# jakovdev/SequenceAligner

Hardware: AMD Instinct MI355X
Metric: pair-alignments/sec (higher is better)
Workload: dtype u16x2; 1 GPU; cfg2: 10000 protein seqs x U[80,120], nw blosum62 {'gap_pen': 4}, all-vs-all packed triangular; pairs=49995000, cells=501594494441, parallelism=pair-range x1

## Files before the change

### include/seqalign_hip.h

```cpp
#ifndef SEQALIGN_HIP_H
#define SEQALIGN_HIP_H

#include <stdbool.h>
#include <stddef.h>
#include <stdint.h>

#ifdef __cplusplus
extern "C" {
#endif

#define SA_ABI_VERSION 4


struct sa_meta {
	int32_t off;
	int32_t len;
};

struct sa_input {
	uint8_t *seqs;
	struct sa_meta *meta;
	int32_t max;
	int32_t num;
};

struct sa_output {
	int32_t *matrix;
	const char **seqs;
	size_t dim;
	bool triangular;
};

enum sa_method { SA_METHOD_NW = 0, SA_METHOD_GA = 1, SA_METHOD_SW = 2, SA_METHOD_COUNT = 3 };
enum sa_gap_kind { SA_GAP_LINEAR = 0, SA_GAP_AFFINE = 1 };

#define SA_LUT_SIZE 128
#define SA_SUB_DIM 24
#define SA_SCORE_MIN (INT32_MIN / 2)

struct sa_scoring {
	int32_t method;
	int32_t gap_pen;
	int32_t gap_opn;
	int32_t gap_ext;
	int32_t lut[SA_LUT_SIZE];
	int32_t sub[SA_SUB_DIM * SA_SUB_DIM];
};


bool sa_hip_memory(size_t bytes);

bool sa_hip_align(struct sa_input in, struct sa_output out, const struct sa_scoring *sc);

int32_t sa_hip_filter(struct sa_input in, float threshold, uint8_t *keep);


typedef struct sa_ctx sa_ctx;

sa_ctx *sa_ctx_create(int device, struct sa_input in, const struct sa_scoring *sc);
void sa_ctx_destroy(sa_ctx *ctx);

int64_t sa_ctx_pairs(const sa_ctx *ctx);

int sa_ctx_align_range(sa_ctx *ctx, int64_t start, int64_t count, int32_t *d_scores, void *stream);

int sa_ctx_token_tiles(const sa_ctx *ctx, int64_t *lean, int64_t *legacy);

int sa_ctx_align_host(sa_ctx *ctx, int64_t start, int64_t count, struct sa_output out, double *phase_seconds);

int sa_hip_host_register(void *p, size_t bytes);
int sa_hip_host_unregister(void *p);

int sa_ctx_scores_fit16(const sa_ctx *ctx);
int sa_ctx_align_range16(sa_ctx *ctx, int64_t start, int64_t count, int16_t *d_scores, void *stream);
int sa_hip_widen16(const int16_t *d_src, int32_t *d_dst, int64_t count, void *stream);

int64_t sa_ctx_share_elems(sa_ctx *ctx, int64_t start, int64_t count, int world, int to_host);
int sa_ctx_align_share(sa_ctx *ctx, int64_t start, int64_t count, int world, int rank, void *d_share, int elem16,
		       int32_t *host_packed, void *stream);
int sa_ctx_place_shares(sa_ctx *ctx, int64_t start, int64_t count, int world, int to_host, const void *d_shares, int elem16,
			int32_t *d_packed, void *stream);

void sa_ctx_leave_room(sa_ctx *ctx, int on);

int sa_ctx_expand_full(sa_ctx *ctx, const int32_t *d_packed, int32_t *d_full, void *stream);

#define SA_HIP_Z_PAIR_LEVEL 7
typedef struct sa_zjob sa_zjob;
sa_zjob *sa_zjob_create(int device, const int32_t *d_packed, const int32_t *d_full, int32_t num, size_t chunk_dim, int level);
size_t sa_zjob_tiles_per_row(const sa_zjob *job);
int sa_zjob_tile_row(sa_zjob *job, size_t tile_row, const uint8_t **streams, size_t *sizes);
int sa_zjob_next(sa_zjob *job, uint32_t *rows, uint32_t *cols, const uint8_t **streams, size_t *sizes);
void sa_zjob_stats(const sa_zjob *job, double *encode_ms, double *copy_ms, uint64_t *raw_bytes, uint64_t *out_bytes);
double sa_zjob_align_seconds(const sa_zjob *job);
void sa_zjob_destroy(sa_zjob *job);
sa_zjob *sa_hip_tiles_begin(struct sa_input in, const struct sa_scoring *sc, size_t chunk_dim, int level);

#define SA_HIP_NEIGHBORS_MAX 64
int sa_ctx_neighbors(sa_ctx *ctx, const int32_t *d_packed, int32_t k, int32_t *d_index, int32_t *d_score, void *stream);
bool sa_hip_neighbors(struct sa_input in, const struct sa_scoring *sc, int32_t k, int32_t *index, int32_t *score);
int sa_zjob_neighbors(sa_zjob *job, int32_t k, int32_t *index, int32_t *score);
double sa_hip_last_neighbors_seconds(void);

enum { SA_ALN_M = 0, SA_ALN_I = 1, SA_ALN_D = 2 };
struct sa_aln {
	int32_t score;
	int32_t a_begin, a_end;
	int32_t b_begin, b_end;
	int32_t columns;
	int32_t identities;
	int32_t cigar_len;
	int64_t cigar_off;
};
typedef struct sa_alns sa_alns;
sa_alns *sa_ctx_alignments(sa_ctx *ctx, const int32_t *a, const int32_t *b, int64_t npairs);
sa_alns *sa_hip_alignments(struct sa_input in, const struct sa_scoring *sc, const int32_t *a, const int32_t *b, int64_t npairs);
const struct sa_aln *sa_alns_records(const sa_alns *alns);
const uint32_t *sa_alns_cigar(const sa_alns *alns, int64_t *runs);
int64_t sa_alns_count(const sa_alns *alns);
void sa_alns_destroy(sa_alns *alns);
double sa_hip_last_alignments_seconds(void);
void sa_hip_last_alignments_breakdown(double *fill_seconds, double *walk_seconds, int64_t *cells, int32_t *batches);

int sa_ctx_edge_offsets(sa_ctx *ctx, const int32_t *d_packed, int32_t min_score, int64_t *d_offsets, void *stream);
int sa_ctx_edge_fill(sa_ctx *ctx, const int32_t *d_packed, int32_t min_score, const int64_t *d_offsets,
		     int32_t *d_index, int32_t *d_score, void *stream);
typedef struct sa_edges sa_edges;
sa_edges *sa_hip_edges(struct sa_input in, const struct sa_scoring *sc, int32_t min_score);
sa_edges *sa_zjob_edges(sa_zjob *job, int32_t min_score);
const int64_t *sa_edges_offsets(const sa_edges *e, int32_t *num);
const int32_t *sa_edges_index(const sa_edges *e, int64_t *count);
const int32_t *sa_edges_score(const sa_edges *e);
void sa_edges_destroy(sa_edges *e);
double sa_hip_last_edges_seconds(void);

size_t sa_linkage_scratch_bytes(int32_t num);
int sa_ctx_linkage(sa_ctx *ctx, const int32_t *d_packed, int32_t *d_pairs, int32_t *d_score, void *d_scratch, void *stream);
typedef struct sa_linkage sa_linkage;
sa_linkage *sa_hip_linkage(struct sa_input in, const struct sa_scoring *sc);
sa_linkage *sa_zjob_linkage(sa_zjob *job);
const int32_t *sa_linkage_pairs(const sa_linkage *l, int32_t *merges);
const int32_t *sa_linkage_score(const sa_linkage *l);
void sa_linkage_destroy(sa_linkage *l);
double sa_hip_last_linkage_seconds(void);
int sa_hip_last_linkage_rounds(void);
int32_t sa_linkage_labels(const int32_t *pairs, const int32_t *score, int32_t num, int32_t min_score, int32_t *labels);
int sa_linkage_merges(const int32_t *pairs, int32_t num, int32_t *left, int32_t *right, int32_t *size);

#define SA_HIP_SELECT_MAX 16
size_t  sa_select_scratch_bytes(int32_t m);
int64_t sa_score_rank(int64_t pairs, double q);
int  sa_ctx_select(sa_ctx *ctx, const int32_t *d_packed, const int64_t *ranks, int32_t m,
		   int32_t *d_value, int64_t *d_below, void *d_scratch, void *stream);
bool sa_hip_select(struct sa_input in, const struct sa_scoring *sc, const int64_t *ranks, int32_t m, int32_t *value, int64_t *below);
int  sa_zjob_select(sa_zjob *job, const int64_t *ranks, int32_t m, int32_t *value, int64_t *below);
sa_edges   *sa_hip_edges_at_rank(struct sa_input in, const struct sa_scoring *sc, int64_t rank, int32_t *min_score, int64_t *below);
sa_linkage *sa_hip_linkage_with_ranks(struct sa_input in, const struct sa_scoring *sc, const int64_t *ranks, int32_t m,
				      int32_t *value, int64_t *below);
double sa_hip_last_select_seconds(void);

enum { SA_NORM_SELF = 0, SA_NORM_LENGTH = 1 };
enum { SA_NORM_MIN = 0, SA_NORM_MAX = 1, SA_NORM_MEAN = 2 };
#define SA_NORM_SCALE 1000000
struct sa_norm {
	int32_t source;
	int32_t rule;
	int32_t *denominators;
};
int32_t sa_norm_value(int32_t s, int32_t di, int32_t dj, int32_t rule);
int sa_ctx_denominators(sa_ctx *ctx, int32_t source, int32_t *d_den, void *stream);
int sa_ctx_normalize(sa_ctx *ctx, const int32_t *d_packed, const int32_t *d_den, int32_t rule, int32_t *d_out, void *stream);
int sa_zjob_normalize(sa_zjob *job, const struct sa_norm *norm);
bool sa_hip_neighbors_norm(struct sa_input in, const struct sa_scoring *sc, int32_t k, int32_t *index, int32_t *score, const struct sa_norm *norm);
sa_edges *sa_hip_edges_norm(struct sa_input in, const struct sa_scoring *sc, int32_t min_score, const struct sa_norm *norm);
sa_linkage *sa_hip_linkage_norm(struct sa_input in, const struct sa_scoring *sc, const struct sa_norm *norm);
bool sa_hip_select_norm(struct sa_input in, const struct sa_scoring *sc, const int64_t *ranks, int32_t m, int32_t *value, int64_t *below,
			const struct sa_norm *norm);
sa_edges *sa_hip_edges_at_rank_norm(struct sa_input in, const struct sa_scoring *sc, int64_t rank, int32_t *min_score, int64_t *below,
				    const struct sa_norm *norm);
sa_linkage *sa_hip_linkage_with_ranks_norm(struct sa_input in, const struct sa_scoring *sc, const int64_t *ranks, int32_t m,
					   int32_t *value, int64_t *below, const struct sa_norm *norm);
double sa_hip_last_normalize_seconds(void);

enum { SA_PID_COLUMNS = 0, SA_PID_SHORTER = 1, SA_PID_LONGER = 2, SA_PID_MEAN = 3 };
struct sa_identity_out {
	int32_t *score, *identities, *columns, *pid;
	int32_t denom;
};
int32_t sa_pid_value(int32_t identities, int32_t columns, int32_t len_i, int32_t len_j, int32_t denom);
int sa_ctx_identity_range(sa_ctx *ctx, int64_t start, int64_t count, const struct sa_identity_out *d_out, void *stream);
bool sa_hip_identity(struct sa_input in, const struct sa_scoring *sc, int32_t denom, int32_t *identities, int32_t *columns, int32_t *pid);
int sa_zjob_identity(sa_zjob *job, int32_t denom);
bool sa_hip_neighbors_pid(struct sa_input in, const struct sa_scoring *sc, int32_t k, int32_t *index, int32_t *score, int32_t denom);
sa_edges *sa_hip_edges_pid(struct sa_input in, const struct sa_scoring *sc, int32_t min_score, int32_t denom);
sa_linkage *sa_hip_linkage_pid(struct sa_input in, const struct sa_scoring *sc, int32_t denom);
bool sa_hip_select_pid(struct sa_input in, const struct sa_scoring *sc, const int64_t *ranks, int32_t m, int32_t *value, int64_t *below,
		       int32_t denom);
sa_edges *sa_hip_edges_at_rank_pid(struct sa_input in, const struct sa_scoring *sc, int64_t rank, int32_t *min_score, int64_t *below,
				   int32_t denom);
sa_linkage *sa_hip_linkage_with_ranks_pid(struct sa_input in, const struct sa_scoring *sc, const int64_t *ranks, int32_t m,
					  int32_t *value, int64_t *below, int32_t denom);
double sa_hip_last_identity_seconds(void);

int64_t sa_pairs_cells(const struct sa_meta *meta, int32_t num, int64_t start, int64_t count);
int sa_pairs_partition(const struct sa_meta *meta, int32_t num, int parts, int64_t *bounds);

void sa_ctx_timing(sa_ctx *ctx, int enable);
int sa_ctx_timing_read(sa_ctx *ctx, char *kernel_name, int cap, int64_t *launches, double *total_ms,
		       int64_t *pairs, int64_t *cells, double *all_kernels_ms);


int sa_matrix_load(const char *name, int32_t lut[SA_LUT_SIZE], int32_t sub[SA_SUB_DIM * SA_SUB_DIM]);
int sa_matrix_count(void);
const char *sa_matrix_name(int index);
int sa_matrix_is_nucleotide(int index);

int sa_method_parse(const char *alias);
const char *sa_method_name(int method);
int sa_method_gap_kind(int method);
// ... 31 lines not shown
```

### sequencealigner_amd/binding.py

```python
from __future__ import annotations

import ctypes as C
import importlib.util
import os
import pathlib
import sys
from dataclasses import dataclass, field
from typing import Iterable, Optional, Sequence

import numpy as np

_LIB_PATH = pathlib.Path(__file__).resolve().parent / "lib" / "libseqalign_hip.so"
_lib: Optional[C.CDLL] = None

LUT_SIZE = 128
NEIGHBORS_MAX = 64
SUB_DIM = 24
SCORE_MIN = -(1 << 30)

METHOD_NW, METHOD_GA, METHOD_SW = 0, 1, 2
GAP_LINEAR, GAP_AFFINE = 0, 1


class AlignError(RuntimeError):
    """A call through the C ABI returned failure (message = sa_last_error())."""


class _Meta(C.Structure):
    _fields_ = [("off", C.c_int32), ("len", C.c_int32)]


class _Input(C.Structure):
    _fields_ = [("seqs", C.c_void_p), ("meta", C.c_void_p), ("max", C.c_int32), ("num", C.c_int32)]


class _Output(C.Structure):
    _fields_ = [("matrix", C.c_void_p), ("seqs", C.c_void_p), ("dim", C.c_size_t), ("triangular", C.c_bool)]


class _Scoring(C.Structure):
    _fields_ = [("method", C.c_int32), ("gap_pen", C.c_int32), ("gap_opn", C.c_int32), ("gap_ext", C.c_int32),
                ("lut", C.c_int32 * LUT_SIZE), ("sub", C.c_int32 * (SUB_DIM * SUB_DIM))]


ABI_SYMBOLS = (
    "sa_hip_memory", "sa_hip_align", "sa_hip_filter", "sa_ctx_create", "sa_ctx_destroy", "sa_ctx_pairs", "sa_pairs_cells",
    "sa_ctx_align_range", "sa_ctx_align_range16", "sa_ctx_token_tiles", "sa_ctx_scores_fit16", "sa_hip_widen16", "sa_ctx_expand_full", "sa_pairs_partition", "sa_ctx_timing", "sa_ctx_timing_read",
    "sa_matrix_load", "sa_matrix_count", "sa_matrix_name", "sa_matrix_is_nucleotide", "sa_method_parse",
    "sa_method_name", "sa_method_gap_kind", "sa_hip_device_count", "sa_hip_device_name", "sa_last_error",
    "sa_abi_version",
    "sa_hip_last_align_seconds", "sa_ctx_align_host", "sa_hip_host_register", "sa_hip_host_unregister",
    "sa_ctx_share_elems", "sa_ctx_align_share", "sa_ctx_place_shares", "sa_hip_last_align_breakdown", "sa_ctx_leave_room", "sa_hip_set_progress",
    "sa_hip_last_align_path",
    "sa_zjob_create", "sa_zjob_destroy", "sa_zjob_tiles_per_row", "sa_zjob_tile_row", "sa_zjob_stats", "sa_zjob_next", "sa_zjob_align_seconds", "sa_hip_tiles_begin",
    "sa_ctx_neighbors", "sa_hip_neighbors", "sa_zjob_neighbors", "sa_hip_last_neighbors_seconds",
    "sa_ctx_alignments", "sa_hip_alignments", "sa_alns_records", "sa_alns_cigar", "sa_alns_count", "sa_alns_destroy",
    "sa_hip_last_alignments_seconds", "sa_hip_last_alignments_breakdown",
    "sa_norm_value", "sa_ctx_denominators", "sa_ctx_normalize", "sa_zjob_normalize", "sa_hip_neighbors_norm", "sa_hip_edges_norm",
    "sa_hip_linkage_norm", "sa_hip_select_norm", "sa_hip_edges_at_rank_norm", "sa_hip_linkage_with_ranks_norm", "sa_hip_last_normalize_seconds",
    "sa_ctx_edge_offsets", "sa_ctx_edge_fill", "sa_hip_edges", "sa_zjob_edges", "sa_edges_offsets", "sa_edges_index", "sa_edges_score",
    "sa_edges_destroy", "sa_hip_last_edges_seconds",
    "sa_linkage_scratch_bytes", "sa_ctx_linkage", "sa_hip_linkage", "sa_zjob_linkage", "sa_linkage_pairs", "sa_linkage_score",
    "sa_linkage_destroy", "sa_hip_last_linkage_seconds", "sa_hip_last_linkage_rounds", "sa_linkage_labels", "sa_linkage_merges",
    "sa_select_scratch_bytes", "sa_score_rank", "sa_ctx_select", "sa_hip_select", "sa_zjob_select", "sa_hip_edges_at_rank",
    "sa_hip_linkage_with_ranks", "sa_hip_last_select_seconds",
    "sa_pid_value", "sa_ctx_identity_range", "sa_hip_identity", "sa_zjob_identity", "sa_hip_neighbors_pid", "sa_hip_edges_pid",
    "sa_hip_linkage_pid", "sa_hip_select_pid", "sa_hip_edges_at_rank_pid", "sa_hip_linkage_with_ranks_pid", "sa_hip_last_identity_seconds",
)


class _Norm(C.Structure):
    _fields_ = [("source", C.c_int32), ("rule", C.c_int32), ("denominators", C.c_void_p)]


class _IdentityOut(C.Structure):
    _fields_ = [("score", C.c_void_p), ("identities", C.c_void_p), ("columns", C.c_void_p), ("pid", C.c_void_p), ("denom", C.c_int32)]


def library_path() -> pathlib.Path:
    return _LIB_PATH


def _share_hip_runtime_with_torch() -> None:
    if "torch" in sys.modules or os.environ.get("SA_HIP_NO_TORCH_RUNTIME"):
        return
    try:
        spec = importlib.util.find_spec("torch")
    except (ImportError, ValueError):
        return
    if spec is None or not spec.submodule_search_locations:
        return
    cand = pathlib.Path(list(spec.submodule_search_locations)[0]) / "lib" / "libamdhip64.so"
    if cand.exists():
        C.CDLL(str(cand), mode=C.RTLD_GLOBAL)


def load_library() -> C.CDLL:
    global _lib
    if _lib is not None:
        return _lib
    if not _LIB_PATH.exists():
        raise AlignError(f"{_LIB_PATH} is missing: run `python __graft_entry__.py` (hipcc, gfx950) first; "
                         "there is no CPU fallback")
    _share_hip_runtime_with_torch()
    lib = C.CDLL(str(_LIB_PATH))
    lib.sa_hip_memory.argtypes = [C.c_size_t]
    lib.sa_hip_memory.restype = C.c_bool
    lib.sa_hip_align.argtypes = [_Input, _Output, C.POINTER(_Scoring)]
    lib.sa_hip_align.restype = C.c_bool
    lib.sa_hip_filter.argtypes = [_Input, C.c_float, C.c_void_p]
    lib.sa_hip_filter.restype = C.c_int32
    lib.sa_ctx_create.argtypes = [C.c_int, _Input, C.POINTER(_Scoring)]
    lib.sa_ctx_create.restype = C.c_void_p
    lib.sa_ctx_destroy.argtypes = [C.c_void_p]
    lib.sa_ctx_destroy.restype = None
    lib.sa_ctx_pairs.argtypes = [C.c_void_p]
    lib.sa_ctx_pairs.restype = C.c_int64
    lib.sa_pairs_cells.argtypes = [C.c_void_p, C.c_int32, C.c_int64, C.c_int64]
    lib.sa_pairs_cells.restype = C.c_int64
    lib.sa_ctx_align_range.argtypes = [C.c_void_p, C.c_int64, C.c_int64, C.c_void_p, C.c_void_p]
    lib.sa_ctx_align_range.restype = C.c_int
    lib.sa_ctx_token_tiles.argtypes = [C.c_void_p, C.POINTER(C.c_int64), C.POINTER(C.c_int64)]
    lib.sa_ctx_token_tiles.restype = C.c_int
    lib.sa_ctx_align_range16.argtypes = [C.c_void_p, C.c_int64, C.c_int64, C.c_void_p, C.c_void_p]
    lib.sa_ctx_align_range16.restype = C.c_int
    lib.sa_ctx_scores_fit16.argtypes = [C.c_void_p]
    lib.sa_ctx_scores_fit16.restype = C.c_int
    lib.sa_hip_widen16.argtypes = [C.c_void_p, C.c_void_p, C.c_int64, C.c_void_p]
    lib.sa_hip_widen16.restype = C.c_int
    lib.sa_ctx_expand_full.argtypes = [C.c_void_p, C.c_void_p, C.c_void_p, C.c_void_p]
    lib.sa_ctx_expand_full.restype = C.c_int
    lib.sa_pairs_partition.argtypes = [C.c_void_p, C.c_int32, C.c_int, C.POINTER(C.c_int64)]
    lib.sa_pairs_partition.restype = C.c_int
    lib.sa_ctx_timing.argtypes = [C.c_void_p, C.c_int]
    lib.sa_ctx_timing.restype = None
    lib.sa_ctx_timing_read.argtypes = [C.c_void_p, C.c_char_p, C.c_int, C.POINTER(C.c_int64), C.POINTER(C.c_double),
                                       C.POINTER(C.c_int64), C.POINTER(C.c_int64), C.POINTER(C.c_double)]
    lib.sa_ctx_timing_read.restype = C.c_int
    lib.sa_matrix_load.argtypes = [C.c_char_p, C.POINTER(C.c_int32), C.POINTER(C.c_int32)]
    lib.sa_matrix_load.restype = C.c_int
    lib.sa_matrix_count.restype = C.c_int
    lib.sa_matrix_name.argtypes = [C.c_int]
    lib.sa_matrix_name.restype = C.c_char_p
    lib.sa_matrix_is_nucleotide.argtypes = [C.c_int]
    lib.sa_matrix_is_nucleotide.restype = C.c_int
    lib.sa_method_parse.argtypes = [C.c_char_p]
    lib.sa_method_parse.restype = C.c_int
    lib.sa_method_name.argtypes = [C.c_int]
    lib.sa_method_name.restype = C.c_char_p
    lib.sa_method_gap_kind.argtypes = [C.c_int]
    lib.sa_method_gap_kind.restype = C.c_int
    lib.sa_hip_device_count.restype = C.c_int
    lib.sa_hip_device_name.argtypes = [C.c_int]
    lib.sa_hip_device_name.restype = C.c_char_p
    lib.sa_last_error.restype = C.c_char_p
    lib.sa_abi_version.restype = C.c_int
    lib.sa_hip_last_align_seconds.restype = C.c_double
    lib.sa_hip_last_align_path.restype = C.c_int
    lib.sa_ctx_align_host.argtypes = [C.c_void_p, C.c_int64, C.c_int64, _Output, C.POINTER(C.c_double)]
    lib.sa_ctx_align_host.restype = C.c_int
    lib.sa_hip_host_register.argtypes = [C.c_void_p, C.c_size_t]
    lib.sa_hip_host_register.restype = C.c_int
    lib.sa_hip_host_unregister.argtypes = [C.c_void_p]
    lib.sa_hip_host_unregister.restype = C.c_int
    lib.sa_hip_last_align_breakdown.argtypes = [C.POINTER(C.c_double), C.c_int]
    lib.sa_hip_last_align_breakdown.restype = C.c_int
    lib.sa_hip_set_progress.argtypes = [C.c_void_p, C.c_void_p]
    lib.sa_hip_set_progress.restype = None
    lib.sa_ctx_leave_room.argtypes = [C.c_void_p, C.c_int]
    lib.sa_ctx_leave_room.restype = None
    lib.sa_ctx_share_elems.argtypes = [C.c_void_p, C.c_int64, C.c_int64, C.c_int, C.c_int]
    lib.sa_ctx_share_elems.restype = C.c_int64
    lib.sa_ctx_align_share.argtypes = [C.c_void_p, C.c_int64, C.c_int64, C.c_int, C.c_int, C.c_void_p, C.c_int, C.c_void_p, C.c_void_p]
    lib.sa_ctx_align_share.restype = C.c_int
    lib.sa_ctx_place_shares.argtypes = [C.c_void_p, C.c_int64, C.c_int64, C.c_int, C.c_int, C.c_void_p, C.c_int, C.c_void_p, C.c_void_p]
    lib.sa_ctx_place_shares.restype = C.c_int
    lib.sa_zjob_create.argtypes = [C.c_int, C.c_void_p, C.c_void_p, C.c_int32, C.c_size_t, C.c_int]
    lib.sa_zjob_create.restype = C.c_void_p
    lib.sa_zjob_destroy.argtypes = [C.c_void_p]
    lib.sa_zjob_destroy.restype = None
    lib.sa_zjob_tiles_per_row.argtypes = [C.c_void_p]
    lib.sa_zjob_tiles_per_row.restype = C.c_size_t
    lib.sa_zjob_tile_row.argtypes = [C.c_void_p, C.c_size_t, C.POINTER(C.c_void_p), C.POINTER(C.c_size_t)]
    lib.sa_zjob_tile_row.restype = C.c_int
    lib.sa_zjob_stats.argtypes = [C.c_void_p, C.POINTER(C.c_double), C.POINTER(C.c_double), C.POINTER(C.c_uint64), C.POINTER(C.c_uint64)]
    lib.sa_zjob_stats.restype = None
    lib.sa_zjob_next.argtypes = [C.c_void_p, C.POINTER(C.c_uint32), C.POINTER(C.c_uint32), C.POINTER(C.c_void_p), C.POINTER(C.c_size_t)]
    lib.sa_zjob_next.restype = C.c_int
    lib.sa_zjob_align_seconds.argtypes = [C.c_void_p]
    lib.sa_zjob_align_seconds.restype = C.c_double
    lib.sa_hip_tiles_begin.argtypes = [_Input, C.POINTER(_Scoring), C.c_size_t, C.c_int]
    lib.sa_hip_tiles_begin.restype = C.c_void_p
    lib.sa_ctx_neighbors.argtypes = [C.c_void_p, C.c_void_p, C.c_int32, C.c_void_p, C.c_void_p, C.c_void_p]
    lib.sa_ctx_neighbors.restype = C.c_int
    lib.sa_hip_neighbors.argtypes = [_Input, C.POINTER(_Scoring), C.c_int32, C.c_void_p, C.c_void_p]
    lib.sa_hip_neighbors.restype = C.c_bool
    lib.sa_zjob_neighbors.argtypes = [C.c_void_p, C.c_int32, C.c_void_p, C.c_void_p]
    lib.sa_zjob_neighbors.restype = C.c_int
    lib.sa_hip_last_neighbors_seconds.restype = C.c_double
    lib.sa_ctx_alignments.argtypes = [C.c_void_p, C.c_void_p, C.c_void_p, C.c_int64]
    lib.sa_ctx_alignments.restype = C.c_void_p
    lib.sa_hip_alignments.argtypes = [_Input, C.POINTER(_Scoring), C.c_void_p, C.c_void_p, C.c_int64]
    lib.sa_hip_alignments.restype = C.c_void_p
    lib.sa_alns_records.argtypes = [C.c_void_p]
    lib.sa_alns_records.restype = C.c_void_p
    lib.sa_alns_cigar.argtypes = [C.c_void_p, C.POINTER(C.c_int64)]
    lib.sa_alns_cigar.restype = C.c_void_p
    lib.sa_alns_count.argtypes = [C.c_void_p]
    lib.sa_alns_count.restype = C.c_int64
    lib.sa_alns_destroy.argtypes = [C.c_void_p]
    lib.sa_alns_destroy.restype = None
    lib.sa_hip_last_alignments_seconds.restype = C.c_double
    lib.sa_hip_last_alignments_breakdown.argtypes = [C.POINTER(C.c_double), C.POINTER(C.c_double), C.POINTER(C.c_int64), C.POINTER(C.c_int32)]
    lib.sa_hip_last_alignments_breakdown.restype = None
    lib.sa_ctx_edge_offsets.argtypes = [C.c_void_p, C.c_void_p, C.c_int32, C.c_void_p, C.c_void_p]
    lib.sa_ctx_edge_offsets.restype = C.c_int
    lib.sa_ctx_edge_fill.argtypes = [C.c_void_p, C.c_void_p, C.c_int32, C.c_void_p, C.c_void_p, C.c_void_p, C.c_void_p]
    lib.sa_ctx_edge_fill.restype = C.c_int
    lib.sa_hip_edges.argtypes = [_Input, C.POINTER(_Scoring), C.c_int32]
    lib.sa_hip_edges.restype = C.c_void_p
    lib.sa_zjob_edges.argtypes = [C.c_void_p, C.c_int32]
    lib.sa_zjob_edges.restype = C.c_void_p
    lib.sa_edges_offsets.argtypes = [C.c_void_p, C.POINTER(C.c_int32)]
    lib.sa_edges_offsets.restype = C.c_void_p
    lib.sa_edges_index.argtypes = [C.c_void_p, C.POINTER(C.c_int64)]
    lib.sa_edges_index.restype = C.c_void_p
    lib.sa_edges_score.argtypes = [C.c_void_p]
    lib.sa_edges_score.restype = C.c_void_p
    lib.sa_edges_destroy.argtypes = [C.c_void_p]
    lib.sa_edges_destroy.restype = None
    lib.sa_hip_last_edges_seconds.restype = C.c_double
    lib.sa_linkage_scratch_bytes.argtypes = [C.c_int32]
    lib.sa_linkage_scratch_bytes.restype = C.c_size_t
    lib.sa_ctx_linkage.argtypes = [C.c_void_p, C.c_void_p, C.c_void_p, C.c_void_p, C.c_void_p, C.c_void_p]
    lib.sa_ctx_linkage.restype = C.c_int
    lib.sa_hip_linkage.argtypes = [_Input, C.POINTER(_Scoring)]
    lib.sa_hip_linkage.restype = C.c_void_p
    lib.sa_zjob_linkage.argtypes = [C.c_void_p]
    lib.sa_zjob_linkage.restype = C.c_void_p
    lib.sa_linkage_pairs.argtypes = [C.c_void_p, C.POINTER(C.c_int32)]
    lib.sa_linkage_pairs.restype = C.c_void_p
    lib.sa_linkage_score.argtypes = [C.c_void_p]
    lib.sa_linkage_score.restype = C.c_void_p
    lib.sa_linkage_destroy.argtypes = [C.c_void_p]
    lib.sa_linkage_destroy.restype = None
    lib.sa_hip_last_linkage_seconds.restype = C.c_double
    lib.sa_hip_last_linkage_rounds.restype = C.c_int
    lib.sa_linkage_labels.argtypes = [C.c_void_p, C.c_void_p, C.c_int32, C.c_int32, C.c_void_p]
    lib.sa_linkage_labels.restype = C.c_int32
    lib.sa_linkage_merges.argtypes = [C.c_void_p, C.c_int32, C.c_void_p, C.c_void_p, C.c_void_p]
    lib.sa_linkage_merges.restype = C.c_int
    lib.sa_select_scratch_bytes.argtypes = [C.c_int32]
    lib.sa_select_scratch_bytes.restype = C.c_size_t
    lib.sa_score_rank.argtypes = [C.c_int64, C.c_double]
    lib.sa_score_rank.restype = C.c_int64
    lib.sa_ctx_select.argtypes = [C.c_void_p, C.c_void_p, C.c_void_p, C.c_int32, C.c_void_p, C.c_void_p, C.c_void_p, C.c_void_p]
    lib.sa_ctx_select.restype = C.c_int
    lib.sa_hip_select.argtypes = [_Input, C.POINTER(_Scoring), C.c_void_p, C.c_int32, C.c_void_p, C.c_void_p]
    lib.sa_hip_select.restype = C.c_bool
    lib.sa_zjob_select.argtypes = [C.c_void_p, C.c_void_p, C.c_int32, C.c_void_p, C.c_void_p]
    lib.sa_zjob_select.restype = C.c_int
    lib.sa_hip_edges_at_rank.argtypes = [_Input, C.POINTER(_Scoring), C.c_int64, C.POINTER(C.c_int32), C.POINTER(C.c_int64)]
    lib.sa_hip_edges_at_rank.restype = C.c_void_p
    lib.sa_hip_linkage_with_ranks.argtypes = [_Input, C.POINTER(_Scoring), C.c_void_p, C.c_int32, C.c_void_p, C.c_void_p]
    lib.sa_hip_linkage_with_ranks.restype = C.c_void_p
    lib.sa_hip_last_select_seconds.restype = C.c_double
    lib.sa_norm_value.argtypes = [C.c_int32, C.c_int32, C.c_int32, C.c_int32]
    lib.sa_norm_value.restype = C.c_int32
    lib.sa_ctx_denominators.argtypes = [C.c_void_p, C.c_int32, C.c_void_p, C.c_void_p]
    lib.sa_ctx_denominators.restype = C.c_int
    lib.sa_ctx_normalize.argtypes = [C.c_void_p, C.c_void_p, C.c_void_p, C.c_int32, C.c_void_p, C.c_void_p]
    lib.sa_ctx_normalize.restype = C.c_int
    lib.sa_zjob_normalize.argtypes = [C.c_void_p, C.POINTER(_Norm)]
    lib.sa_zjob_normalize.restype = C.c_int
    lib.sa_hip_neighbors_norm.argtypes = lib.sa_hip_neighbors.argtypes + [C.POINTER(_Norm)]
    lib.sa_hip_neighbors_norm.restype = C.c_bool
# ... 515 lines not shown

@dataclass
class Alignments:
    pairs: np.ndarray
    records: np.ndarray
    cigar: np.ndarray

    def runs(self, t: int) -> list[tuple[int, str]]:
        r = self.records[t]
        return [(int(w) >> 4, CIGAR_OPS[int(w) & 15]) for w in self.cigar[int(r["cigar_off"]):int(r["cigar_off"]) + int(r["cigar_len"])]]

    def cigar_string(self, t: int) -> str:
        return "".join(f"{n}{op}" for n, op in self.runs(t))

    def aligned(self, t: int, store: "SequenceStore") -> tuple[str, str]:
        r = self.records[t]
        sa, sb = store.sequence(int(self.pairs[t, 0])).decode(), store.sequence(int(self.pairs[t, 1])).decode()
        i, j, ga, gb = int(r["a_begin"]), int(r["b_begin"]), [], []
        for n, op in self.runs(t):
            ga.append(sa[i:i + n] if op != "D" else "-" * n)
            gb.append(sb[j:j + n] if op != "I" else "-" * n)
            i += n if op != "D" else 0
            j += n if op != "I" else 0
        return "".join(ga), "".join(gb)


def _pairs_array(pairs) -> np.ndarray:
    arr = np.asarray(pairs, dtype=np.int64).reshape(-1, 2) if len(pairs) else np.zeros((0, 2), np.int64)
    if arr.size and (arr.min() < -2**31 or arr.max() >= 2**31):
        raise AlignError("pair indices must be int32")
    return np.ascontiguousarray(arr.astype(np.int32))


def _take_alignments(lib, handle, pairs: np.ndarray) -> Alignments:
    if not handle:
        raise AlignError(_err())
    try:
        n = int(lib.sa_alns_count(handle))
        runs = C.c_int64(0)
        cig = lib.sa_alns_cigar(handle, C.byref(runs))
        rec = lib.sa_alns_records(handle)
        records = np.frombuffer(C.string_at(rec, n * ALN_DTYPE.itemsize), dtype=ALN_DTYPE).copy() if n else np.zeros(0, ALN_DTYPE)
        cigar = np.frombuffer(C.string_at(cig, 4 * runs.value), dtype=np.uint32).copy() if runs.value else np.zeros(0, np.uint32)
    finally:
        lib.sa_alns_destroy(handle)
    return Alignments(pairs=pairs, records=records, cigar=cigar)


def hip_alignments(store: SequenceStore, scoring: Scoring, pairs) -> Alignments:
    lib = load_library()
    arr = _pairs_array(pairs)
    a, b = np.ascontiguousarray(arr[:, 0]), np.ascontiguousarray(arr[:, 1])
    sc = scoring._as_c()
    return _take_alignments(lib, lib.sa_hip_alignments(store._as_c(), C.byref(sc), a.ctypes.data, b.ctypes.data, len(arr)), arr)


def last_alignments_seconds() -> float:
    return float(load_library().sa_hip_last_alignments_seconds())


def last_alignments_breakdown() -> dict:
    f, w, c, b = C.c_double(0), C.c_double(0), C.c_int64(0), C.c_int32(0)
    load_library().sa_hip_last_alignments_breakdown(C.byref(f), C.byref(w), C.byref(c), C.byref(b))
    return {"fill_seconds": f.value, "walk_seconds": w.value, "cells": c.value, "batches": b.value}


class PinnedMatrix:

    def __init__(self, elements: int, shared: Optional[str] = None, create: bool = True):
        self._lib = load_library()
        if shared is not None:
            if create:
                with open(shared, "wb") as f:
                    f.truncate(4 * max(int(elements), 1))
            self.array = np.memmap(shared, dtype=np.int32, mode="r+", shape=(max(int(elements), 1),))[:int(elements)]
        else:
            import mmap
            self._map = mmap.mmap(-1, 4 * max(int(elements), 1))
            self.array = np.frombuffer(self._map, dtype=np.int32)[:int(elements)]
        self.path = shared
        self._registered = False
        if elements and self._lib.sa_hip_host_register(C.c_void_p(self.array.ctypes.data), self.array.nbytes):
            raise AlignError(_err())
        self._registered = bool(elements)

    @property
    def ptr(self) -> int:
        return int(self.array.ctypes.data)

    def close(self) -> None:
        if self._registered:
            self._registered = False
            try:
                self._lib.sa_hip_host_unregister(C.c_void_p(self.array.ctypes.data))
            except ImportError:
                pass

    __del__ = close


def hip_filter(store: SequenceStore, threshold: float) -> np.ndarray:
    keep = np.ones(store.num, dtype=np.uint8)
    rc = load_library().sa_hip_filter(store._as_c(), C.c_float(threshold), keep.ctypes.data)
    if rc < 0:
        raise AlignError(_err())
    return keep.astype(bool)


class Context:

    def __init__(self, store: SequenceStore, scoring: Scoring, device: int = 0):
        self._lib = load_library()
        self._store = store
        sc = scoring._as_c()
        self._h = self._lib.sa_ctx_create(int(device), store._as_c(), C.byref(sc))
        if not self._h:
            raise AlignError(_err())
        self.num = store.num
        self.device = int(device)

    def close(self) -> None:
        if getattr(self, "_h", None):
            self._lib.sa_ctx_destroy(self._h)
            self._h = None

    __del__ = close

    def __enter__(self):
        return self

    def __exit__(self, *exc):
        self.close()

    @property
    def pairs(self) -> int:
        return int(self._lib.sa_ctx_pairs(self._h))

    def cells(self, start: int = 0, count: Optional[int] = None) -> int:
        return self._store.cells(start, count)

    def partition(self, parts: int) -> list[int]:
        return self._store.partition(parts)

    def align_range(self, start: int, count: int, d_scores_ptr: int, stream: int = 0) -> None:
        if self._lib.sa_ctx_align_range(self._h, start, count, C.c_void_p(d_scores_ptr), C.c_void_p(stream)):
            raise AlignError(_err())

    def token_tiles(self) -> tuple[int, int]:
        lean, legacy = C.c_int64(0), C.c_int64(0)
        if self._lib.sa_ctx_token_tiles(self._h, C.byref(lean), C.byref(legacy)):
            raise AlignError(_err())
        return int(lean.value), int(legacy.value)

    @property
    def scores_fit16(self) -> bool:
        return bool(self._lib.sa_ctx_scores_fit16(self._h))

    def align_range16(self, start: int, count: int, d_scores16_ptr: int, stream: int = 0) -> None:
        if self._lib.sa_ctx_align_range16(self._h, start, count, C.c_void_p(d_scores16_ptr), C.c_void_p(stream)):
            raise AlignError(_err())

    def widen16(self, d_src16_ptr: int, d_dst32_ptr: int, count: int, stream: int = 0) -> None:
        if self._lib.sa_hip_widen16(C.c_void_p(d_src16_ptr), C.c_void_p(d_dst32_ptr), count, C.c_void_p(stream)):
            raise AlignError(_err())

    def leave_room(self, on: bool) -> None:
        self._lib.sa_ctx_leave_room(self._h, int(on))

    def share_elems(self, start: int, count: int, world: int, to_host: bool = False) -> int:
        v = int(self._lib.sa_ctx_share_elems(self._h, start, count, world, int(to_host)))
        if v < 0:
            raise AlignError(_err())
        return v

    def align_share(self, start: int, count: int, world: int, rank: int, d_share_ptr: int, elem16: bool, stream: int = 0,
                    host_packed_ptr: int = 0) -> None:
        if self._lib.sa_ctx_align_share(self._h, start, count, world, rank, C.c_void_p(d_share_ptr), int(elem16),
                                        C.c_void_p(host_packed_ptr or None), C.c_void_p(stream)):
            raise AlignError(_err())

    def place_shares(self, start: int, count: int, world: int, d_shares_ptr: int, elem16: bool, d_packed_ptr: int, stream: int = 0,
                     to_host: bool = False) -> None:
        if self._lib.sa_ctx_place_shares(self._h, start, count, world, int(to_host), C.c_void_p(d_shares_ptr), int(elem16),
                                         C.c_void_p(d_packed_ptr), C.c_void_p(stream)):
            raise AlignError(_err())

    def align_host(self, matrix: Optional[np.ndarray], triangular: bool, start: int = 0, count: Optional[int] = None) -> float:
        count = self.pairs - start if count is None else count
        out = _Output(matrix.ctypes.data if matrix is not None else None, None, self.num, bool(triangular))
        phase = C.c_double()
        if self._lib.sa_ctx_align_host(self._h, start, count, out, C.byref(phase)):
            raise AlignError(_err())
        return float(phase.value)

    def expand_full(self, d_packed_ptr: int, d_full_ptr: int, stream: int = 0) -> None:
        if self._lib.sa_ctx_expand_full(self._h, C.c_void_p(d_packed_ptr), C.c_void_p(d_full_ptr), C.c_void_p(stream)):
            raise AlignError(_err())

    def neighbors(self, d_packed_ptr: int, k: int, d_index_ptr: int, d_score_ptr: int, stream: int = 0) -> None:
        if self._lib.sa_ctx_neighbors(self._h, C.c_void_p(d_packed_ptr), int(k), C.c_void_p(d_index_ptr), C.c_void_p(d_score_ptr),
                                      C.c_void_p(stream)):
            raise AlignError(_err())

    def edge_offsets(self, d_packed_ptr: int, min_score: int, d_offsets_ptr: int, stream: int = 0) -> None:
        if self._lib.sa_ctx_edge_offsets(self._h, C.c_void_p(d_packed_ptr), _min_score(min_score), C.c_void_p(d_offsets_ptr),
                                         C.c_void_p(stream)):
            raise AlignError(_err())

    def edge_fill(self, d_packed_ptr: int, min_score: int, d_offsets_ptr: int, d_index_ptr: int, d_score_ptr: int, stream: int = 0) -> None:
        if self._lib.sa_ctx_edge_fill(self._h, C.c_void_p(d_packed_ptr), _min_score(min_score), C.c_void_p(d_offsets_ptr),
                                      C.c_void_p(d_index_ptr), C.c_void_p(d_score_ptr), C.c_void_p(stream)):
            raise AlignError(_err())

    def linkage(self, d_packed_ptr: int, d_pairs_ptr: int, d_score_ptr: int, d_scratch_ptr: int, stream: int = 0) -> None:
        if self._lib.sa_ctx_linkage(self._h, C.c_void_p(d_packed_ptr), C.c_void_p(d_pairs_ptr), C.c_void_p(d_score_ptr),
                                    C.c_void_p(d_scratch_ptr), C.c_void_p(stream)):
            raise AlignError(_err())

    def select(self, d_packed_ptr: int, ranks, d_value_ptr: int, d_below_ptr: int, d_scratch_ptr: int, stream: int = 0) -> None:
        r = _ranks(ranks)
        if self._lib.sa_ctx_select(self._h, C.c_void_p(d_packed_ptr), r.ctypes.data, len(r), C.c_void_p(d_value_ptr),
                                   C.c_void_p(d_below_ptr), C.c_void_p(d_scratch_ptr), C.c_void_p(stream)):
            raise AlignError(_err())

    def denominators(self, source: int, d_den_ptr: int, stream: int = 0) -> None:
        source = int(source)
        if not -2**31 <= source < 2**31:
            raise AlignError(f"source = {source} is not an int32")
        if self._lib.sa_ctx_denominators(self._h, source, C.c_void_p(d_den_ptr or None), C.c_void_p(stream)):
            raise AlignError(_err())

    def normalize(self, d_packed_ptr: int, d_den_ptr: int, rule: int, d_out_ptr: int, stream: int = 0) -> None:
        rule = int(rule)
        if not -2**31 <= rule < 2**31:
            raise AlignError(f"rule = {rule} is not an int32")
        if self._lib.sa_ctx_normalize(self._h, C.c_void_p(d_packed_ptr or None), C.c_void_p(d_den_ptr or None), rule,
                                      C.c_void_p(d_out_ptr or None), C.c_void_p(stream)):
            raise AlignError(_err())

    def identity_range(self, start: int, count: int, score: int = 0, identities: int = 0, columns: int = 0, pid: int = 0,
                       denom: int = 0, stream: int = 0) -> None:
        out = _IdentityOut(score or None, identities or None, columns or None, pid or None, _denom(denom))
        if self._lib.sa_ctx_identity_range(self._h, int(start), int(count), C.byref(out), C.c_void_p(stream)):
            raise AlignError(_err())

    def alignments(self, pairs) -> Alignments:
        arr = _pairs_array(pairs)
        a, b = np.ascontiguousarray(arr[:, 0]), np.ascontiguousarray(arr[:, 1])
        return _take_alignments(self._lib, self._lib.sa_ctx_alignments(self._h, a.ctypes.data, b.ctypes.data, len(arr)), arr)

    def timing(self, enable: bool) -> None:
        self._lib.sa_ctx_timing(self._h, int(enable))

    def timing_read(self) -> dict:
        name = C.create_string_buffer(256)
        launches, pairs, cells = C.c_int64(), C.c_int64(), C.c_int64()
        ms, all_ms = C.c_double(), C.c_double()
        if self._lib.sa_ctx_timing_read(self._h, name, 256, C.byref(launches), C.byref(ms), C.byref(pairs),
                                        C.byref(cells), C.byref(all_ms)):
            raise AlignError(_err())
        return dict(kernel=name.value.decode(), launches=int(launches.value), ms=float(ms.value),
                    pairs=int(pairs.value), cells=int(cells.value), all_kernels_ms=float(all_ms.value))


class DeflateJob:

    def __init__(self, num: int, chunk_dim: int, d_packed_ptr: int = 0, d_full_ptr: int = 0, device: int = 0, level: int = 6, _handle=None):
        self._lib = load_library()
        self._h = _handle or self._lib.sa_zjob_create(int(device), C.c_void_p(d_packed_ptr or None), C.c_void_p(d_full_ptr or None),
                                                      int(num), int(chunk_dim), int(level))
        if not self._h:
            raise AlignError(_err())
        self.tiles_per_row = int(self._lib.sa_zjob_tiles_per_row(self._h))
        self.num = int(num)

    @classmethod
    def begin(cls, store: "SequenceStore", scoring: "Scoring", chunk_dim: int, level: int = 6) -> "DeflateJob":
        lib = load_library()
        sc = scoring._as_c()
        h = lib.sa_hip_tiles_begin(store._as_c(), C.byref(sc), int(chunk_dim), int(level))
        if not h:
            raise AlignError(_err())
        job = cls(store.num, chunk_dim, _handle=h)
        job._store = store
        return job

    def next(self) -> list[tuple[int, int, bytes]]:
        n = self.tiles_per_row
        rows, cols = (C.c_uint32 * n)(), (C.c_uint32 * n)()
        ptrs, sizes = (C.c_void_p * n)(), (C.c_size_t * n)()
        got = self._lib.sa_zjob_next(self._h, rows, cols, ptrs, sizes)
        if got < 0:
            raise AlignError(_err())
        return [(int(rows[t]), int(cols[t]), C.string_at(ptrs[t], sizes[t])) for t in range(got)]

    @property
    def align_seconds(self) -> float:
        return float(self._lib.sa_zjob_align_seconds(self._h))

    def tile_row(self, row: int) -> list[bytes]:
        ptrs = (C.c_void_p * self.tiles_per_row)()
        sizes = (C.c_size_t * self.tiles_per_row)()
        if self._lib.sa_zjob_tile_row(self._h, int(row), ptrs, sizes):
            raise AlignError(_err())
        return [C.string_at(ptrs[t], sizes[t]) for t in range(self.tiles_per_row)]

# ... 49 lines not shown
```

### sequencealigner_amd/csrc/sa_context.hip

```cpp
#include <algorithm>
#include <cmath>
#include <cstdio>
#include <cstdlib>
#include <cstring>

#include "sa_ctx.h"

bool sa_device_ready(int device)
{
	int count = 0;
	hipError_t err = hipGetDeviceCount(&count);
	if (err != hipSuccess || count <= 0) {
		sa_set_error("No HIP devices available (%s); libseqalign_hip has no CPU fallback",
			     err == hipSuccess ? "device count is 0" : hipGetErrorString(err));
		return false;
	}
	if (device < 0 || device >= count) {
		sa_set_error("HIP device %d out of range (%d visible)", device, count);
		return false;
	}
	SA_HIP_CHECK(hipSetDevice(device), return false);
	return true;
}

extern "C" int sa_hip_device_count(void)
{
	int count = 0;
	if (hipGetDeviceCount(&count) != hipSuccess)
		return 0;
	return count;
}

extern "C" const char *sa_hip_device_name(int device)
{
	static thread_local char name[256];
	hipDeviceProp_t prop;
	if (hipGetDeviceProperties(&prop, device) != hipSuccess)
		return nullptr;
	snprintf(name, sizeof(name), "%s (%s, %d CUs)", prop.name, prop.gcnArchName, prop.multiProcessorCount);
	return name;
}

static bool validate_and_encode(const sa_input &in, const sa_scoring &sc, std::vector<uint8_t> &codes,
				std::vector<int32_t> &off, int32_t &max_len)
{
	if (!in.seqs || !in.meta) {
		sa_set_error("sa_input: null sequence store");
		return false;
	}
	if (in.num < 2) {
		sa_set_error("Not enough sequences: %d (min: 2)", in.num);
		return false;
	}
	if (sc.method < 0 || sc.method >= SA_METHOD_COUNT) {
		sa_set_error("Invalid alignment method id %d", sc.method);
		return false;
	}
	int64_t end = 0;
	max_len = 0;
	off.assign((size_t)in.num + 1, 0);
	for (int32_t k = 0; k < in.num; k++) {
		const sa_meta m = in.meta[k];
		if (m.len < 1 || m.off < 0) {
			sa_set_error("Sequence #%d has invalid offset/length (%d/%d)", k + 1, m.off, m.len);
			return false;
		}
		off[(size_t)k] = (int32_t)end;
		end += (int64_t)m.len + 1;
		max_len = std::max(max_len, m.len);
		if (end > INT32_MAX) {
			sa_set_error("Sequence store exceeds 2 GiB");
			return false;
		}
	}
	off[(size_t)in.num] = (int32_t)end;
	codes.assign((size_t)end, (uint8_t)SA_CODE_SEP);
	for (int32_t k = 0; k < in.num; k++) {
		const sa_meta m = in.meta[k];
		const uint8_t *s = in.seqs + m.off;
		for (int32_t p = 0; p < m.len; p++) {
			const uint8_t ch = s[p];
			const int32_t idx = ch < SA_LUT_SIZE ? sc.lut[ch] : -1;
			if (idx < 0 || idx >= SA_SUB_DIM) {
				sa_set_error("Invalid character 0x%02x in sequence #%d at position %d", ch, k + 1, p + 1);
				return false;
			}
			codes[(size_t)off[(size_t)k] + p] = (uint8_t)idx;
		}
		if (s[m.len] != 0) {
			sa_set_error("Sequence #%d is not NUL-terminated at its recorded length", k + 1);
			return false;
		}
	}
	int64_t amax = 0, smax = 0;
	if (sc.method == SA_METHOD_NW)
		amax = std::llabs((int64_t)sc.gap_pen);
	else
		amax = std::max(std::llabs((int64_t)sc.gap_opn), std::llabs((int64_t)sc.gap_ext));
	for (int k = 0; k < SA_SUB_DIM * SA_SUB_DIM; k++)
		smax = std::max<int64_t>(smax, std::llabs((int64_t)sc.sub[k]));
	const __int128 bound = (__int128)(2 * (int64_t)max_len + 3) * amax + (__int128)max_len * smax;
	if (bound >= ((__int128)1 << 30)) {
		sa_set_error("Gap penalty %lld with sequence length %d overflows 32-bit scores "
			     "(undefined in the reference as well)", (long long)amax, max_len);
		return false;
	}
	return true;
}

SaPlanInputs sa_plan_inputs(const sa_ctx *ctx)
{
	SaPlanInputs in;
	in.num = ctx->num;
	in.meta = ctx->meta.data();
	in.min_len = ctx->min_len;
	in.method = ctx->sc.method;
	in.gap_ext = ctx->sc.gap_ext;
	in.sys_ok = ctx->sys_ok;
	in.pk_kmax = ctx->pk_kmax;
	in.pk16_kmax = ctx->pk16_kmax;
	in.pk16_f16_kmax = ctx->pk16_f16_kmax;
	in.pk_chunk_cap = ctx->pk_chunk_cap;
	in.pk_q = ctx->pk_q;
	in.pk_floor = ctx->pk_floor;
	in.pk_gain = ctx->pk_gain;
	in.pk_slack = ctx->pk_slack;
	in.persistent_wgs = ctx->persistent_wgs;
	in.env_chunk = ctx->env.chunk;
	in.no_sort = ctx->env.no_sort;
	in.no_tokens = ctx->env.no_tokens;
	return in;
}

namespace {
struct CtxDeleter {
	void operator()(sa_ctx *c) const { sa_ctx_destroy(c); }
};
}

static sa_ctx *ctx_create_impl(int device, struct sa_input in, const struct sa_scoring *sc)
{
	if (!sc) {
		sa_set_error("sa_ctx_create: null scoring");
		return nullptr;
	}
	std::vector<uint8_t> codes;
	std::vector<int32_t> off;
	int32_t max_len = 0;
	const auto t_encode = std::chrono::steady_clock::now();
	if (!validate_and_encode(in, *sc, codes, off, max_len))
		return nullptr;
	const double encode_ms = sa_ms_since(t_encode);
	const SaEnv env = sa_env_read();
	const bool verbose = env.verbose;
	const auto t_create = std::chrono::steady_clock::now();
	auto since = [&]() { return std::chrono::duration<double, std::milli>(std::chrono::steady_clock::now() - t_create).count(); };
	if (!sa_device_ready(device))
		return nullptr;
	const double device_ms = since();
	if (verbose)
		fprintf(stderr, "[seqalign_hip] sa_ctx_create: device ready at %.1f ms\n", since());

	std::unique_ptr<sa_ctx, CtxDeleter> holder(new sa_ctx());
	sa_ctx *ctx = holder.get();
	ctx->env = env;
	ctx->setup.encode = encode_ms;
	ctx->setup.device = device_ms;
	ctx->device = device;
	ctx->num = in.num;
	ctx->max_len = max_len;
	ctx->min_len = max_len;
	for (int32_t k = 0; k < in.num; k++)
		ctx->min_len = std::min<int32_t>(ctx->min_len, (int32_t)in.meta[k].len);
	ctx->pairs = (int64_t)in.num * (in.num - 1) / 2;
	ctx->sc = *sc;
	ctx->meta.resize((size_t)in.num);
	for (int32_t k = 0; k < in.num; k++)
		ctx->meta[(size_t)k] = sa_meta{ off[(size_t)k], in.meta[k].len };
	ctx->off = off;
	ctx->codes = codes;
	{
		const SaKernelLimits L = sa_kernel_limits(*sc, max_len, ctx->min_len, env.force_generic, env.no_pk, env.no_pk16);
		ctx->sys_ok = L.sys_ok;
		ctx->sys_pconst = L.sys_pconst;
		ctx->sys_q = L.sys_q;
		ctx->sys_gain = L.sys_gain;
		ctx->sys_slack = L.sys_slack;
		ctx->pk_kmax = L.pk_kmax;
		ctx->pk16_kmax = L.pk16_kmax;
		ctx->pk16_f16_kmax = L.pk16_f16_kmax;
		ctx->pk_chunk_cap = L.pk_chunk_cap;
		ctx->pk_pconst = L.pk_pconst;
		ctx->pk_q = L.pk_q;
		ctx->pk_floor = L.pk_floor;
		ctx->pk_gain = L.pk_gain;
		ctx->pk_slack = L.pk_slack;
		ctx->pk_extra = L.pk_extra;
	}
	const bool col_major = sc->method != SA_METHOD_NW;
	int8_t sub8[SA_SUB_DIM * SA_SUB_DIM];
	for (int a = 0; a < SA_SUB_DIM; a++)
		for (int b = 0; b < SA_SUB_DIM; b++)
			sub8[a * SA_SUB_DIM + b] = (int8_t)std::max(-128, std::min(127, sc->sub[col_major ? b * SA_SUB_DIM + a : a * SA_SUB_DIM + b]));

	bool ok = false;
	do {
		SA_HIP_CHECK(hipMalloc(&ctx->d_codes, codes.size()), break);
		SA_HIP_CHECK(hipMalloc(&ctx->d_meta, sizeof(sa_meta) * (size_t)in.num), break);
		SA_HIP_CHECK(hipMalloc(&ctx->d_sub, sizeof(sc->sub)), break);
		if (verbose)
			fprintf(stderr, "[seqalign_hip] sa_ctx_create: first allocations at %.1f ms\n", since());
		SA_HIP_CHECK(hipMemcpy(ctx->d_codes, codes.data(), codes.size(), hipMemcpyHostToDevice), break);
		if (verbose)
			fprintf(stderr, "[seqalign_hip] sa_ctx_create: first upload at %.1f ms\n", since());
		SA_HIP_CHECK(hipMemcpy(ctx->d_meta, ctx->meta.data(), sizeof(sa_meta) * (size_t)in.num, hipMemcpyHostToDevice), break);
		SA_HIP_CHECK(hipMemcpy(ctx->d_sub, sc->sub, sizeof(sc->sub), hipMemcpyHostToDevice), break);
		SA_HIP_CHECK(hipMalloc(&ctx->d_off, sizeof(int32_t) * off.size()), break);
		SA_HIP_CHECK(hipMemcpy(ctx->d_off, off.data(), sizeof(int32_t) * off.size(), hipMemcpyHostToDevice), break);
		SA_HIP_CHECK(hipMalloc(&ctx->d_sub8, sizeof(sub8)), break);
		SA_HIP_CHECK(hipMemcpy(ctx->d_sub8, sub8, sizeof(sub8), hipMemcpyHostToDevice), break);
		if (verbose)
			fprintf(stderr, "[seqalign_hip] sa_ctx_create: uploads at %.1f ms\n", since());

		hipDeviceProp_t prop;
		SA_HIP_CHECK(hipGetDeviceProperties(&prop, device), break);
		ctx->scratch_stride = 2 * ((int64_t)max_len + 2);
		int64_t blocks = (int64_t)prop.multiProcessorCount * 8;
		const int64_t budget = (int64_t)1 << 30;
		const int64_t per_block = ctx->scratch_stride * 4 * (int64_t)sizeof(int32_t);
		blocks = std::max<int64_t>(prop.multiProcessorCount, std::min(blocks, budget / per_block));
		ctx->generic_blocks = (int)blocks;
		SA_HIP_CHECK(hipMalloc(&ctx->d_scratch, (size_t)(blocks * per_block)), break);
		SA_HIP_CHECK(hipMalloc(&ctx->d_counters, sizeof(unsigned) * sa_ctx::COUNTER_SLOTS * sa_ctx::COUNTERS_PER_SLOT), break);
		SA_HIP_CHECK(hipMemset(ctx->d_counters, 0, sizeof(unsigned) * sa_ctx::COUNTER_SLOTS * sa_ctx::COUNTERS_PER_SLOT), break);
		if (verbose)
			fprintf(stderr, "[seqalign_hip] sa_ctx_create: scratch at %.1f ms\n", since());
		ctx->persistent_wgs = prop.multiProcessorCount * 32;
		int families = 0;
		for (int32_t k = 0; k < in.num; k++) {
			const int n = in.meta[k].len, k8 = (n + 7) / 8, k16 = (n + 15) / 16;
			families |= k8 <= ctx->pk_kmax ? SA_WARM_PK8
				    : (k16 >= SA_PK_K16_MIN && k16 <= ctx->pk16_kmax) ? (sa_pk_bundle_klo(16, k16) >= 45 ? SA_WARM_PK16HI : SA_WARM_PK16)
										       : SA_WARM_S32;
		}
		if (verbose)
			fprintf(stderr, "[seqalign_hip] sa_ctx_create: buffers, streams and events at %.1f ms\n", since());
		ctx->setup.upload = since() - device_ms;
		const double t_warm = since();
		SA_HIP_CHECK(sa_warm_kernels(sc->method, families), break);
		ctx->setup.code_objects = since() - t_warm;
		if (verbose)
			fprintf(stderr, "[seqalign_hip] sa_ctx_create: code objects of families %d loaded at %.1f ms\n", families, since());
		ok = true;
	} while (0);
	if (!ok)
		return nullptr;
	return holder.release();
}

extern "C" sa_ctx *sa_ctx_create(int device, struct sa_input in, const struct sa_scoring *sc)
{
	return sa_guard("sa_ctx_create", (sa_ctx *)nullptr, [&] { return ctx_create_impl(device, in, sc); });
}

extern "C" void sa_ctx_destroy(sa_ctx *ctx)
{
	if (!ctx)
		return;
	(void)hipSetDevice(ctx->device);
	for (auto &ev : ctx->events) {
		(void)hipEventDestroy(ev.e0);
		(void)hipEventDestroy(ev.e1);
	}
	sa_plan_release(ctx);
	sa_deliver_release(ctx);
	for (auto &ar : ctx->arranged) {
		(void)hipFree(ar.d_codes);
		(void)hipFree(ar.d_off);
		(void)hipFree(ar.d_rowmap);
		(void)hipFree(ar.d_posmap);
		(void)hipFree(ar.d_tok);
		(void)hipFree(ar.d_tok_off);
		(void)hipFree(ar.d_mine);
// ... 157 lines not shown
```

### sequencealigner_amd/csrc/sa_ctx.h

```cpp
#ifndef SA_CTX_H
#define SA_CTX_H

#include <atomic>
#include <chrono>
#include <deque>
#include <exception>
#include <memory>
#include <new>
#include <string>
#include <vector>

#include "sa_env.h"
#include "sa_guard.h"
#include "sa_internal.h"
#include "sa_plan.h"

struct sa_ctx {
	int device = 0;
	int32_t num = 0, max_len = 0, min_len = 0;
	int64_t pairs = 0;
	sa_scoring sc{};
	SaEnv env;
	std::vector<sa_meta> meta;
	std::vector<int32_t> off;
	std::vector<uint8_t> codes;
	uint8_t *d_codes = nullptr;
	sa_meta *d_meta = nullptr;
	int32_t *d_off = nullptr;
	int32_t *d_sub = nullptr;
	int8_t *d_sub8 = nullptr;
	int32_t *d_scratch = nullptr;
	int64_t scratch_stride = 0;
	int generic_blocks = 0;
	void *d_id_scratch = nullptr;
	enum { COUNTER_SLOTS = 256, COUNTERS_PER_SLOT = 2 * SA_PLAN_NCLASSES };
	unsigned *d_counters = nullptr;
	uint64_t call_no = 0;
	hipEvent_t slot_done[COUNTER_SLOTS] = {};
	bool slot_dirty[COUNTER_SLOTS] = {};
	int32_t *d_long_scratch = nullptr;
	int64_t long_stride = 0;
	int long_wgs = 0;
	int persistent_wgs = 0;
	bool sys_ok = false;
	int32_t sys_pconst = 0, sys_q = 0;
	int64_t sys_gain = 0, sys_slack = 0;
	int pk_kmax = 0, pk16_kmax = 0;
	int pk16_f16_kmax = 0;
	int pk_chunk_cap = SA_SYS_CHUNK;
	int32_t pk_pconst = 0, pk_q = 0, pk_floor = 0;
	int64_t pk_gain = 0, pk_slack = 0, pk_extra = 0;
	struct Arranged {
		SaArrKey key;
		uint8_t *d_codes = nullptr;
		int32_t *d_off = nullptr, *d_rowmap = nullptr, *d_posmap = nullptr;
		uint16_t *d_tok = nullptr, *d_mine = nullptr, *d_any = nullptr;
		int32_t *d_tok_off = nullptr;
	};
	std::deque<Arranged> arranged;
	int64_t tok_lean = 0, tok_legacy = 0;
	bool out_is_host = false;
	struct Plan {
		SaHostPlan h;
		struct DevClass {
			int32_t *d_jlist = nullptr, *d_tprefix = nullptr, *d_tlist = nullptr;
			int64_t *d_doff = nullptr;
		};
		struct DevBundle {
			SaPkClassArgs *d_args = nullptr;
			uint32_t *d_ulist = nullptr;
		};
		std::vector<DevClass> dc;
		std::vector<DevBundle> db;
		SaPlaceSeg *d_segs = nullptr;
		int32_t nsegs = 0;
		uint64_t stamp = 0;
	};
	std::vector<std::unique_ptr<Plan>> plans;
	Plan *plan = nullptr;
	uint64_t plan_clock = 0;
	bool timing = false;
	struct Timed {
		std::string name;
		hipEvent_t e0, e1;
		int64_t pairs, cells;
	};
	std::vector<Timed> events;
	bool leave_room = false;
	struct ProgItem {
		const unsigned *counter;
		int64_t tiles;
	};
	std::vector<ProgItem> prog_items;
	struct SetupMs {
		double encode = 0, device = 0, upload = 0, code_objects = 0, pin = 0, plan = 0, arrange = 0;
	} setup;
	struct Deliver {
		hipStream_t compute = nullptr, copy = nullptr;
		hipEvent_t done[2] = {}, copied[2] = {};
		int32_t *d_buf[2] = {};
		int64_t buf_elems[2] = {};
		int32_t *h_stage[2] = {};
		int64_t stage_elems[2] = {};
		int32_t *d_packed = nullptr, *d_full = nullptr;
		int64_t packed_elems = 0, full_elems = 0;
		unsigned *h_counters = nullptr;
		int64_t h_counters_n = 0;
	} dl;
};

static inline double sa_ms_since(std::chrono::steady_clock::time_point t0)
{
	return std::chrono::duration<double, std::milli>(std::chrono::steady_clock::now() - t0).count();
}

bool sa_device_ready(int device);
bool sa_arranged_store(sa_ctx *ctx, const SaArrKey &key, const sa_ctx::Arranged **out);
SaPlanInputs sa_plan_inputs(const sa_ctx *ctx);

void sa_plan_release(sa_ctx *ctx);
bool sa_plan_get(sa_ctx *ctx, int64_t start, int64_t count, int world, bool share_host);
bool sa_prepare_range(sa_ctx *ctx, int64_t start, int64_t count, bool host_out);
int sa_align_range_impl(sa_ctx *ctx, int64_t start, int64_t count, int32_t *d_scores, void *stream, bool out16,
			int world = 0, int rank = 0, int32_t *host_out = nullptr);

void sa_deliver_release(sa_ctx *ctx);
bool sa_host_range_is_pinned(const void *p, size_t bytes);
size_t sa_host_available_bytes();
bool sa_host_range_in_malloc_heap(const void *p, size_t bytes);

bool sa_progress_wanted();
void sa_report_progress(double fraction);
void sa_progress_speaker(bool here);
int sa_devices_in_use(const SaEnv &env);

bool sa_align_gathered(struct sa_input in, struct sa_output out, const struct sa_scoring *sc, const int *devices, int ndev,
		       double *phase_seconds, double *breakdown_ms);
bool sa_rccl_available(std::string *why);

bool sa_norm_check(const char *who, const struct sa_norm *norm);
bool sa_normalize_in_place(const char *who, sa_ctx *ctx, int32_t *d_packed, const struct sa_norm *norm, hipStream_t s);

bool sa_identity_denom_check(const char *who, int32_t denom);
bool sa_identity_in_place(const char *who, sa_ctx *ctx, int32_t *d_packed, int32_t denom, hipStream_t s);

#endif
```

### sequencealigner_amd/csrc/sa_env.cpp

```cpp
#include "sa_env.h"

#include <algorithm>
#include <cstdlib>

static bool flag(const char *name) { return getenv(name) != nullptr; }
static int number(const char *name, int fallback, int lo, int hi)
{
	const char *v = getenv(name);
	if (!v || !*v)
		return fallback;
	return std::max(lo, std::min(hi, atoi(v)));
}

SaEnv sa_env_read()
{
	SaEnv e;
	e.force_generic = flag("SA_HIP_FORCE_GENERIC");
	e.no_pk = flag("SA_HIP_NO_PK");
	e.no_pk16 = flag("SA_HIP_NO_PK16");
	e.no_sort = flag("SA_HIP_NO_SORT");
	e.no_tokens = flag("SA_HIP_NO_TOKENS");
	e.chunk = number("SA_HIP_CHUNK", 0, 1, 32);
	e.stagger = number("SA_HIP_STAGGER", 0, 0, 64);
	e.no_pin = flag("SA_HIP_NO_PIN");
	e.no_direct = flag("SA_HIP_NO_DIRECT");
	e.no_shells = flag("SA_HIP_NO_SHELLS");
	e.devices = number("SA_HIP_DEVICES", 0, 0, 1024);
	e.split = number("SA_HIP_SPLIT", 0, 0, 1024);
	e.gather = getenv("SA_HIP_GATHER") ? (atoi(getenv("SA_HIP_GATHER")) != 0) : -1;
	e.tiles_split = number("SA_HIP_TILES_SPLIT", 0, 0, 64);
	e.trace_batch_bytes = getenv("SA_HIP_TRACE_BATCH_BYTES") ? std::max(0LL, atoll(getenv("SA_HIP_TRACE_BATCH_BYTES"))) : 0LL;
	e.identity_batch_bytes = getenv("SA_HIP_IDENTITY_BATCH_BYTES") ? std::max(0LL, atoll(getenv("SA_HIP_IDENTITY_BATCH_BYTES"))) : 0LL;
	e.verbose = flag("SA_HIP_VERBOSE");
	e.stamps = flag("SA_HIP_STAMPS");
	e.stamps_dump = getenv("SA_HIP_STAMPS_DUMP");
	e.ztrace = flag("SA_HIP_ZTRACE");
	return e;
}
```

### sequencealigner_amd/csrc/sa_env.h

```cpp
#ifndef SA_ENV_H
#define SA_ENV_H

struct SaEnv {
	bool force_generic = false;
	bool no_pk = false;
	bool no_pk16 = false;
	bool no_sort = false;
	bool no_tokens = false;
	int chunk = 0;
	int stagger = 0;
	bool no_pin = false;
	bool no_direct = false;
	bool no_shells = false;
	int devices = 0;
	int split = 0;
	int gather = -1;
	int tiles_split = 0;
	long long trace_batch_bytes = 0;
	long long identity_batch_bytes = 0;
	bool verbose = false;
	bool stamps = false;
	const char *stamps_dump = nullptr;
	bool ztrace = false;
};

SaEnv sa_env_read();

#endif
```

### sequencealigner_amd/csrc/sa_internal.h

```cpp
#ifndef SA_INTERNAL_H
#define SA_INTERNAL_H

#include <hip/hip_runtime.h>
#include <cstdint>
#include <cstdarg>
#include <string>
#include <vector>


#include "sa_shapes.h"

#define SA_HIP_CHECK(call, onfail)                                                  \
	if (hipError_t err__ = (call); err__ != hipSuccess) {                       \
		sa_set_error("%s failed: %s", #call, hipGetErrorString(err__));      \
		onfail;                                                              \
	} else                                                                      \
		(void)0

struct SaSeqStore {
	const uint8_t *codes;
	const struct sa_meta *meta;
	int32_t num;
};

struct SaGenericArgs {
	SaSeqStore st;
	int32_t *host_out;
	const int32_t *sub;
	int32_t gap_pen, gap_opn, gap_ext;
	int64_t start, count;
	int32_t *out;
	int32_t out16;
	int32_t *scratch;
	int64_t scratch_stride;
};

struct SaSysArgs {
	const uint8_t *codes;
	const int32_t *off;
	const int8_t *sub8;
	const int32_t *jlist;
	const int32_t *tprefix;
	int32_t ncols, num;
	int64_t start, end;
	int32_t *out;
	int32_t out16;
	int32_t pconst;
	int32_t q;
	int32_t gap_g, gap_o, gap_e;
	int32_t delta;
	int32_t chunk;
	int32_t *long_scratch;
	int64_t long_stride;
	int32_t pk_base;
	const SaArranged *lvp;
	int32_t npart;
	int32_t out_nt;
	int32_t pk_f16;
	const int32_t *tlist;
	const int64_t *dense_off;
	int32_t *host_out;
	int32_t nlocal;
	const SaPkClassArgs *pkc;
	const uint32_t *ulist;
	int32_t tile_pair;
	int32_t npkc;
	unsigned *counter;
	int32_t rotate_prio;
	int32_t stagger;
	int32_t stamp_u;
	unsigned long long *stamps;
};

hipError_t sa_launch_place(const SaPlaceSeg *segs, int32_t nsegs, const void *shares, int elem16, int32_t *packed, hipStream_t s);

hipError_t sa_launch_systolic(int method, int cls, const SaSysArgs &a, int workgroups, hipStream_t s);
hipError_t sa_launch_systolic_pk(int method, int g, int klo, int f16, const SaSysArgs &a, int workgroups, unsigned lds_bytes,
				 hipStream_t s);
enum : int { SA_WARM_S32 = 1, SA_WARM_PK8 = 2, SA_WARM_PK16 = 4, SA_WARM_PK16HI = 8 };
hipError_t sa_warm_kernels(int method, int families);

hipError_t sa_launch_generic(int method, const SaGenericArgs &a, int blocks, hipStream_t s);
const char *sa_generic_kernel_name(int method);

long long sa_filter_row_offset(long long j);
hipError_t sa_launch_filter_relation(const uint8_t *codes, const int32_t *off, int32_t num, float threshold,
				      unsigned long long *rel, int32_t jt0, int32_t tile_rows, hipStream_t s);

hipError_t sa_launch_expand_full(const int32_t *packed, int32_t *full, int32_t num, hipStream_t s);
hipError_t sa_launch_expand_shell(const int32_t *packed, int64_t pbase, int32_t *full, int32_t num, int32_t ja, int32_t jb,
				  hipStream_t s);
hipError_t sa_launch_widen16(const int16_t *src, int32_t *dst, int64_t count, hipStream_t s);

bool sa_neighbors_check(const char *who, int64_t num, int32_t k);
hipError_t sa_launch_neighbors(const int32_t *packed, int32_t num, int32_t k, int32_t *index, int32_t *score, hipStream_t s);
bool sa_neighbors_to_host(const int32_t *d_packed, int32_t num, int32_t k, int32_t *index, int32_t *score, hipStream_t s);

struct sa_edges;
sa_edges *sa_edges_to_host(const char *who, const int32_t *d_packed, int32_t num, int32_t min_score, hipStream_t s);

struct sa_linkage;
sa_linkage *sa_linkage_to_host(const char *who, const int32_t *d_packed, int32_t num, hipStream_t s);

bool sa_select_check(const char *who, int32_t num, const int64_t *ranks, int32_t m);
bool sa_select_to_host(const char *who, const int32_t *d_packed, int32_t num, const int64_t *ranks, int32_t m, int32_t *value, int64_t *below,
		       hipStream_t s);

#endif
```

### sequencealigner_amd/csrc/sa_launch.hip

```cpp
#include <algorithm>
#include <cstdio>
#include <cstring>

#include "sa_ctx.h"


static void plan_free_device(sa_ctx::Plan &pl)
{
	for (auto &c : pl.dc) {
		(void)hipFree(c.d_jlist);
		(void)hipFree(c.d_tprefix);
		(void)hipFree(c.d_tlist);
		(void)hipFree(c.d_doff);
	}
	(void)hipFree(pl.d_segs);
	for (auto &b : pl.db) {
		(void)hipFree(b.d_args);
		(void)hipFree(b.d_ulist);
	}
	pl.dc.clear();
	pl.db.clear();
	pl.d_segs = nullptr;
}

void sa_plan_release(sa_ctx *ctx)
{
	for (auto &pl : ctx->plans)
		plan_free_device(*pl);
	ctx->plans.clear();
	ctx->plan = nullptr;
}

template <typename T> static bool upload(T *&dst, const std::vector<T> &v)
{
	SA_HIP_CHECK(hipMalloc(reinterpret_cast<void **>(&dst), sizeof(T) * std::max<size_t>(v.size(), 1)), return false);
	if (!v.empty()) {
		SA_HIP_CHECK(hipMemcpy(dst, v.data(), sizeof(T) * v.size(), hipMemcpyHostToDevice), return false);
	}
	return true;
}

static bool resolve_levels(sa_ctx *ctx, const SaArrKey (&keys)[SA_PK_SORT_LEVELS], SaArranged (&lv)[SA_PK_SORT_LEVELS])
{
	for (int l = 0; l < SA_PK_SORT_LEVELS; l++) {
		lv[l] = SaArranged{};
		if (!keys[l].block)
			continue;
		const sa_ctx::Arranged *ar = nullptr;
		if (!sa_arranged_store(ctx, keys[l], &ar))
			return false;
		if (ar)
			lv[l] = { ar->d_codes, ar->d_off, ar->d_rowmap, ar->d_posmap, ar->key.block, ar->d_tok, ar->d_tok_off, ar->d_mine, ar->d_any };
	}
	return true;
}

static bool plan_upload(sa_ctx *ctx, sa_ctx::Plan &pl)
{
	const SaHostPlan &h = pl.h;
	pl.dc.resize(h.classes.size());
	for (size_t ci = 0; ci < h.classes.size(); ci++) {
		const auto &cl = h.classes[ci];
		auto &d = pl.dc[ci];
		if (!upload(d.d_jlist, cl.jlist) || !upload(d.d_tprefix, cl.tprefix))
			return false;
		if (h.world >= 1 && (!upload(d.d_tlist, cl.tlist) || !upload(d.d_doff, cl.doff)))
			return false;
	}
	if (h.world >= 1 && !h.segs.empty()) {
		std::vector<SaPlaceSeg> segs(h.segs.size());
		for (size_t k = 0; k < h.segs.size(); k++) {
			const SaHostSeg &hs = h.segs[k];
			SaPlaceSeg &sg = segs[k];
			sg = SaPlaceSeg{};
			sg.src = hs.src;
			sg.dst = hs.dst;
			sg.count = hs.count;
			sg.pos0 = hs.pos0;
			sg.ia = hs.ia;
			sg.ib = hs.ib;
			sg.flags = hs.flags;
			sg.map = nullptr;
			if (hs.map_kind) {
				const sa_ctx::Arranged *ar = nullptr;
				if (!sa_arranged_store(ctx, hs.key, &ar))
					return false;
				if (!ar) {
					sa_set_error("plan: placement names an arranged copy the store does not have");
					return false;
				}
				sg.map = hs.map_kind == 2 ? ar->d_posmap : ar->d_rowmap;
			}
		}
		if (!upload(pl.d_segs, segs))
			return false;
		pl.nsegs = (int32_t)segs.size();
	}
	pl.db.resize(h.bundles.size());
	for (size_t bi = 0; bi < h.bundles.size(); bi++) {
		const auto &b = h.bundles[bi];
		std::vector<SaPkClassArgs> args(b.args.size());
		for (size_t x = 0; x < b.args.size(); x++) {
			const SaHostPkArgs &ha = b.args[x];
			SaPkClassArgs &a = args[x];
			a = SaPkClassArgs{};
			if (!resolve_levels(ctx, ha.lv, a.lv))
				return false;
			const auto &d = pl.dc[(size_t)ha.cls_index];
			a.jlist = d.d_jlist;
			a.tprefix = d.d_tprefix;
			a.dense_off = h.world >= 1 ? d.d_doff : nullptr;
			a.ncols = ha.ncols;
			a.npart = ha.npart;
			a.k = ha.k;
			a.delta = ha.delta;
			a.pk_base = ha.pk_base;
			a.chunk = ha.chunk;
		}
		if (!upload(pl.db[bi].d_args, args) || !upload(pl.db[bi].d_ulist, b.ulist))
			return false;
	}
	return true;
}

bool sa_plan_get(sa_ctx *ctx, int64_t start, int64_t count, int world, bool share_host)
{
	for (auto &pl : ctx->plans)
		if (pl->h.start == start && pl->h.count == count && pl->h.world == world && pl->h.share_host == share_host) {
			pl->stamp = ++ctx->plan_clock;
			ctx->plan = pl.get();
			return true;
		}
	const auto t_plan = std::chrono::steady_clock::now();
	struct Acc {
		sa_ctx *c;
		std::chrono::steady_clock::time_point t;
		double a0;
		~Acc() { c->setup.plan += sa_ms_since(t) - (c->setup.arrange - a0); }
	} acc{ ctx, t_plan, ctx->setup.arrange };
	constexpr size_t MAX_PLANS = 160;
	ctx->plan = nullptr;
	if (ctx->plans.size() >= MAX_PLANS) {
		size_t victim = 0;
		for (size_t k = 1; k < ctx->plans.size(); k++)
			if (ctx->plans[k]->stamp < ctx->plans[victim]->stamp)
				victim = k;
		plan_free_device(*ctx->plans[victim]);
		ctx->plans.erase(ctx->plans.begin() + (long)victim);
	}
	std::unique_ptr<sa_ctx::Plan> pl(new sa_ctx::Plan());
	if (!sa_plan_host(sa_plan_inputs(ctx), start, count, world, share_host, pl->h))
		return false;
	struct Undo {
		sa_ctx::Plan *p;
		~Undo()
		{
			if (p)
				plan_free_device(*p);
		}
	} undo{ pl.get() };
	if (!plan_upload(ctx, *pl))
		return false;
	pl->stamp = ++ctx->plan_clock;
	ctx->plans.push_back(std::move(pl));
	undo.p = nullptr;
	ctx->plan = ctx->plans.back().get();
	return true;
}

bool sa_prepare_range(sa_ctx *ctx, int64_t start, int64_t count, bool host_out)
{
	if (count <= 0)
		return true;
	return sa_plan_get(ctx, start, count, 0, host_out);
}


static const char *const METHOD_TAG[] = { "nw", "ga", "sw" };

static void print_stamps(const sa_ctx *ctx, const char *name, bool is_pk, const std::vector<unsigned long long> &h, size_t nstamp)
{
	if (!nstamp)
		return;
	if (!is_pk) {
		double cyc = 0, rt = 0, steps = 0;
		for (size_t k = 0; k < nstamp; k++) {
			cyc += (double)h[3 * k];
			rt += (double)h[3 * k + 1];
			steps += (double)h[3 * k + 2];
		}
		fprintf(stderr, "[stamps] %s: %zu wave-tiles, %.1f cycles/step per wave, clock %.0f MHz, %.0f steps/tile\n",
			name, nstamp, cyc / steps, cyc / rt * 100.0, steps / (double)nstamp);
		return;
	}
	unsigned long long t_lo = ~0ull, t_hi = 0;
	double busy = 0;
	for (size_t k = 0; k < nstamp; k++) {
		t_lo = std::min(t_lo, h[3 * k]);
		t_hi = std::max(t_hi, h[3 * k + 1]);
		busy += (double)(h[3 * k + 1] - h[3 * k]);
	}
	const double span = (double)(t_hi - t_lo);
	constexpr int BINS = 20;
	double act[BINS] = {};
	for (size_t k = 0; k < nstamp; k++) {
		const double a0 = (double)(h[3 * k] - t_lo) / span * BINS, a1 = (double)(h[3 * k + 1] - t_lo) / span * BINS;
		for (int b = (int)a0; b < BINS && b <= (int)a1; b++)
			act[b] += std::min(a1, (double)b + 1) - std::max(a0, (double)b);
	}
	if (ctx->env.stamps_dump) {
		if (FILE *f = fopen(ctx->env.stamps_dump, "wb")) {
			fwrite(h.data(), sizeof(h[0]), h.size(), f);
			fclose(f);
		}
	}
	double clocks = 0, pro = 0, loop = 0, epi = 0, steps = 0;
	for (size_t k = 0; k < nstamp; k++) {
		const unsigned long long c0 = h[3 * k + 2], c1 = h[3 * nstamp + 3 * k], c2 = h[3 * nstamp + 3 * k + 1], c3 = h[6 * nstamp + k];
		clocks += (double)(c3 - c0);
		pro += (double)(c1 - c0);
		loop += (double)(c2 - c1);
		epi += (double)(c3 - c2);
		steps += (double)h[3 * nstamp + 3 * k + 2];
	}
	fprintf(stderr, "[stamps] per tile: prologue %.0f clocks, main loop %.0f (%.0f steps, %.1f clocks per step), epilogue %.0f\n",
		pro / (double)nstamp, loop / (double)nstamp, steps / (double)nstamp, loop / steps, epi / (double)nstamp);
	fprintf(stderr, "[stamps] %s: %zu tiles, makespan %.1f us, mean tile %.1f us = %.0f shader clocks (%.0f MHz), mean active workgroups %.0f; active per 5%% of the launch:",
		name, nstamp, span / 100.0, busy / (double)nstamp / 100.0, clocks / (double)nstamp, clocks / busy * 100.0, busy / span);
	for (int b = 0; b < BINS; b++)
		fprintf(stderr, " %.0f", act[b]);
	double fine[10] = {}, rows_end[10] = {}, n_end[10] = {};
	for (size_t k = 0; k < nstamp; k++) {
		const double a0 = ((double)(h[3 * k] - t_lo) / span - 0.9) * 100.0, a1 = ((double)(h[3 * k + 1] - t_lo) / span - 0.9) * 100.0;
		for (int b = std::max(0, (int)a0); b < 10 && b <= (int)a1; b++)
			fine[b] += std::min(a1, (double)b + 1) - std::max(a0, (double)b);
		if (a1 >= 0) {
			const int b = std::min(9, (int)a1);
			rows_end[b] += (double)h[3 * nstamp + 3 * k + 2];
			n_end[b] += 1;
		}
	}
	fprintf(stderr, "; per 1%% of the last tenth (mean steps of the tiles ending there):");
	for (int b = 0; b < 10; b++)
		fprintf(stderr, " %.0f(%.0f)", fine[b], n_end[b] ? rows_end[b] / n_end[b] : 0.0);
	fprintf(stderr, "\n");
}

struct Launch {
	SaSysArgs a{};
	bool is_pk = false;
	int cls = -1, g = 0, klo = 0;
	bool f16 = false;
	unsigned lds = 0;
	int wgs = 0;
	int32_t ntiles = 0;
	int64_t pairs = 0, cells = 0;
	size_t nstamp = 0, stamp_words = 0;
	char name[96] = "";
};

static bool timed_begin(sa_ctx *ctx, hipStream_t s, hipEvent_t &e0, hipEvent_t &e1)
{
	if (!ctx->timing)
		return true;
	SA_HIP_CHECK(hipEventCreate(&e0), return false);
	SA_HIP_CHECK(hipEventCreate(&e1), return false);
	SA_HIP_CHECK(hipEventRecord(e0, s), return false);
	return true;
}

static bool timed_end(sa_ctx *ctx, hipStream_t s, const std::string &name, hipEvent_t e0, hipEvent_t e1, int64_t pairs, int64_t cells)
{
	if (!ctx->timing)
		return true;
	SA_HIP_CHECK(hipEventRecord(e1, s), return false);
	ctx->events.push_back(sa_ctx::Timed{ name, e0, e1, pairs, cells });
	return true;
}

static Launch pk_launch(const sa_ctx *ctx, const sa_ctx::Plan &pl, size_t bi, int rk, bool share, unsigned *counters, const SaSysArgs &common)
{
	const SaHostBundle &b = pl.h.bundles[bi];
	Launch L;
	L.is_pk = true;
	L.g = b.g;
	L.klo = b.klo;
	L.f16 = b.f16;
	L.lds = (unsigned)sa_pk_lds_bytes(ctx->sc.method, b.g, b.kmax);
	SaSysArgs &a = L.a = common;
	a.pconst = ctx->pk_pconst;
	a.q = ctx->sc.method == SA_METHOD_SW ? 0 : ctx->pk_q;
	a.out_nt = ctx->out_is_host && !share ? 1 : 0;
	a.pk_f16 = b.f16;
	a.chunk = pl.h.chunk_pk;
	a.stagger = ctx->env.stagger;
	a.rotate_prio = ctx->sc.method != SA_METHOD_NW;
	a.pkc = pl.db[bi].d_args;
	a.ulist = pl.db[bi].d_ulist + b.ufirst[(size_t)rk];
	a.npkc = (int32_t)b.cls.size();
	a.nlocal = L.ntiles = b.nlocal[(size_t)rk];
	a.counter = counters + 2 * (SA_PK_CLASS0 + (int)bi);
	L.pairs = b.pairs[(size_t)rk];
	L.cells = b.cells[(size_t)rk];
	L.nstamp = (size_t)L.ntiles;
	L.stamp_words = 7 * L.nstamp;
	L.wgs = (int)std::min<int64_t>(ctx->persistent_wgs / 32 * (ctx->leave_room ? 3 : 4), L.ntiles);
	int klo_seen = b.kmax;
	for (int ci : b.cls)
		klo_seen = std::min(klo_seen, sa_pk_decode(pl.h.classes[(size_t)ci].cls).k);
	snprintf(L.name, sizeof(L.name), "sa_k_systolic_pk_bundle<%s,%d,%d,%s>[K%d-%d]", METHOD_TAG[ctx->sc.method], b.g, b.klo,
		 b.f16 ? "true" : "false", klo_seen, b.kmax);
	return L;
}

static bool long_scratch_ready(sa_ctx *ctx)
{
	if (ctx->d_long_scratch)
		return true;
	ctx->long_stride = 2 * (16 * ((int64_t)ctx->max_len + 1) + 64);
	const int64_t budget_ints = ((int64_t)4 << 30) / 4;
	const int64_t wpb = SA_SYS_WPB(64, true);
	ctx->long_wgs = (int)std::max<int64_t>(16, std::min<int64_t>(ctx->persistent_wgs / 4, budget_ints / (ctx->long_stride * wpb)));
	SA_HIP_CHECK(hipMalloc(&ctx->d_long_scratch, sizeof(int32_t) * (size_t)(ctx->long_stride * ctx->long_wgs * wpb)), return false);
	return true;
}

static bool sys_launch(sa_ctx *ctx, const sa_ctx::Plan &pl, size_t ci, bool share, int rank, unsigned *counters, const SaSysArgs &common,
		       Launch &L)
{
	const SaHostClass &cl = pl.h.classes[ci];
	const auto &dc = pl.dc[ci];
	const int cls = L.cls = cl.cls;
	const bool is_long = cls == SA_SYS_CLASS_LONG;
	const int64_t W = is_long ? ((int64_t)ctx->max_len + SA_SYS_LONG_W - 1) / SA_SYS_LONG_W * SA_SYS_LONG_W
				  : SA_SYS_CLASSES[cls].G * SA_SYS_CLASSES[cls].K;
	SaSysArgs &a = L.a = common;
	a.jlist = dc.d_jlist;
	a.tprefix = dc.d_tprefix;
	a.npart = cl.npart;
	a.ncols = cl.ncols;
	a.pconst = ctx->sys_pconst;
	a.q = ctx->sys_q;
	a.delta = (int32_t)(ctx->sys_gain * W + ctx->sys_slack);
	a.counter = counters + 2 * cls;
	a.chunk = is_long ? std::min(pl.h.chunk, 16) : pl.h.chunk;
	L.ntiles = cl.ntiles;
	L.pairs = cl.pairs;
	L.cells = cl.cells;
	if (share) {
		a.tlist = dc.d_tlist + cl.rank_first[(size_t)rank];
		a.nlocal = L.ntiles = cl.rank_first[(size_t)rank + 1] - cl.rank_first[(size_t)rank];
		a.dense_off = dc.d_doff;
		L.pairs = cl.rank_pairs[(size_t)rank];
		L.cells = cl.rank_cells[(size_t)rank];
	}
	L.nstamp = (size_t)cl.ntiles;
	L.stamp_words = 3 * L.nstamp;
	if (is_long) {
		if (!long_scratch_ready(ctx))
			return false;
		a.long_scratch = ctx->d_long_scratch;
		a.long_stride = ctx->long_stride;
		snprintf(L.name, sizeof(L.name), "sa_k_systolic<%s,G64,K16,strips>", METHOD_TAG[ctx->sc.method]);
	} else {
		snprintf(L.name, sizeof(L.name), "sa_k_systolic<%s,G%d,K%d>", METHOD_TAG[ctx->sc.method], SA_SYS_CLASSES[cls].G,
			 SA_SYS_CLASSES[cls].K);
	}
	L.wgs = (int)std::min<int64_t>(is_long ? ctx->long_wgs : ctx->persistent_wgs, L.ntiles);
	return true;
}

static bool run_launch(sa_ctx *ctx, Launch &L, hipStream_t s)
{
	unsigned long long *d_stamps = nullptr;
	if (ctx->env.stamps) {
		SA_HIP_CHECK(hipMalloc(&d_stamps, sizeof(unsigned long long) * std::max<size_t>(L.stamp_words, 1)), return false);
		SA_HIP_CHECK(hipMemset(d_stamps, 0, sizeof(unsigned long long) * std::max<size_t>(L.stamp_words, 1)), return false);
		L.a.stamps = d_stamps;
	}
	ctx->prog_items.push_back({ L.a.counter, L.ntiles });
	hipEvent_t e0 = nullptr, e1 = nullptr;
	if (!timed_begin(ctx, s, e0, e1))
		return false;
	if (L.is_pk) {
		SA_HIP_CHECK(sa_launch_systolic_pk(ctx->sc.method, L.g, L.klo, L.f16, L.a, L.wgs, L.lds, s), return false);
	} else {
		SA_HIP_CHECK(sa_launch_systolic(ctx->sc.method, L.cls, L.a, L.wgs, s), return false);
	}
	if (d_stamps) {
		std::vector<unsigned long long> h(L.stamp_words);
		SA_HIP_CHECK(hipStreamSynchronize(s), return false);
		SA_HIP_CHECK(hipMemcpy(h.data(), d_stamps, h.size() * sizeof(h[0]), hipMemcpyDeviceToHost), return false);
		(void)hipFree(d_stamps);
		print_stamps(ctx, L.name, L.is_pk, h, L.nstamp);
	}
	return timed_end(ctx, s, L.name, e0, e1, L.pairs, L.cells);
}

static bool generic_runs(sa_ctx *ctx, const SaHostPlan &hp, int64_t start, int32_t *d_scores, hipStream_t s, bool out16, bool share, int rank,
			 int32_t *host_out)
{
	std::vector<std::pair<int64_t, int64_t>> runs = hp.generic;
	std::vector<int64_t> run_out;
	if (share) {
		runs.clear();
		for (const auto &gs : hp.generic_share[(size_t)rank]) {
			runs.emplace_back(gs.start, gs.count);
			run_out.push_back(gs.doff);
		}
	}
	for (size_t ri = 0; ri < runs.size(); ri++) {
		const auto &run = runs[ri];
		const int64_t out_at = share ? run_out[ri] : run.first - start;
		SaGenericArgs a{};
		a.st.codes = ctx->d_codes;
		a.st.meta = ctx->d_meta;
		a.st.num = ctx->num;
		a.sub = ctx->d_sub;
		a.gap_pen = ctx->sc.gap_pen;
		a.gap_opn = ctx->sc.gap_opn;
		a.gap_ext = ctx->sc.gap_ext;
		a.start = run.first;
		a.count = run.second;
		a.out = out16 ? reinterpret_cast<int32_t *>(reinterpret_cast<int16_t *>(d_scores) + out_at) : d_scores + out_at;
		a.out16 = out16 ? 1 : 0;
		a.host_out = host_out ? host_out + (run.first - start) : nullptr;
		a.scratch = ctx->d_scratch;
		a.scratch_stride = ctx->scratch_stride;
		const int blocks = (int)std::min<int64_t>(ctx->generic_blocks, (run.second + 3) / 4);
		hipEvent_t e0 = nullptr, e1 = nullptr;
		if (!timed_begin(ctx, s, e0, e1))
			return false;
		SA_HIP_CHECK(sa_launch_generic(ctx->sc.method, a, blocks, s), return false);
		int64_t run_cells = 0;
		if (ctx->timing) {
			SaPairPlan pp(ctx->meta.data(), ctx->num);
			run_cells = pp.cells_before(run.first + run.second) - pp.cells_before(run.first);
		}
		if (!timed_end(ctx, s, sa_generic_kernel_name(ctx->sc.method), e0, e1, run.second, run_cells))
			return false;
	}
	return true;
}

static int align_range_launches(sa_ctx *ctx, int64_t start, int64_t count, int32_t *d_scores, hipStream_t s, bool out16,
				int world, int rank, int32_t *host_out, size_t slot)
{
	const bool share = world >= 1;
	const sa_ctx::Plan &pl = *ctx->plan;
	const int rk = share ? rank : 0;
	unsigned *const counters = ctx->d_counters + slot * sa_ctx::COUNTERS_PER_SLOT;
	SaSysArgs common{};
	common.codes = ctx->d_codes;
	common.off = ctx->d_off;
	common.sub8 = ctx->d_sub8;
	common.num = ctx->num;
	common.start = start;
	common.end = start + count;
	common.out = d_scores;
	common.out16 = out16 ? 1 : 0;
	common.gap_g = ctx->sc.gap_pen;
	common.gap_o = ctx->sc.gap_opn;
	common.gap_e = ctx->sc.gap_ext;
	common.host_out = host_out;

	ctx->prog_items.clear();
	ctx->tok_lean = ctx->tok_legacy = 0;
	for (size_t bi = 0; bi < pl.h.bundles.size(); bi++) {
		if (pl.h.bundles[bi].nlocal[(size_t)rk] <= 0)
			continue;
		ctx->tok_lean += pl.h.bundles[bi].tok_lean[(size_t)rk];
		ctx->tok_legacy += pl.h.bundles[bi].tok_legacy[(size_t)rk];
		Launch L = pk_launch(ctx, pl, bi, rk, share, counters, common);
		if (!run_launch(ctx, L, s))
			return 1;
	}
	for (size_t ci = 0; ci < pl.h.classes.size(); ci++) {
		const SaHostClass &cl = pl.h.classes[ci];
		if (cl.cls >= SA_PK_CLASS0)
			continue;
		if (share && cl.rank_first[(size_t)rank + 1] == cl.rank_first[(size_t)rank])
			continue;
		Launch L;
		if (!sys_launch(ctx, pl, ci, share, rank, counters, common, L) || !run_launch(ctx, L, s))
			return 1;
	}
	SA_HIP_CHECK(hipEventRecord(ctx->slot_done[slot], s), return 1);
	return generic_runs(ctx, pl.h, start, d_scores, s, out16, share, rank, host_out) ? 0 : 1;
}

int sa_align_range_impl(sa_ctx *ctx, int64_t start, int64_t count, int32_t *d_scores, void *stream, bool out16, int world, int rank,
			int32_t *host_out)
{
	if (!ctx || start < 0 || count < 0 || start > ctx->pairs - count || (!d_scores && count)) {
		sa_set_error("sa_ctx_align_range: bad range [%lld,+%lld) of %lld pairs", (long long)start,
			     (long long)count, ctx ? (long long)ctx->pairs : -1LL);
		return 1;
	}
	if (count == 0)
		return 0;
	SA_HIP_CHECK(hipSetDevice(ctx->device), return 1);
	hipStream_t s = (hipStream_t)stream;
	const bool share = world >= 1;
	if (!sa_plan_get(ctx, start, count, world, share ? host_out != nullptr : ctx->out_is_host))
		return 1;
	const size_t slot = (size_t)(ctx->call_no++ % sa_ctx::COUNTER_SLOTS);
	if (ctx->slot_done[slot]) {
		SA_HIP_CHECK(hipStreamWaitEvent(s, ctx->slot_done[slot], 0), return 1);
	} else {
		SA_HIP_CHECK(hipEventCreateWithFlags(&ctx->slot_done[slot], hipEventDisableTiming), return 1);
	}
	if (ctx->slot_dirty[slot]) {
		SA_HIP_CHECK(hipDeviceSynchronize(), return 1);
		SA_HIP_CHECK(hipMemsetAsync(ctx->d_counters + slot * sa_ctx::COUNTERS_PER_SLOT, 0,
					    sizeof(unsigned) * sa_ctx::COUNTERS_PER_SLOT, s), return 1);
		ctx->slot_dirty[slot] = false;
	}
	int rc = 1;
	struct Mark {
		sa_ctx *c;
		size_t slot;
		int *rc;
		~Mark()
		{
			if (*rc)
				c->slot_dirty[slot] = true;
		}
	} mark{ ctx, slot, &rc };
	rc = align_range_launches(ctx, start, count, d_scores, s, out16, world, rank, host_out, slot);
	return rc;
}

extern "C" int sa_ctx_token_tiles(const sa_ctx *ctx, int64_t *lean, int64_t *legacy)
{
	return sa_guard("sa_ctx_token_tiles", 1, [&] {
		if (!ctx || !lean || !legacy) {
			sa_set_error("sa_ctx_token_tiles: null argument");
			return 1;
		}
		*lean = ctx->tok_lean;
		*legacy = ctx->tok_legacy;
		return 0;
	});
}

extern "C" int sa_ctx_align_range(sa_ctx *ctx, int64_t start, int64_t count, int32_t *d_scores, void *stream)
{
	return sa_guard("sa_ctx_align_range", 1, [&] { return sa_align_range_impl(ctx, start, count, d_scores, stream, false); });
}

static int64_t score_magnitude_bound(const sa_ctx *ctx)
{
	int64_t smax = 0;
	for (int k = 0; k < SA_SUB_DIM * SA_SUB_DIM; k++)
		smax = std::max<int64_t>(smax, std::llabs((long long)ctx->sc.sub[k]));
	const int64_t L = ctx->max_len;
	const int64_t gap = std::max<int64_t>(std::llabs((long long)ctx->sc.gap_pen),
					      std::max<int64_t>(std::llabs((long long)ctx->sc.gap_opn), std::llabs((long long)ctx->sc.gap_ext)));
	return L * smax + 2 * L * gap;
}

extern "C" int sa_ctx_scores_fit16(const sa_ctx *ctx)
{
	return ctx && score_magnitude_bound(ctx) <= 32767 ? 1 : 0;
}

extern "C" int sa_ctx_align_range16(sa_ctx *ctx, int64_t start, int64_t count, int16_t *d_scores, void *stream)
{
	if (!sa_ctx_scores_fit16(ctx)) {
		sa_set_error("sa_ctx_align_range16: scores of this store and scoring are not provably within int16");
		return 1;
	}
	return sa_guard("sa_ctx_align_range16", 1,
			[&] { return sa_align_range_impl(ctx, start, count, reinterpret_cast<int32_t *>(d_scores), stream, true); });
}

extern "C" int sa_hip_widen16(const int16_t *d_src, int32_t *d_dst, int64_t count, void *stream)
{
	if (count < 0 || (count && (!d_src || !d_dst))) {
		sa_set_error("sa_hip_widen16: bad arguments");
		return 1;
	}
	SA_HIP_CHECK(sa_launch_widen16(d_src, d_dst, count, (hipStream_t)stream), return 1);
	return 0;
}

static bool share_args_ok(sa_ctx *ctx, int64_t start, int64_t count, int world, const char *who)
{
	if (!ctx || start < 0 || count <= 0 || start > ctx->pairs - count || world < 1 || world > 1024) {
		sa_set_error("%s: bad range [%lld,+%lld) of %lld pairs or world %d", who, (long long)start, (long long)count,
			     ctx ? (long long)ctx->pairs : -1LL, world);
		return false;
	}
	return true;
}

extern "C" void sa_ctx_leave_room(sa_ctx *ctx, int on)
{
	if (ctx)
		ctx->leave_room = on != 0;
}

extern "C" int64_t sa_ctx_share_elems(sa_ctx *ctx, int64_t start, int64_t count, int world, int to_host)
{
	return sa_guard("sa_ctx_share_elems", (int64_t)-1, [&]() -> int64_t {
		if (!share_args_ok(ctx, start, count, world, "sa_ctx_share_elems"))
			return -1;
		SA_HIP_CHECK(hipSetDevice(ctx->device), return -1);
		if (!sa_plan_get(ctx, start, count, world, to_host != 0))
			return -1;
		return ctx->plan->h.share_elems;
	});
}

extern "C" int sa_ctx_align_share(sa_ctx *ctx, int64_t start, int64_t count, int world, int rank, void *d_share, int elem16,
				   int32_t *host_packed, void *stream)
{
	return sa_guard("sa_ctx_align_share", 1, [&] {
		if (!share_args_ok(ctx, start, count, world, "sa_ctx_align_share"))
			return 1;
		if (rank < 0 || rank >= world || !d_share) {
			sa_set_error("sa_ctx_align_share: rank %d of %d, share buffer %p", rank, world, d_share);
			return 1;
		}
		if (elem16 && !sa_ctx_scores_fit16(ctx)) {
			sa_set_error("sa_ctx_align_share: scores of this store and scoring are not provably within int16");
			return 1;
		}
		int32_t *host_dev = nullptr;
		if (host_packed) {
			SA_HIP_CHECK(hipSetDevice(ctx->device), return 1);
			void *dp = nullptr;
			if (!sa_host_range_is_pinned(host_packed + start, sizeof(int32_t) * (size_t)count) ||
			    hipHostGetDevicePointer(&dp, host_packed + start, 0) != hipSuccess) {
				(void)hipGetLastError();
				sa_set_error("sa_ctx_align_share: the host matrix is not page-locked over the range (sa_hip_host_register)");
				return 1;
			}
			host_dev = static_cast<int32_t *>(dp);
		}
		return sa_align_range_impl(ctx, start, count, static_cast<int32_t *>(d_share), stream, elem16 != 0, world, rank, host_dev);
	});
}

extern "C" int sa_ctx_place_shares(sa_ctx *ctx, int64_t start, int64_t count, int world, int to_host, const void *d_shares,
				    int elem16, int32_t *d_packed, void *stream)
{
	return sa_guard("sa_ctx_place_shares", 1, [&] {
		if (!share_args_ok(ctx, start, count, world, "sa_ctx_place_shares"))
			return 1;
		if (!d_shares || !d_packed) {
			sa_set_error("sa_ctx_place_shares: null buffer");
			return 1;
		}
		SA_HIP_CHECK(hipSetDevice(ctx->device), return 1);
		if (!sa_plan_get(ctx, start, count, world, to_host != 0))
			return 1;
		SA_HIP_CHECK(sa_launch_place(ctx->plan->d_segs, ctx->plan->nsegs, d_shares, elem16, d_packed, (hipStream_t)stream), return 1);
		return 0;
	});
}

extern "C" int sa_ctx_expand_full(sa_ctx *ctx, const int32_t *d_packed, int32_t *d_full, void *stream)
{
	if (!ctx || !d_packed || !d_full) {
		sa_set_error("sa_ctx_expand_full: null argument");
		return 1;
	}
	SA_HIP_CHECK(hipSetDevice(ctx->device), return 1);
	SA_HIP_CHECK(sa_launch_expand_full(d_packed, d_full, ctx->num, (hipStream_t)stream), return 1);
	return 0;
}
```

### sequencealigner_amd/csrc/sa_plan.cpp

```cpp
#include "sa_plan.h"
#include "sa_guard.h"

#include <algorithm>
#include <cmath>
#include <cstdlib>

int32_t sa_column_of(int64_t p)
{
	int64_t j = (int64_t)((1.0 + std::sqrt(1.0 + 8.0 * (double)p)) * 0.5);
	while (j * (j - 1) / 2 > p)
		--j;
	while ((j + 1) * j / 2 <= p)
		++j;
	return (int32_t)j;
}

SaPairPlan::SaPairPlan(const sa_meta *m, int32_t n) : num(n), pairs((int64_t)n * (n - 1) / 2), meta(m)
{
	len_prefix.assign((size_t)n + 1, 0);
	cell_prefix.assign((size_t)n + 1, 0);
	for (int32_t k = 0; k < n; k++) {
		len_prefix[(size_t)k + 1] = len_prefix[(size_t)k] + m[k].len;
		cell_prefix[(size_t)k + 1] = cell_prefix[(size_t)k] + (int64_t)m[k].len * len_prefix[(size_t)k];
	}
// ... 41 lines not shown
	const int64_t wave_rows = (int64_t)key.ng * key.ch;
	return key.block > 0 && wave_rows > 0 && key.block % (wave_rows * SA_PK_WPB) == 0 && key.block <= num;
}

int sa_pk_arranged_keys(const SaPlanInputs &in, int pk_g, int pk_k, int32_t chunk_pk, bool host_out, SaArrKey (&lv)[SA_PK_SORT_LEVELS])
{
	for (auto &x : lv)
		x = SaArrKey{};
	if (in.no_sort || chunk_pk <= 0)
		return 0;
	const int ng = 64 / pk_g;
	const int32_t rows = sa_pk_wpb(in.method, pk_g, pk_k) * ng * chunk_pk;
	int nl = 0;
	for (int l = 0; l < SA_PK_SORT_LEVELS; l++) {
		const int32_t block = SA_PK_SORT_ROWS >> l;
		if (host_out || rows >= SA_PK_ROWS_OWN_BLOCK || block <= rows || block % rows != 0)
			continue;
		const SaArrKey key{ ng, chunk_pk, block };
		if (sa_arranged_exists(in.num, key))
			lv[nl++] = key;
	}
	if (nl < SA_PK_SORT_LEVELS) {
		const SaArrKey key{ ng, chunk_pk, rows };
		if (sa_arranged_exists(in.num, key))
			lv[nl++] = key;
	}
	return nl;
}

void sa_arrange_rows(const sa_meta *meta, int32_t num, const SaArrKey &key, std::vector<int32_t> &rowmap)
{
	rowmap.resize((size_t)num);
	for (int32_t i = 0; i < num; i++)
		rowmap[(size_t)i] = i;
	if (!sa_arranged_exists(num, key))
		return;
	const int ng = key.ng, ch = key.ch;
	const int32_t block = key.block;
	const int32_t wave_rows = ng * ch;
	const int32_t slots = block / wave_rows;
	std::vector<int32_t> idx((size_t)block), rounds, rest;
	for (int32_t b0 = 0; b0 + block <= num; b0 += block) {
		for (int32_t k = 0; k < block; k++)
			idx[(size_t)k] = b0 + k;
		std::stable_sort(idx.begin(), idx.end(), [&](int32_t a, int32_t b) { return meta[a].len > meta[b].len; });
		rounds.clear();
		rest.clear();
		for (int32_t k = 0; k < block;) {
			int32_t e = k;
			while (e < block && meta[idx[(size_t)e]].len == meta[idx[(size_t)k]].len)
				e++;
			const int32_t pure = (e - k) / ng * ng;
			rounds.insert(rounds.end(), idx.begin() + k, idx.begin() + k + pure);
			rest.insert(rest.end(), idx.begin() + k + pure, idx.begin() + e);
			k = e;
		}
		rounds.insert(rounds.end(), rest.begin(), rest.end());
		for (int32_t r = 0; r < block / ng; r++) {
			const int32_t pass = r / slots, w = r % slots;
			const int32_t slot = (pass & 1) ? slots - 1 - w : w;
			for (int g = 0; g < ng; g++) {
				const int gg = (pass & 1) ? ng - 1 - g : g;
				rowmap[(size_t)(b0 + slot * wave_rows + gg * ch + pass)] = rounds[(size_t)(r * ng + g)];
			}
		}
	}
}

bool sa_build_tokens(const uint8_t *codes, const int32_t *off, int32_t num, const SaArrKey &key, SaTokenStreams &ts)
{
	ts = SaTokenStreams();
	if (!sa_arranged_exists(num, key))
		return true;
	const int ng = key.ng, ch = key.ch, g = 64 / ng;
	const int32_t streams = num / key.block * (key.block / ch), slots = streams / ng;
	ts.streams = streams;
	ts.tok_off.resize((size_t)streams + 1);
	int64_t total = 0;
	for (int32_t w = 0; w < slots; w++) {
		int32_t smax = 0;
		for (int s = w * ng; s < (w + 1) * ng; s++)
			smax = std::max(smax, off[(size_t)(s + 1) * ch] - off[(size_t)s * ch]);
		const int32_t nblk = (smax + g - 1 + 15) >> 4, padded = 16 * sa_token_blocks(smax, g);
		if (padded < 16 * (nblk + 1) + 16 || padded != (smax + g - 1 + 15) / 16 * 16 + 32) {
			sa_set_error("token streams: padded length %d does not cover the lookahead of %d blocks", padded, nblk);
			return false;
		}
		for (int s = w * ng; s < (w + 1) * ng; s++) {
			ts.tok_off[(size_t)s] = (int32_t)total;
			total += padded;
		}
		if (total > (int64_t)1 << 30) {
			sa_set_error("token streams: store too large for 32-bit stream offsets");
			return false;
		}
	}
	ts.tok_off[(size_t)streams] = (int32_t)total;
	ts.tok.assign((size_t)total, (uint16_t)SA_CODE_NOP);
	ts.mine.assign((size_t)(total / 16), 0);
	ts.any.assign((size_t)(total / 16 / ng), 0);
	for (int32_t s = 0; s < streams; s++) {
		const int32_t b = off[(size_t)s * ch], n = off[(size_t)(s + 1) * ch] - b, at = ts.tok_off[(size_t)s];
		const int32_t any_at = ts.tok_off[(size_t)(s / ng * ng)] / 16 / ng;
		for (int32_t p = 0; p < n; p++) {
			const uint8_t c = codes[(size_t)b + (size_t)p];
			ts.tok[(size_t)at + (size_t)p] = c;
			if (c == SA_CODE_SEP) {
				ts.mine[(size_t)(at / 16 + p / 16)] |= (uint16_t)(1u << (p & 15));
				ts.any[(size_t)(any_at + p / 16)] |= (uint16_t)(1u << (p & 15));
			}
		}
	}
	return true;
}

static const char *const TOO_LARGE = "packed range too large for one launch; split it into smaller ranges";

bool sa_plan_host(const SaPlanInputs &in, int64_t start, int64_t count, int world, bool share_host, SaHostPlan &plan)
{
	plan = SaHostPlan();
	const int32_t num = in.num;
	const int64_t all_pairs = (int64_t)num * (num - 1) / 2;
	if (num < 2 || !in.meta || start < 0 || count <= 0 || start > all_pairs - count || world < 0 || world > 1024) {
		sa_set_error("plan: bad range [%lld,+%lld) of %lld pairs or world %d", (long long)start, (long long)count,
			     (long long)all_pairs, world);
		return false;
	}
	const int64_t end = start + count;
	std::vector<std::vector<int32_t>> jl((size_t)SA_PLAN_NCLASSES), tp((size_t)SA_PLAN_NCLASSES);
	std::vector<int64_t> cpairs((size_t)SA_PLAN_NCLASSES, 0), ccells((size_t)SA_PLAN_NCLASSES, 0);
	std::vector<std::vector<std::pair<int32_t, int32_t>>> rows_of((size_t)SA_PLAN_NCLASSES);
	std::vector<int64_t> lenpre((size_t)num + 1, 0);
	for (int32_t k = 0; k < num; k++)
		lenpre[(size_t)k + 1] = lenpre[(size_t)k] + in.meta[k].len;
	{
		const int64_t want_tiles = (int64_t)in.persistent_wgs * 6;
		const int64_t mine = world > 1 ? count / world : count;
		int32_t chunk = SA_SYS_CHUNK;
		while (chunk > 8 && mine / (4 * chunk) < want_tiles)
			chunk >>= 1;
		if (in.env_chunk)
			chunk = in.env_chunk;
		plan.chunk = chunk;
		const int64_t want_pk = (int64_t)in.persistent_wgs * 5 / 8;
		int32_t cpk = SA_SYS_CHUNK;
		while (cpk > 4 && mine / ((int64_t)2 * SA_PK_WPB * 8 * cpk) < want_pk)
			cpk >>= 1;
		if (in.env_chunk)
			cpk = in.env_chunk;
		cpk = std::min(cpk, in.pk_chunk_cap);
		plan.chunk_pk = cpk;
		constexpr int TWO_SIZES_BELOW = 16, SMALL_TILE_DIV = 4, SMALL_PAIRS_FRAC = 5;
		const int64_t slots = (int64_t)in.persistent_wgs / 8;
		if (!in.env_chunk && mine / ((int64_t)2 * SA_PK_WPB * 8 * cpk) < (int64_t)TWO_SIZES_BELOW * slots) {
			int32_t big = SA_SYS_CHUNK;
			while (big > 16 && 2 * mine / ((int64_t)2 * SA_PK_WPB * 8 * big) < 5 * slots)
				big >>= 1;
			big = std::min(std::max(big, cpk), in.pk_chunk_cap);
			if (big >= 16) {
				plan.chunk_pk = big;
				plan.chunk_pk_small = std::max(4, big / SMALL_TILE_DIV);
				const int64_t jlo = sa_column_of(start), jhi = sa_column_of(end - 1) + 1;
				int64_t lo = jlo, hi = jhi;
				while (lo < hi) {
					const int64_t mid = (lo + hi) / 2;
					if (mid * (mid - 1) / 2 - start >= count / SMALL_PAIRS_FRAC)
						hi = mid;
					else
						lo = mid + 1;
				}
				plan.j_small = (int32_t)lo;
			}
		}
	}
	const int32_t j0 = sa_column_of(start), j1 = sa_column_of(end - 1);
	for (int32_t j = j0; j <= j1; j++) {
		const int64_t tri = (int64_t)j * (j - 1) / 2;
		const int64_t ia = std::max<int64_t>(0, start - tri), ib = std::min<int64_t>(j, end - tri);
		if (ib <= ia)
			continue;
		const int32_t n = in.meta[j].len;
		const int k8 = (n + 7) / 8, k16 = (n + 15) / 16;
		if (k8 <= in.pk_kmax || (k16 >= SA_PK_K16_MIN && k16 <= in.pk16_kmax)) {
			const size_t pc = (size_t)(k8 <= in.pk_kmax ? SA_PK_CLASS0 + k8 : SA_PK16_CLASS0 + k16) + (j < plan.j_small ? SA_PK_SMALL : 0);
			jl[pc].push_back(j);
			rows_of[pc].emplace_back((int32_t)ia, (int32_t)ib);
			cpairs[pc] += ib - ia;
			ccells[pc] += (int64_t)n * (lenpre[(size_t)ib] - lenpre[(size_t)ia]);
			continue;
		}
		const int cls = in.sys_ok ? sa_systolic_class_for(n) : -1;
		if (cls < 0) {
			if (!plan.generic.empty() && plan.generic.back().first + plan.generic.back().second == tri + ia)
				plan.generic.back().second += ib - ia;
			else
				plan.generic.emplace_back(tri + ia, ib - ia);
			continue;
		}
		const int rows = cls == SA_SYS_CLASS_LONG ? SA_SYS_WPB(64, true) * std::min(plan.chunk, 16)
							   : SA_SYS_WPB(SA_SYS_CLASSES[cls].G, false) * (64 / SA_SYS_CLASSES[cls].G) * plan.chunk;
		if (tp[(size_t)cls].empty())
			tp[(size_t)cls].push_back(0);
		const int64_t tiles = (ib - ia + rows - 1) / rows;
		if ((int64_t)tp[(size_t)cls].back() + tiles > INT32_MAX) {
			sa_set_error("%s", TOO_LARGE);
			return false;
		}
		jl[(size_t)cls].push_back(j);
		tp[(size_t)cls].push_back(tp[(size_t)cls].back() + (int32_t)tiles);
		cpairs[(size_t)cls] += ib - ia;
		ccells[(size_t)cls] += (int64_t)n * (lenpre[(size_t)ib] - lenpre[(size_t)ia]);
	}
	std::vector<int32_t> nparts((size_t)SA_PLAN_NCLASSES, 0);
	std::vector<std::vector<int32_t>> part_rows((size_t)SA_PLAN_NCLASSES);
	for (int cls = SA_PK_CLASS0; cls < SA_PLAN_NCLASSES; cls++) {
		const auto &rw = rows_of[(size_t)cls];
		if (rw.empty())
			continue;
		const SaPkCls pc = sa_pk_decode(cls);
		const int64_t rows = (int64_t)sa_pk_wpb(in.method, pc.g, pc.k) * (64 / pc.g) * (pc.small ? plan.chunk_pk_small : plan.chunk_pk);
		tp[(size_t)cls].push_back(0);
		std::vector<std::pair<int32_t, int32_t>> parts;
		for (size_t c = 0; c < rw.size(); c += 2) {
			const auto &a = rw[c], &b = rw[c + 1 < rw.size() ? c + 1 : c];
			const int64_t span = std::max(a.second, b.second) - std::min(a.first, b.first);
			const int64_t tiles = span / rows;
			if ((int64_t)tp[(size_t)cls].back() + tiles + (int64_t)parts.size() + 1 > ((int64_t)1 << SA_PK_UTILE_BITS)) {
				sa_set_error("%s", TOO_LARGE);
				return false;
			}
			tp[(size_t)cls].push_back(tp[(size_t)cls].back() + (int32_t)tiles);
			if (span % rows)
				parts.emplace_back((int32_t)(span % rows), (int32_t)(c / 2));
		}
		std::stable_sort(parts.begin(), parts.end(), [](const auto &x, const auto &y) { return x.first > y.first; });
		for (const auto &pt : parts) {
			tp[(size_t)cls].push_back(pt.second);
			part_rows[(size_t)cls].push_back(pt.first);
		}
		nparts[(size_t)cls] = (int32_t)parts.size();
	}
	for (int cls = 0; cls < SA_PLAN_NCLASSES; cls++) {
		if (jl[(size_t)cls].empty())
			continue;
		SaHostClass cl;
		cl.cls = cls;
		cl.ncols = (int32_t)jl[(size_t)cls].size();
		cl.npart = nparts[(size_t)cls];
		cl.ntiles = cl.npart ? tp[(size_t)cls][tp[(size_t)cls].size() - 1 - (size_t)cl.npart] + cl.npart : tp[(size_t)cls].back();
		cl.pairs = cpairs[(size_t)cls];
		cl.cells = ccells[(size_t)cls];
		cl.part_rows = std::move(part_rows[(size_t)cls]);
		cl.chunk = cls >= SA_PK_CLASS0 ? (sa_pk_decode(cls).small ? plan.chunk_pk_small : plan.chunk_pk) : 0;
		if (cls >= SA_PK_CLASS0 && cl.ntiles > (1 << SA_PK_UTILE_BITS)) {
			sa_set_error("%s", TOO_LARGE);
			return false;
		}
		cl.jlist = std::move(jl[(size_t)cls]);
		cl.tprefix = std::move(tp[(size_t)cls]);
		plan.classes.push_back(std::move(cl));
	}
	std::stable_sort(plan.classes.begin(), plan.classes.end(),
			 [](const SaHostClass &x, const SaHostClass &y) { return x.cells > y.cells; });
	plan.start = start;
	plan.count = count;
	plan.world = world;
	plan.share_host = share_host;
	if (world >= 1) {
		std::vector<int64_t> load((size_t)world, 0), fill((size_t)world, 0);
		struct Geo {
			int32_t owner;
			int32_t j[2], ia[2], ib[2], i_begin, i_count;
			bool dup, own;
			SaArrKey key;
			int64_t doff;
		};
		std::vector<Geo> geo;
		for (size_t ci = 0; ci < plan.classes.size(); ci++) {
			auto &cl = plan.classes[ci];
			const int cls = cl.cls;
			const bool is_pk = cls >= SA_PK_CLASS0;
			const int pk_g = is_pk ? sa_pk_decode(cls).g : 8;
			const int G = is_pk ? pk_g : cls == SA_SYS_CLASS_LONG ? 64 : SA_SYS_CLASSES[cls].G;
			const int K = is_pk ? sa_pk_decode(cls).k : cls == SA_SYS_CLASS_LONG ? 16 : SA_SYS_CLASSES[cls].K;
			const int64_t weight = (int64_t)(K + 6) * (G / 8);
			const auto &J = cl.jlist;
			const auto &T = cl.tprefix;
			std::vector<Geo> tiles((size_t)cl.ntiles);
			if (is_pk) {
				SaArrKey lv[SA_PK_SORT_LEVELS];
				sa_pk_arranged_keys(in, pk_g, K, cl.chunk, share_host, lv);
				const int32_t lvrows[SA_PK_SORT_LEVELS] = { lv[0].block, lv[1].block, lv[2].block, lv[3].block };
				const int32_t rows = sa_pk_wpb(in.method, pk_g, K) * (64 / pk_g) * cl.chunk;
				const auto &rw = rows_of[(size_t)cls];
				const int32_t npairs = (cl.ncols + 1) / 2, nfull = T[(size_t)npairs];
				for (int32_t t = 0; t < cl.ntiles; t++) {
					int32_t lo;
					if (t < nfull)
						lo = (int32_t)(std::upper_bound(T.begin(), T.begin() + npairs + 1, t) - T.begin()) - 1;
					else
						lo = T[(size_t)(npairs + 1 + (t - nfull))];
					const size_t c0 = (size_t)2 * (size_t)lo, c1 = c0 + 1 < rw.size() ? c0 + 1 : c0;
					Geo &g = tiles[(size_t)t];
					g.dup = c1 == c0;
					g.j[0] = J[c0], g.j[1] = J[c1];
					g.ia[0] = rw[c0].first, g.ib[0] = rw[c0].second;
					g.ia[1] = rw[c1].first, g.ib[1] = rw[c1].second;
					const int32_t ra = std::min(g.ia[0], g.ia[1]), rb = std::max(g.ib[0], g.ib[1]);
					const int32_t chunk = t < nfull ? t - T[(size_t)lo] : T[(size_t)lo + 1] - T[(size_t)lo];
					g.i_begin = ra + chunk * rows;
					g.i_count = std::min(rows, rb - g.i_begin);
					const int l = sa_pk_pick_level(lvrows, ra, rb, g.i_begin, rows);
					g.key = l >= 0 ? lv[l] : SaArrKey{};
					g.own = l >= 0 && lv[l].block == g.i_count;
				}
			} else {
				const int rows = cls == SA_SYS_CLASS_LONG ? SA_SYS_WPB(64, true) * std::min(plan.chunk, 16)
									   : SA_SYS_WPB(G, false) * (64 / G) * plan.chunk;
				for (int32_t k = 0; k < cl.ncols; k++) {
					const int32_t j = J[(size_t)k];
					const int64_t tri = (int64_t)j * (j - 1) / 2;
					const int32_t ia = (int32_t)std::max<int64_t>(0, start - tri), ib = (int32_t)std::min<int64_t>(j, end - tri);
					for (int32_t t = T[(size_t)k]; t < T[(size_t)k + 1]; t++) {
						Geo &g = tiles[(size_t)t];
						g.dup = true;
						g.j[0] = g.j[1] = j;
						g.ia[0] = g.ia[1] = ia, g.ib[0] = g.ib[1] = ib;
						g.i_begin = ia + (t - T[(size_t)k]) * rows;
						g.i_count = std::min(rows, ib - g.i_begin);
						g.key = SaArrKey{};
						g.own = false;
					}
				}
			}
			std::vector<std::vector<int32_t>> mine((size_t)world);
			cl.doff.assign((size_t)cl.ntiles, 0);
			cl.rank_pairs.assign((size_t)world, 0);
			cl.rank_cells.assign((size_t)world, 0);
			cl.owner.assign((size_t)cl.ntiles, 0);
			for (int32_t t = 0; t < cl.ntiles; t++) {
				Geo &g = tiles[(size_t)t];
				const int64_t res = lenpre[(size_t)(g.i_begin + g.i_count)] - lenpre[(size_t)g.i_begin] + g.i_count;
				int r = 0;
				for (int q = 1; q < world; q++)
					if (load[(size_t)q] < load[(size_t)r])
						r = q;
				load[(size_t)r] += res * weight;
				g.owner = r;
				cl.owner[(size_t)t] = (int16_t)r;
				g.doff = fill[(size_t)r];
				cl.doff[(size_t)t] = g.doff;
				fill[(size_t)r] += (int64_t)(g.dup ? 1 : 2) * SA_SHARE_PAD(g.i_count);
				mine[(size_t)r].push_back(t);
				for (int h = 0; h < (g.dup ? 1 : 2); h++) {
					const int64_t lo_i = std::max(g.ia[h], g.i_begin), hi_i = std::min(g.ib[h], g.i_begin + g.i_count);
					if (hi_i > lo_i) {
						cl.rank_pairs[(size_t)r] += hi_i - lo_i;
						cl.rank_cells[(size_t)r] += (int64_t)in.meta[g.j[h]].len * (lenpre[(size_t)hi_i] - lenpre[(size_t)lo_i]);
					}
				}
				geo.push_back(g);
			}
			cl.rank_first.assign((size_t)world + 1, 0);
			for (int r = 0; r < world; r++) {
				cl.tlist.insert(cl.tlist.end(), mine[(size_t)r].begin(), mine[(size_t)r].end());
				cl.rank_first[(size_t)r + 1] = (int32_t)cl.tlist.size();
			}
		}
		plan.generic_share.assign((size_t)world, {});
		for (const auto &run : plan.generic) {
			const int64_t per = (run.second + world - 1) / world;
			for (int r = 0; r < world; r++) {
				const int64_t lo_p = std::min(run.second, (int64_t)r * per), hi_p = std::min(run.second, lo_p + per);
				if (hi_p <= lo_p)
					continue;
				plan.generic_share[(size_t)r].push_back({ run.first + lo_p, hi_p - lo_p, fill[(size_t)r] });
				fill[(size_t)r] += SA_SHARE_PAD(hi_p - lo_p);
			}
		}
		plan.share_elems = std::max<int64_t>(8, *std::max_element(fill.begin(), fill.end()));
		for (const Geo &g : geo)
			for (int h = 0; h < (g.dup ? 1 : 2); h++) {
				SaHostSeg sg{};
				sg.src = (int64_t)g.owner * plan.share_elems + g.doff + (int64_t)h * SA_SHARE_PAD(g.i_count);
				sg.dst = (int64_t)g.j[h] * (g.j[h] - 1) / 2 - start;
				sg.map_kind = g.key.block ? (g.own ? 2 : 1) : 0;
				sg.key = g.key;
				sg.count = g.i_count;
				sg.pos0 = g.i_begin;
				sg.ia = g.ia[h];
				sg.ib = g.ib[h];
				sg.flags = g.own ? 1 : 0;
				plan.segs.push_back(sg);
			}
		for (int r = 0; r < world; r++)
			for (const auto &gs : plan.generic_share[(size_t)r])
				for (int64_t o = 0; o < gs.count; o += 8192) {
					SaHostSeg sg{};
					sg.src = (int64_t)r * plan.share_elems + gs.doff + o;
					sg.dst = gs.start + o - start;
					sg.map_kind = 0;
					sg.count = (int32_t)std::min<int64_t>(8192, gs.count - o);
					sg.pos0 = 0;
					sg.ia = 0;
					sg.ib = sg.count;
					plan.segs.push_back(sg);
				}
		if (plan.segs.size() > (size_t)INT32_MAX) {
			sa_set_error("%s", TOO_LARGE);
			return false;
		}
	}
	const int nranks = std::max(world, 1);
	std::vector<int> order;
	for (size_t ci = 0; ci < plan.classes.size(); ci++)
		if (plan.classes[ci].cls >= SA_PK_CLASS0)
			order.push_back((int)ci);
	std::sort(order.begin(), order.end(), [&](int x, int y) { return plan.classes[(size_t)x].cls > plan.classes[(size_t)y].cls; });
	std::stable_partition(order.begin(), order.end(), [&](int x) { return !sa_pk_decode(plan.classes[(size_t)x].cls).small; });
	for (int ci : order) {
		const auto &cl = plan.classes[(size_t)ci];
		const int g = sa_pk_decode(cl.cls).g;
		const int k = sa_pk_decode(cl.cls).k;
		const int klo = sa_pk_bundle_klo(g, k);
		const int f16 = g == 8 || k <= in.pk16_f16_kmax ? 1 : 0;
		SaHostBundle *b = nullptr;
		for (auto &x : plan.bundles)
			if (x.g == g && x.klo == klo && x.f16 == f16)
				b = &x;
		if (!b) {
			plan.bundles.emplace_back();
			b = &plan.bundles.back();
			b->g = g, b->klo = klo, b->f16 = f16, b->kmax = k;
		}
		b->kmax = std::max(b->kmax, k);
		b->cls.push_back(ci);
	}
	for (auto &b : plan.bundles) {
		b.args.resize(b.cls.size());
		for (size_t x = 0; x < b.cls.size(); x++) {
			const auto &cl = plan.classes[(size_t)b.cls[x]];
			const int k = sa_pk_decode(cl.cls).k;
			SaHostPkArgs &a = b.args[x];
			sa_pk_arranged_keys(in, b.g, k, cl.chunk, share_host, a.lv);
			a.cls_index = b.cls[x];
			a.chunk = cl.chunk;
			a.ncols = cl.ncols;
			a.npart = cl.npart;
			a.k = k;
			a.delta = sa_pk_delta(in, b.g, k);
			a.pk_base = sa_pk_base(in, b.g, k);
		}
		auto &ul = b.ulist;
		b.ufirst.assign((size_t)nranks + 1, 0);
		b.nlocal.assign((size_t)nranks, 0);
		b.pairs.assign((size_t)nranks, 0);
		b.cells.assign((size_t)nranks, 0);
		b.tok_lean.assign((size_t)nranks, 0);
		b.tok_legacy.assign((size_t)nranks, 0);
		struct Part {
			int64_t work;
			uint32_t code, pair;
		};
		std::vector<Part> parts;
		for (int r = 0; r < nranks; r++) {
			parts.clear();
			for (size_t x = 0; x < b.cls.size(); x++) {
				const auto &cl = plan.classes[(size_t)b.cls[x]];
				const int32_t nfull = cl.ntiles - cl.npart;
				const auto &T = cl.tprefix;
				const int32_t npairs = (cl.ncols + 1) / 2;
				const bool small = sa_pk_decode(cl.cls).small;
				const int64_t full_rows = (int64_t)sa_pk_wpb(in.method, b.g, sa_pk_decode(cl.cls).k) * (64 / b.g) * cl.chunk;
				const auto &rw = rows_of[(size_t)cl.cls];
				const int32_t lvrows[SA_PK_SORT_LEVELS] = { b.args[x].lv[0].block, b.args[x].lv[1].block, b.args[x].lv[2].block,
									    b.args[x].lv[3].block };
				int32_t pair_of_full = 0;
				for (int32_t t = 0; t < cl.ntiles; t++) {
					uint32_t pair;
					if (t < nfull) {
						while (pair_of_full + 1 < npairs && T[(size_t)pair_of_full + 1] <= t)
							pair_of_full++;
						pair = (uint32_t)pair_of_full;
					} else {
						pair = (uint32_t)T[(size_t)(npairs + 1 + (t - nfull))];
					}
					if (world >= 1 && cl.owner[(size_t)t] != r)
						continue;
					{
						const size_t c0 = (size_t)2 * pair, c1 = c0 + 1 < rw.size() ? c0 + 1 : c0;
						const int32_t ra = std::min(rw[c0].first, rw[c1].first), rb = std::max(rw[c0].second, rw[c1].second);
						const int32_t chunk = t < nfull ? t - T[(size_t)pair] : T[(size_t)pair + 1] - T[(size_t)pair];
						const int32_t i_begin = ra + chunk * (int32_t)full_rows;
						const bool lean = !in.no_tokens && sa_pk_pick_level(lvrows, ra, rb, i_begin, (int32_t)full_rows) >= 0;
						(lean ? b.tok_lean : b.tok_legacy)[(size_t)r]++;
					}
					const uint32_t code = ((uint32_t)x << SA_PK_UTILE_BITS) | (uint32_t)t;
					if (t < nfull && !small) {
						ul.push_back(code);
						ul.push_back(pair);
					} else
						parts.push_back({ (t < nfull ? full_rows : (int64_t)cl.part_rows[(size_t)(t - nfull)]) * (b.args[x].k + 4), code, pair });
				}
				b.pairs[(size_t)r] += world >= 1 ? cl.rank_pairs[(size_t)r] : cl.pairs;
				b.cells[(size_t)r] += world >= 1 ? cl.rank_cells[(size_t)r] : cl.cells;
			}
			std::stable_sort(parts.begin(), parts.end(), [](const Part &p, const Part &q) { return p.work > q.work; });
			for (const Part &pt : parts) {
				ul.push_back(pt.code);
				ul.push_back(pt.pair);
			}
			b.ufirst[(size_t)r + 1] = (int64_t)ul.size();
			const int64_t n = (b.ufirst[(size_t)r + 1] - b.ufirst[(size_t)r]) / 2;
			if (n > INT32_MAX) {
				sa_set_error("%s", TOO_LARGE);
				return false;
			}
			b.nlocal[(size_t)r] = (int32_t)n;
		}
	}
	return true;
}

extern "C" int64_t sa_pairs_cells(const struct sa_meta *meta, int32_t num, int64_t start, int64_t count)
{
	return sa_guard("sa_pairs_cells", (int64_t)-1, [&]() -> int64_t {
		if (!meta || num < 2)
			return -1;
		SaPairPlan plan(meta, num);
		if (start < 0 || count < 0 || start > plan.pairs - count)
			return -1;
		return plan.cells_before(start + count) - plan.cells_before(start);
	});
}

extern "C" int sa_pairs_partition(const struct sa_meta *meta, int32_t num, int parts, int64_t *bounds)
{
	return sa_guard("sa_pairs_partition", 1, [&] {
		if (!meta || num < 2 || parts < 1 || !bounds) {
			sa_set_error("sa_pairs_partition: bad arguments");
			return 1;
		}
		SaPairPlan plan(meta, num);
		const int64_t total = plan.cell_prefix[(size_t)num];
		bounds[0] = 0;
		for (int k = 1; k < parts; k++) {
			const int64_t target = (int64_t)((__int128)total * k / parts);
			int64_t lo = bounds[k - 1], hi = plan.pairs;
			while (lo < hi) {
				const int64_t mid = lo + (hi - lo) / 2;
				if (plan.cells_before(mid) >= target)
					hi = mid;
				else
					lo = mid + 1;
			}
			bounds[k] = lo;
		}
		bounds[parts] = plan.pairs;
		return 0;
	});
}
```

### sequencealigner_amd/csrc/sa_plan.h

```cpp
#ifndef SA_PLAN_H
#define SA_PLAN_H

#include <cstdint>
#include <string>
#include <utility>
#include <vector>

#include "sa_shapes.h"

int32_t sa_column_of(int64_t p);
inline int64_t sa_tri(int64_t j) { return j * (j - 1) / 2; }

struct SaPairPlan {
	int32_t num = 0;
	int64_t pairs = 0;
	const sa_meta *meta = nullptr;
	std::vector<int64_t> len_prefix;
	std::vector<int64_t> cell_prefix;
	SaPairPlan(const sa_meta *m, int32_t n);
	int64_t cells_before(int64_t p) const;
};

struct SaArrKey {
	int ng = 0, ch = 0;
	int32_t block = 0;
	bool operator==(const SaArrKey &o) const { return ng == o.ng && ch == o.ch && block == o.block; }
};

inline int sa_pk_live(int32_t min_len, int g) { return 1 + (g - 1) / ((min_len > 1 ? min_len : 1) + 1); }

struct SaPlanInputs {
	int32_t num = 0;
	const sa_meta *meta = nullptr;
	int32_t min_len = 1;
	int method = 0;
	int32_t gap_ext = 0;
	bool sys_ok = false;
	int pk_kmax = 0, pk16_kmax = 0, pk16_f16_kmax = 0, pk_chunk_cap = SA_SYS_CHUNK;
	int32_t pk_q = 0, pk_floor = 0;
	int64_t pk_gain = 0, pk_slack = 0;
	int persistent_wgs = 256 * 32;
	int env_chunk = 0;
	bool no_sort = false;
	bool no_tokens = false;
};

struct SaKernelLimits {
	bool sys_ok = false;
	int32_t sys_pconst = 0, sys_q = 0;
	int64_t sys_gain = 0, sys_slack = 0;
	int pk_kmax = 0, pk16_kmax = 0, pk16_f16_kmax = 0, pk_chunk_cap = SA_SYS_CHUNK;
	int32_t pk_pconst = 0, pk_q = 0, pk_floor = 0;
	int64_t pk_gain = 0, pk_slack = 0, pk_extra = 0;
};
SaKernelLimits sa_kernel_limits(const sa_scoring &sc, int32_t max_len, int32_t min_len, bool force_generic, bool no_pk, bool no_pk16);

int32_t sa_pk_delta(const SaPlanInputs &in, int g, int k);
int32_t sa_pk_base(const SaPlanInputs &in, int g, int k);

struct SaPkCls {
	bool small;
	int g, k;
};
SaPkCls sa_pk_decode(int cls);
int sa_systolic_class_for(int32_t n);

bool sa_arranged_exists(int32_t num, const SaArrKey &key);
int sa_pk_arranged_keys(const SaPlanInputs &in, int pk_g, int pk_k, int32_t chunk_pk, bool host_out, SaArrKey (&lv)[SA_PK_SORT_LEVELS]);
void sa_arrange_rows(const sa_meta *meta, int32_t num, const SaArrKey &key, std::vector<int32_t> &rowmap);

struct SaTokenStreams {
	int32_t streams = 0;
	std::vector<uint16_t> tok, mine, any;
	std::vector<int32_t> tok_off;
};
inline int32_t sa_token_blocks(int32_t smax, int g) { return ((smax + g - 1 + 15) >> 4) + 2; }
bool sa_build_tokens(const uint8_t *codes, const int32_t *off, int32_t num, const SaArrKey &key, SaTokenStreams &ts);

struct SaHostClass {
	int cls = 0;
	int32_t ncols = 0, ntiles = 0;
	int32_t npart = 0;
	int32_t chunk = 0;
	int64_t pairs = 0, cells = 0;
	std::vector<int32_t> jlist, tprefix;
	std::vector<int32_t> part_rows;
	std::vector<int32_t> tlist;
	std::vector<int64_t> doff;
	std::vector<int16_t> owner;
	std::vector<int32_t> rank_first;
	std::vector<int64_t> rank_pairs, rank_cells;
};

struct SaHostSeg {
	int64_t src, dst;
	int32_t count, pos0, ia, ib, flags;
	int map_kind;
	SaArrKey key;
};

struct SaHostPkArgs {
	int cls_index = 0;
	int32_t ncols = 0, npart = 0, k = 0, delta = 0, pk_base = 0, chunk = 0;
	SaArrKey lv[SA_PK_SORT_LEVELS];
};

struct SaHostBundle {
	int g = 8, klo = 1, f16 = 1, kmax = 1;
	std::vector<int> cls;
	std::vector<SaHostPkArgs> args;
	std::vector<uint32_t> ulist;
	std::vector<int64_t> ufirst;
	std::vector<int32_t> nlocal;
	std::vector<int64_t> pairs, cells;
	std::vector<int64_t> tok_lean, tok_legacy;
};

struct SaGenericShare {
	int64_t start, count, doff;
};

struct SaHostPlan {
	int64_t start = -1, count = -1;
	int32_t chunk = SA_SYS_CHUNK;
	int32_t chunk_pk = SA_SYS_CHUNK;
	int32_t chunk_pk_small = 0;
	int32_t j_small = 0;
	std::vector<SaHostClass> classes;
	std::vector<std::pair<int64_t, int64_t>> generic;
	int world = 0;
	bool share_host = false;
	int64_t share_elems = 0;
	std::vector<SaHostSeg> segs;
	std::vector<SaHostBundle> bundles;
	std::vector<std::vector<SaGenericShare>> generic_share;
};

bool sa_plan_host(const SaPlanInputs &in, int64_t start, int64_t count, int world, bool share_host, SaHostPlan &plan);

#endif
```

### sequencealigner_amd/csrc/sa_systolic_pk.inc

```
#include "sa_internal.h"
#include <atomic>
#include <type_traits>
#if !defined(SA_PK_G) || (SA_PK_G != 8 && SA_PK_G != 16)
#error "define SA_PK_G (8 or 16) before including sa_systolic_pk.inc"
#endif
#if SA_PK_G == 16 && !defined(SA_PK16_PART)
#error "define SA_PK16_PART (0: K = 13..44, 1: K = 45..64) before including sa_systolic_pk.inc with SA_PK_G 16"
#endif

#define SA_PK_STORE(nt, v, p)                          \
	do {                                           \
		if (nt) {                              \
			asm volatile("");  \
			__builtin_nontemporal_store((v), (p)); \
		} else                                 \
			*(p) = (v);                    \
	} while (0)

#ifndef SA_PK_OPAQUE_TOKEN
#define SA_PK_OPAQUE_TOKEN 1
#endif
#ifndef SA_PK_PAIRED_ADDS
#define SA_PK_PAIRED_ADDS 1
#endif
#ifndef SA_PK_CHAINED_MAX3
#define SA_PK_CHAINED_MAX3 1
#endif
#ifndef SA_PK_QUIET_BLOCKS
#define SA_PK_QUIET_BLOCKS 0
#endif

namespace {

extern __shared__ __attribute__((aligned(256))) uint8_t sa_pk_lds[];

constexpr int CH = SA_SYS_CHUNK;
typedef unsigned short u16x2 __attribute__((ext_vector_type(2)));
typedef uint32_t u32x4 __attribute__((ext_vector_type(4)));

__device__ __forceinline__ uint32_t pkmax(uint32_t a, uint32_t b)
{
	return __builtin_bit_cast(uint32_t, __builtin_elementwise_max(__builtin_bit_cast(u16x2, a), __builtin_bit_cast(u16x2, b)));
}
__device__ __forceinline__ uint32_t pksubsat(uint32_t a, uint32_t b)
{
	return __builtin_bit_cast(uint32_t, __builtin_elementwise_sub_sat(__builtin_bit_cast(u16x2, a), __builtin_bit_cast(u16x2, b)));
}
template <bool F16> __device__ __forceinline__ uint32_t pkmax3(uint32_t a, uint32_t b, uint32_t c)
{
	if (F16) {
		uint32_t d;
		asm("v_pk_maximum3_f16 %0, %1, %2, %3" : "=v"(d) : "v"(a), "v"(b), "v"(c));
		return d;
	}
	return pkmax(pkmax(a, b), c);
}
#if SA_PK_CHAINED_MAX3
template <int N> __device__ __forceinline__ void pkmax3_chain(uint32_t *V, const uint32_t *d, uint32_t left)
{
	static_assert(N >= 1 && N <= 8, "one statement holds up to eight links");
#define SA_LK0 "v_pk_maximum3_f16 %[v0], %[d0], %[v0], %[l]"
#define SA_LK(i, p) "\n\tv_pk_maximum3_f16 %[v" #i "], %[d" #i "], %[v" #i "], %[v" #p "]"
#define SA_VO(i) [v##i] "+v"(V[i])
#define SA_DI(i) [d##i] "v"(d[i])
	if constexpr (N == 1)
		asm(SA_LK0 : SA_VO(0) : SA_DI(0), [l] "v"(left));
	else if constexpr (N == 2)
		asm(SA_LK0 SA_LK(1, 0) : SA_VO(0), SA_VO(1) : SA_DI(0), SA_DI(1), [l] "v"(left));
	else if constexpr (N == 3)
		asm(SA_LK0 SA_LK(1, 0) SA_LK(2, 1) : SA_VO(0), SA_VO(1), SA_VO(2) : SA_DI(0), SA_DI(1), SA_DI(2), [l] "v"(left));
	else if constexpr (N == 4)
		asm(SA_LK0 SA_LK(1, 0) SA_LK(2, 1) SA_LK(3, 2)
		    : SA_VO(0), SA_VO(1), SA_VO(2), SA_VO(3)
		    : SA_DI(0), SA_DI(1), SA_DI(2), SA_DI(3), [l] "v"(left));
	else if constexpr (N == 5)
		asm(SA_LK0 SA_LK(1, 0) SA_LK(2, 1) SA_LK(3, 2) SA_LK(4, 3)
		    : SA_VO(0), SA_VO(1), SA_VO(2), SA_VO(3), SA_VO(4)
		    : SA_DI(0), SA_DI(1), SA_DI(2), SA_DI(3), SA_DI(4), [l] "v"(left));
	else if constexpr (N == 6)
		asm(SA_LK0 SA_LK(1, 0) SA_LK(2, 1) SA_LK(3, 2) SA_LK(4, 3) SA_LK(5, 4)
		    : SA_VO(0), SA_VO(1), SA_VO(2), SA_VO(3), SA_VO(4), SA_VO(5)
		    : SA_DI(0), SA_DI(1), SA_DI(2), SA_DI(3), SA_DI(4), SA_DI(5), [l] "v"(left));
	else if constexpr (N == 7)
		asm(SA_LK0 SA_LK(1, 0) SA_LK(2, 1) SA_LK(3, 2) SA_LK(4, 3) SA_LK(5, 4) SA_LK(6, 5)
		    : SA_VO(0), SA_VO(1), SA_VO(2), SA_VO(3), SA_VO(4), SA_VO(5), SA_VO(6)
		    : SA_DI(0), SA_DI(1), SA_DI(2), SA_DI(3), SA_DI(4), SA_DI(5), SA_DI(6), [l] "v"(left));
	else
		asm(SA_LK0 SA_LK(1, 0) SA_LK(2, 1) SA_LK(3, 2) SA_LK(4, 3) SA_LK(5, 4) SA_LK(6, 5) SA_LK(7, 6)
		    : SA_VO(0), SA_VO(1), SA_VO(2), SA_VO(3), SA_VO(4), SA_VO(5), SA_VO(6), SA_VO(7)
		    : SA_DI(0), SA_DI(1), SA_DI(2), SA_DI(3), SA_DI(4), SA_DI(5), SA_DI(6), SA_DI(7), [l] "v"(left));
#undef SA_LK0
#undef SA_LK
#undef SA_VO
#undef SA_DI
}
template <int K, int Q0 = 0> __device__ __forceinline__ void pkmax3_chain_all(uint32_t (&V)[K], const uint32_t (&d)[K], uint32_t left)
{
	if constexpr (Q0 < K) {
		constexpr int N = K - Q0 < 8 ? K - Q0 : 8;
		pkmax3_chain<N>(&V[Q0], &d[Q0], Q0 ? V[Q0 ? Q0 - 1 : 0] : left);
		pkmax3_chain_all<K, Q0 + N>(V, d, left);
	}
}
#endif
__device__ __forceinline__ void pkadd2(uint32_t lo, uint32_t hi, uint32_t plo, uint32_t phi, uint32_t &dlo, uint32_t &dhi)
{
	const uint64_t x = ((uint64_t)hi << 32) | lo, p = ((uint64_t)phi << 32) | plo;
	uint64_t d;
	asm("v_lshl_add_u64 %0, %1, 0, %2" : "=v"(d) : "v"(x), "v"(p));
	dlo = (uint32_t)d;
	dhi = (uint32_t)(d >> 32);
}
__device__ __forceinline__ uint32_t pk2(uint32_t v) { return (v & 0xffffu) | (v << 16); }
__device__ __forceinline__ uint32_t comp(const uint4 &w, int k) { return k == 0 ? w.x : k == 1 ? w.y : k == 2 ? w.z : w.w; }

template <int G> __device__ __forceinline__ uint32_t shift_in(uint32_t lead, uint32_t src)
{
	if (G == 8)
		return (uint32_t)__builtin_amdgcn_update_dpp((int)lead, (int)src, 0x112, 0xf, 0xf, false);
	return (uint32_t)__builtin_amdgcn_update_dpp((int)lead, (int)src, 0x111, 0xf, 0xf, false);
}

template <typename T> __device__ __forceinline__ T *uniform_ptr(T *p)
{
	const uint64_t v = reinterpret_cast<uint64_t>(p);
	const uint32_t lo = __builtin_amdgcn_readfirstlane((uint32_t)v), hi = __builtin_amdgcn_readfirstlane((uint32_t)(v >> 32));
	typedef __attribute__((address_space(1))) T *global_ptr;
	return (T *)reinterpret_cast<global_ptr>(((uint64_t)hi << 32) | lo);
}

__device__ __forceinline__ int32_t uload(const int32_t *p) { return __builtin_amdgcn_readfirstlane(*p); }

template <int METHOD, int G, int K, bool F16>
__device__ __forceinline__ void pk_tile(const SaSysArgs &A, const int32_t t_raw, const int32_t ntiles)
{
	static_assert(G == 8 || G == 16, "packed kernels: 8- or 16-lane groups");
	constexpr int NG = 64 / G, WPB = sa_pk_wpb(METHOD, G, K), NGW = NG * WPB;
	constexpr int W = G * K;
	constexpr int PARTS = (K + 3) / 4;
	constexpr int NSLOT = G;
	constexpr int COPIES = 16 / G;
	constexpr int PARTSTRIDE = COPIES * NSLOT * 16;
	static_assert(PARTSTRIDE == 256, "a part spans all 64 banks");
	constexpr int ROWSTRIDE = PARTS * PARTSTRIDE;
	constexpr int PROF_BYTES = SA_CODE_ROWS * ROWSTRIDE;
	constexpr int TSHIFT = (SA_CODE_ROWS - 1) * ROWSTRIDE < 65536 ? 0 : 8;
	constexpr uint32_t TUNIT = (uint32_t)ROWSTRIDE >> TSHIFT;
	static_assert((SA_CODE_ROWS - 1) * TUNIT < 65536, "the token of a profile row must fit u16");
	uint8_t *const s_prof = sa_pk_lds + sa_pk_lds_fixed(G, WPB);
	static_assert(PROF_BYTES + sa_pk_lds_fixed(G, WPB) == sa_pk_lds_bytes(METHOD, G, K), "host and kernel agree on the LDS of a class");
	constexpr int OUT_HALFS = 2 * NG * CH;
	static_assert(WPB * OUT_HALFS * 2 >= SA_SUB_DIM * SA_SUB_DIM, "the staged matrix must fit the score storage");
	int16_t *const s_out_all = reinterpret_cast<int16_t *>(sa_pk_lds);
	constexpr int RING = 64;
	constexpr int GSTRIDE = 2 * RING + 16;
	uint16_t *const s_ring_all = reinterpret_cast<uint16_t *>(sa_pk_lds + WPB * OUT_HALFS * 2);
	static_assert(WPB * OUT_HALFS * 2 + WPB * NG * GSTRIDE * 2 == sa_pk_lds_fixed(G, WPB), "LDS carve");
	static_assert(sa_pk_lds_fixed(G, WPB) % 256 == 0, "the profile starts on a 256-byte boundary: a part spans all 64 banks");

	int lane_id = threadIdx.x;
	asm volatile("" : "+v"(lane_id));
	const int lane = lane_id & 63;
	const int wv = __builtin_amdgcn_readfirstlane(lane_id >> 6);
	int16_t *s_out = s_out_all + wv * OUT_HALFS;
	uint16_t *s_ring = s_ring_all + wv * (NG * GSTRIDE);
	const int lig = G == 8 ? (lane & 15) >> 1 : lane & 15;
	const int grp = G == 8 ? (lane >> 4) * 2 + (lane & 1) : lane >> 4;
	const int copy = G == 8 ? lane & 1 : 0;
	const bool leader = lig == 0;

	const bool active = t_raw < ntiles;
	const int32_t t = active ? t_raw : ntiles - 1;
	const int32_t npairs = (A.ncols + 1) >> 1;
	const int32_t nfull = uload(A.tprefix + npairs);
	const int32_t lo = A.tile_pair;
	const int32_t jh[2] = { uload(A.jlist + 2 * lo), uload(A.jlist + (2 * lo + 1 < A.ncols ? 2 * lo + 1 : 2 * lo)) };
	const bool dup = 2 * lo + 1 >= A.ncols;
	int64_t tri[2];
	int32_t ia[2], ib[2], offj[2], nh[2], pad[2];
#pragma unroll
	for (int h = 0; h < 2; h++) {
		const int32_t j = jh[h];
		tri[h] = (int64_t)j * (j - 1) / 2;
		const int64_t a = A.start > tri[h] ? A.start - tri[h] : 0;
		const int64_t b = A.end - tri[h] < j ? A.end - tri[h] : j;
		ia[h] = (int32_t)a;
		ib[h] = (int32_t)(b > a ? b : a);
		offj[h] = uload(A.off + j);
		nh[h] = uload(A.off + j + 1) - offj[h] - 1;
		pad[h] = W - nh[h];
	}
	const int32_t ra = ia[0] < ia[1] ? ia[0] : ia[1], rb = ib[0] > ib[1] ? ib[0] : ib[1];
	const int32_t chunk = t < nfull ? t - uload(A.tprefix + lo) : uload(A.tprefix + lo + 1) - uload(A.tprefix + lo);
	const int32_t ch_full = A.chunk;
	const int32_t i_begin = ra + chunk * (NGW * ch_full);
	const int32_t i_count = rb - i_begin < NGW * ch_full ? rb - i_begin : NGW * ch_full;
	const int32_t ch = (i_count + NGW - 1) / NGW;
	const int gw = wv * NG;
	const uint8_t *rcodes = A.codes;
	const int32_t *roff = A.off, *rowmap = nullptr, *posmap = nullptr;
	int32_t sort_rows = 0;
	const uint16_t *tk_tok = nullptr, *tk_mine = nullptr, *tk_any = nullptr;
	const int32_t *tk_off = nullptr;
	{
		const int32_t lvrows[SA_PK_SORT_LEVELS] = { uload(&A.lvp[0].rows), uload(&A.lvp[1].rows), uload(&A.lvp[2].rows),
							    uload(&A.lvp[3].rows) };
		static_assert(SA_PK_SORT_LEVELS == 4, "lvrows lists four levels");
		const int l = sa_pk_pick_level(lvrows, ra, rb, i_begin, NGW * ch_full);
		if (l >= 0) {
			const SaArranged &L = A.lvp[l];
			rcodes = uniform_ptr(L.codes);
			roff = uniform_ptr(L.off);
			rowmap = uniform_ptr(L.rowmap);
			posmap = uniform_ptr(L.posmap);
			tk_tok = uniform_ptr(L.tok);
			tk_off = uniform_ptr(L.tok_off);
			tk_mine = uniform_ptr(L.mine);
			tk_any = uniform_ptr(L.any);
			sort_rows = lvrows[0];
#pragma unroll
			for (int k = 1; k < SA_PK_SORT_LEVELS; k++)
				if (l == k)
					sort_rows = lvrows[k];
		}
	}
	const bool sorted = sort_rows > 0;

	int8_t *const sub = reinterpret_cast<int8_t *>(s_out_all);
	for (int k = lane_id; k < SA_SUB_DIM * SA_SUB_DIM; k += 64 * WPB)
		sub[k] = A.sub8[k];
	uint8_t *const s_cols = reinterpret_cast<uint8_t *>(s_ring_all);
	static_assert(2 * W <= WPB * NG * GSTRIDE * 2, "the staged columns fit the ring storage");
	for (int k = lane_id; k < 2 * W; k += 64 * WPB) {
		const int h = k >= W, c0 = k - h * W - pad[h];
		s_cols[k] = c0 >= 0 ? A.codes[offj[h] + c0] : (uint8_t)0xff;
	}
	__syncthreads();

	{
		constexpr int BUILDERS = NGW / COPIES;
		constexpr int ROWS_EACH = (SA_CODE_ROWS + BUILDERS - 1) / BUILDERS;
		const int a_lo = ((gw + grp) / COPIES) * ROWS_EACH;
		uint8_t *const slot = s_prof + copy * (NSLOT * 16) + lig * 16;
#pragma unroll 4
		for (int q = 0; q < K; q++) {
			int bq[2];
#pragma unroll
			for (int h = 0; h < 2; h++) {
				const int c = (int)s_cols[h * W + lig * K + q];
				bq[h] = c == 0xff ? -1 : c;
			}
#pragma unroll
			for (int r = 0; r < ROWS_EACH; r++) {
				const int a = a_lo + r;
				if (a >= SA_CODE_ROWS)
					break;
				uint32_t v = 0;
#pragma unroll
				for (int h = 0; h < 2; h++) {
					int e = 0;
					if (a < SA_SUB_DIM && bq[h] >= 0) {
						e = (int)sub[a * SA_SUB_DIM + bq[h]] + A.pconst;
						if (METHOD == SA_METHOD_GA && pad[h] != 0 && lig * K + q == pad[h])
							e -= A.q;
					}
					v |= (uint32_t)(e & 0xffff) << (16 * h);
				}
				*reinterpret_cast<uint32_t *>(slot + a * ROWSTRIDE + (q >> 2) * PARTSTRIDE + (q & 3) * 4) = v;
			}
		}
	}

	const int32_t ib_g = i_begin + (gw + grp) * ch;
	int32_t cnt_g = i_count - (gw + grp) * ch;
	cnt_g = cnt_g < 0 ? 0 : cnt_g > ch ? ch : cnt_g;
	const int32_t sbeg = roff[ib_g < A.num ? ib_g : 0];
	const int32_t slen = cnt_g > 0 ? roff[ib_g + cnt_g] - sbeg : 0;
	int32_t smax = 0;
#pragma unroll
	for (int g = 0; g < NG; g++) {
		int32_t c = i_count - (gw + g) * ch;
		c = c < 0 ? 0 : c > ch ? ch : c;
		const int32_t b = i_begin + (gw + g) * ch;
		const int32_t l = c > 0 ? roff[b + c] - roff[b] : 0;
		smax = l > smax ? l : smax;
	}
	const int32_t steps = smax + G - 1;
	const int32_t nblk = (steps + 15) >> 4;
	const int32_t last = slen > 0 ? slen - 1 : 0;
	const int r16 = lane & 15;
	constexpr int TPL = G == 8 ? 2 : 1;
	typedef typename std::conditional<G == 8, uint32_t, uint16_t>::type tok_t;
	auto fpos = [&](int u) -> int { return G == 8 ? (r16 & ~1) + u : r16; };
	uint32_t bw_a = (uint32_t)(sbeg + fpos(0)), bw_b = (uint32_t)(sbeg + last), bw_c = (uint32_t)slen;
	auto load_block = [&](int32_t blk, int u) -> int {
		const uint32_t at = bw_a + (uint32_t)u + (uint32_t)(blk << 4);
		return (int)rcodes[at < bw_b ? at : bw_b];
	};
	constexpr uint32_t SEPWORD = (uint32_t)SA_CODE_SEP * TUNIT;
	constexpr uint32_t NOPWORD = (uint32_t)SA_CODE_NOP * TUNIT;
	auto block_word = [&](int32_t blk, int raw, int u) -> uint32_t {
		const int32_t pos = (blk << 4) + fpos(u);
		return pos < (int32_t)bw_c ? (uint32_t)raw * TUNIT : NOPWORD;
	};
	uint16_t *ring = s_ring + grp * GSTRIDE;
	auto ring_write = [&](int32_t blk, uint32_t word, int u) {
		const int i0 = ((blk << 4) + fpos(u)) & (RING - 1);
		ring[i0] = (uint16_t)word;
		ring[i0 + RING] = (uint16_t)word;
	};
	auto fold16 = [&](unsigned long long m) -> uint32_t {
		m |= m >> 32;
		m |= m >> 16;
		return (uint32_t)m & 0xffffu;
	};
	auto block_events = [&](const uint32_t (&w)[TPL], uint32_t &mine) -> uint32_t {
		if (G == 16) {
			const unsigned long long m = __ballot(w[0] == SEPWORD);
			mine = (uint32_t)(m >> (lane & 48)) & 0xffffu;
			return fold16(m);
		}
		uint32_t any = 0;
		mine = 0;
#pragma unroll
		for (int u = 0; u < TPL; u++) {
			const unsigned long long m = __ballot(w[u] == SEPWORD);
			const uint32_t f = fold16(m);
			any |= ((f | (f >> 1)) & 0x5555u) << u;
			mine |= ((uint32_t)(m >> ((lane & 48) + (lane & 1))) & 0x5555u) << u;
		}
		return any;
	};

	const int32_t lean = __builtin_amdgcn_readfirstlane(tk_tok != nullptr ? 1 : 0);
	const uint16_t *tk_any_w = nullptr;
	if (lean) {
		const int32_t s0 = i_begin / ch_full + gw;
		const uint32_t o_w = (uint32_t)uload(tk_off + s0), o_g = (uint32_t)tk_off[s0 + grp];
		bw_a = 2u * o_g + (G == 8 ? 4u * (uint32_t)(r16 >> 1) : 2u * (uint32_t)r16);
		bw_b = o_g >> 3;
		tk_any_w = tk_any + (o_w >> 4) / NG;
		bw_c = (uint32_t)(WPB * OUT_HALFS * 2 + 2 * (wv * (NG * GSTRIDE) + grp * GSTRIDE + fpos(0)));
	}
	auto lean_load = [&](int32_t blk) -> uint32_t {
		const uint8_t *const b = reinterpret_cast<const uint8_t *>(tk_tok) + (size_t)(uint32_t)(blk << 5);
		asm volatile("" : "+v"(bw_a));
		return *reinterpret_cast<const tok_t *>(b + bw_a);
	};
	auto lean_mine = [&](int32_t blk) -> uint32_t {
		const uint8_t *const b = reinterpret_cast<const uint8_t *>(tk_mine) + (size_t)(uint32_t)(blk << 1);
		asm volatile("" : "+v"(bw_b));
		return *reinterpret_cast<const uint16_t *>(b + bw_b);
	};
	auto lean_any = [&](int32_t blk) -> uint32_t { return (uint32_t)tk_any_w[blk]; };
	auto lean_any_s = [&](uint32_t v) -> uint32_t { return (uint32_t)__builtin_amdgcn_readfirstlane((int)v); };
	auto lean_ring = [&](int32_t blk, uint32_t raw) {
		const uint32_t w = __umul24(raw, TUNIT);
		tok_t *const at = reinterpret_cast<tok_t *>(sa_pk_lds + bw_c + ((blk & 3) << 5));
		at[0] = (tok_t)w;
		at[RING * 2 / sizeof(tok_t)] = (tok_t)w;
	};

	const uint32_t base2 = pk2((uint32_t)A.pk_base);
	const uint32_t delta2 = pk2((uint32_t)A.delta);
	const uint32_t q2 = pk2((uint32_t)-A.q);
	const uint32_t cmask2 = (pad[0] == 0 ? 0xffffu : 0u) | (pad[1] == 0 ? 0xffff0000u : 0u);
	uint32_t V[K], Y[K];
	uint32_t vl[2];
	constexpr bool PAIRED = SA_PK_PAIRED_ADDS && METHOD == SA_METHOD_NW;
	uint32_t xout = 0;
	uint32_t vbase;
	uint32_t fl = 0;
	uint32_t flead = 0, xlead = 0;
	uint32_t best = 0, carry = 0;
	const uint32_t e2 = pk2((uint32_t)-A.gap_e);
	const uint32_t gqs2 = pk2((uint32_t)(A.gap_e - A.gap_o));
	int32_t frame = 0;
	int nsep = 0;
	const uint32_t inj0 = METHOD == SA_METHOD_NW ? base2 : base2 - 2 * q2;
	vl[0] = vl[1] = vbase = inj0;
	if (METHOD == SA_METHOD_SW) {
		const uint32_t o2 = pk2((uint32_t)-A.gap_o);
		const uint32_t top = base2 - o2 - (uint32_t)lig * e2;
		vl[0] = base2 - o2 - e2;
		vl[1] = top;
		xout = top - e2;
		xlead = base2 - o2;
		flead = base2;
		fl = base2 - (uint32_t)(lig + 1) * e2;
		best = base2 - (uint32_t)lig * e2;
#pragma unroll
		for (int q = 0; q < K; q++)
			V[q] = top, Y[q] = top;
	} else if (METHOD == SA_METHOD_NW) {
#pragma unroll
		for (int q = 0; q < K; q++)
			V[q] = base2, Y[q] = 0;
	} else {
		xout = base2 - q2;
#pragma unroll
		for (int q = 0; q < K; q++)
			V[q] = inj0, Y[q] = inj0;
	}

	__syncthreads();
	for (int k = lane; k < NG * GSTRIDE; k += 64)
		s_ring[k] = (uint16_t)NOPWORD;
	__syncthreads();
	uint32_t ev_lo = METHOD == SA_METHOD_GA ? 0x8000u : 0u, ev_hi;
	uint32_t gm, gmask;
	if (lean) {
		lean_ring(0, lean_load(0));
		gmask = lean_mine(0);
		ev_hi = lean_any_s(lean_any(0));
		gm = (gmask << 2) | (METHOD == SA_METHOD_GA ? 2u : 0u);
	} else {
		uint32_t w0[TPL];
#pragma unroll
		for (int u = 0; u < TPL; u++) {
			w0[u] = block_word(0, load_block(0, u), u);
			ring_write(0, w0[u], u);
		}
		ev_hi = block_events(w0, gmask);
		gm = (gmask << 2) | (METHOD == SA_METHOD_GA ? 2u : 0u);
	}
	int raw_next[TPL];
	uint32_t mask_pf = 0, any_next = 0;
	uint32_t &mask_next = TPL == 2 ? reinterpret_cast<uint32_t &>(raw_next[TPL - 1]) : mask_pf;
	if (lean) {
		raw_next[0] = (int)lean_load(1);
		mask_next = lean_mine(1);
		any_next = lean_any(1);
	} else {
#pragma unroll
		for (int u = 0; u < TPL; u++)
			raw_next[u] = load_block(1, u);
	}
	const uint8_t *const lane_prof = s_prof + copy * (NSLOT * 16) + lig * 16;
	auto ring_base = [&](int32_t blk) -> const uint16_t * { return ring + (((blk << 4) - lig) & (RING - 1)); };
	auto prof_row = [&](uint32_t word, uint4 (&P)[PARTS]) {
		const uint8_t *row = lane_prof + (word << TSHIFT);
#pragma unroll
		for (int p = 0; p < PARTS; p++)
			P[p] = *reinterpret_cast<const uint4 *>(row + p * PARTSTRIDE);
	};
	const uint16_t *rb0 = ring_base(0);
	uint32_t tk_cur = rb0[0], tk_nxt = rb0[1];
	uint4 P[PARTS];
	prof_row(tk_cur, P);

	auto do_block = [&](const int32_t blk) __attribute__((always_inline)) {
		if (A.rotate_prio) {
			switch (((uint32_t)A.rotate_prio + (uint32_t)blk) & 3u) {
			case 0: __builtin_amdgcn_s_setprio(0); break;
			case 1: __builtin_amdgcn_s_setprio(1); break;
			case 2: __builtin_amdgcn_s_setprio(2); break;
			default: __builtin_amdgcn_s_setprio(3); break;
			}
		}
		const uint32_t ev_in =
			METHOD == SA_METHOD_GA ? (ev_hi | (ev_hi << 1) | (ev_hi << 2) | (ev_lo >> 15) | (ev_lo >> 14)) : ev_hi;
		const uint32_t ev = ((ev_lo >> (16 - (G - 1))) | (ev_hi << (G - 1)) | ev_in) & 0xffffu;
		uint32_t gm_next, evn;
		__builtin_amdgcn_s_waitcnt(0x0f70);
		if (lean) {
			lean_ring(blk + 1, (uint32_t)raw_next[0]);
			gm_next = (mask_next << 2) | (gm >> 16);
			evn = lean_any_s(any_next);
			asm volatile("" ::: "memory");
			raw_next[0] = (int)lean_load(blk + 2);
			mask_next = lean_mine(blk + 2);
			any_next = lean_any(blk + 2);
		} else {
			uint32_t gmask_next;
			uint32_t wn[TPL];
#pragma unroll
			for (int u = 0; u < TPL; u++) {
				wn[u] = block_word(blk + 1, raw_next[u], u);
				ring_write(blk + 1, wn[u], u);
			}
			evn = block_events(wn, gmask_next);
			gm_next = (gmask_next << 2) | (gm >> 16);
#pragma unroll
			for (int u = 0; u < TPL; u++)
				raw_next[u] = load_block(blk + 2, u);
		}
		const uint16_t *rbase = ring_base(blk);

		auto step = [&](auto has_events, const int s) __attribute__((always_inline)) {
			uint32_t &vcur = vl[PAIRED ? 0 : s & 1];
			if (METHOD == SA_METHOD_SW)
				carry = pkmax(shift_in<G>(0u, carry), best);
			if (decltype(has_events)::value && __builtin_expect((ev >> s) & 1u, 0)) {
				asm volatile("" ::: "memory");
				if ((gm >> (s + 2)) & 1u) {
#pragma unroll
					for (int q = 0; q < K; q++) {
						V[q] = pksubsat(V[q], delta2);
						if (METHOD != SA_METHOD_NW)
							Y[q] = pksubsat(Y[q], delta2);
					}
					if (METHOD != SA_METHOD_NW)
						xout = pksubsat(xout, delta2);
					if (METHOD == SA_METHOD_SW) {
						fl = pksubsat(fl, delta2);
						best = pksubsat(best, delta2);
						carry = pksubsat(carry, delta2);
					}
					if (!leader) {
						vl[0] = pksubsat(vl[0], delta2);
						if (!PAIRED)
							vl[1] = pksubsat(vl[1], delta2);
					}
					frame++;
				}
				if (METHOD == SA_METHOD_GA && leader) {
					if ((gm >> (s + 2)) & 1u) {
						vl[(s + 1) & 1] = vbase;
						vcur = vbase + q2;
					} else if ((gm >> (s + 1)) & 1u) {
						vl[(s + 1) & 1] = vbase + (q2 & cmask2);
					} else if ((gm >> s) & 1u) {
						vcur = vbase;
					}
				}
				if (lig == G - 1 && tk_cur == SEPWORD) {
					const uint32_t v = METHOD == SA_METHOD_SW ? carry : V[K - 1];
					const int32_t rebase = (frame - nsep) * A.delta - A.pk_base +
							       (METHOD == SA_METHOD_SW ? ((blk << 4) + s - (G - 1)) * A.gap_e : 0);
					s_out[grp * CH + nsep] = (int16_t)((int32_t)(v & 0xffffu) + rebase);
					s_out[NG * CH + grp * CH + nsep] = (int16_t)((int32_t)(v >> 16) + rebase);
					nsep++;
				}
			}
			const uint32_t tk_far = rbase[s + 2];
			const uint32_t vprev = vl[PAIRED ? 0 : (s + 1) & 1];
			const uint8_t *const row_next = lane_prof + (tk_nxt << TSHIFT);
			auto reload = [&](int q_done) {
				if ((q_done & 3) == 3 || q_done == K - 1) {
					P[q_done >> 2] = *reinterpret_cast<const uint4 *>(row_next + (q_done >> 2) * PARTSTRIDE);
					if ((K & 3) != 0 && (q_done >> 2) == PARTS - 1)
						asm volatile("" ::"v"(P[PARTS - 1].y), "v"(P[PARTS - 1].z), "v"(P[PARTS - 1].w));
				}
			};
			uint32_t dnw[K];
			if (METHOD == SA_METHOD_NW) {
				if (PAIRED) {
#pragma unroll
					for (int q = 0; q + 1 < K; q += 2)
						pkadd2(q ? V[q - 1] : vprev, V[q], comp(P[q >> 2], q & 3), comp(P[q >> 2], (q & 3) + 1), dnw[q], dnw[q + 1]);
					if (K & 1)
						dnw[K - 1] = (K > 1 ? V[K > 1 ? K - 2 : 0] : vprev) + comp(P[(K - 1) >> 2], (K - 1) & 3);
				} else {
					dnw[0] = vprev + comp(P[0], 0);
#pragma unroll
					for (int q = 1; q < K; q++)
						dnw[q] = V[q - 1] + comp(P[q >> 2], q & 3);
				}
#pragma unroll
				for (int p = 0; p < PARTS; p++)
					P[p] = *reinterpret_cast<const uint4 *>(row_next + p * PARTSTRIDE);
// ... 154 lines not shown
		do_block(blk2);
		if (blk2 + 1 < nblk)
			do_block(blk2 + 1);
	}
	if (A.stamps && threadIdx.x == 0) {
		A.stamps[3 * (size_t)A.nlocal + 3 * (size_t)A.stamp_u + 0] = ph1;
		A.stamps[3 * (size_t)A.nlocal + 3 * (size_t)A.stamp_u + 1] = __builtin_amdgcn_s_memtime();
		A.stamps[3 * (size_t)A.nlocal + 3 * (size_t)A.stamp_u + 2] = (unsigned long long)nblk * 16;
	}
	__syncthreads();

	if (A.dense_off) {
		const int64_t draw = A.dense_off[t];
		const int64_t dbase = (int64_t)(((uint64_t)(uint32_t)__builtin_amdgcn_readfirstlane((int32_t)(draw >> 32)) << 32) |
						(uint32_t)__builtin_amdgcn_readfirstlane((int32_t)draw));
		const int32_t cntp = SA_SHARE_PAD(i_count);
#pragma unroll
		for (int g = 0; g < NG; g++) {
			int32_t c = i_count - (gw + g) * ch;
			c = c < 0 ? 0 : c > ch ? ch : c;
			if (lane < c && active) {
				const int32_t is = i_begin + (gw + g) * ch + lane;
				const int32_t m = roff[is + 1] - roff[is] - 1;
#pragma unroll
				for (int h = 0; h < 2; h++) {
					if (h == 1 && dup)
						continue;
					const int32_t raw = s_out[h * NG * CH + g * CH + lane];
					int32_t score;
					if (METHOD == SA_METHOD_NW)
						score = raw + (m + nh[h]) * A.gap_g;
					else if (METHOD == SA_METHOD_GA)
						score = raw - A.q + (m + nh[h]) * A.gap_e;
					else
						score = raw;
					const int64_t at = dbase + h * cntp + (is - i_begin);
					if (A.out16)
						reinterpret_cast<int16_t *>(A.out)[at] = (int16_t)score;
					else
						A.out[at] = score;
				}
			}
		}
		if (!A.host_out)
			return;
	}
	int32_t *const pout = A.dense_off ? A.host_out : A.out;
	const bool p16 = A.dense_off ? false : A.out16 != 0;
	const bool pnt = A.dense_off ? true : A.out_nt != 0;
	if (sorted && sort_rows == NGW * ch_full) {
		if (active) {
			constexpr int E = 4;
			const int32_t wrows = NG * ch_full;
			for (int32_t n = 0; n < wrows; n += 64 * E) {
				const int32_t r0 = n + E * lane;
				if (r0 >= wrows)
					continue;
				const int32_t i0 = i_begin + wv * wrows + r0;
				int32_t sc[2][E];
#pragma unroll
				for (int e = 0; e < E; e++) {
					const int32_t i = i0 + e;
					const int32_t p = posmap[i] - i_begin;
					const int32_t st = p / ch_full, k = p - st * ch_full;
					const int16_t *const so = s_out_all + (st / NG) * OUT_HALFS + (st % NG) * CH + k;
					const int32_t m = A.off[i + 1] - A.off[i] - 1;
#pragma unroll
					for (int h = 0; h < 2; h++) {
						const int32_t raw = so[h * NG * CH];
						if (METHOD == SA_METHOD_NW)
							sc[h][e] = raw + (m + nh[h]) * A.gap_g;
						else if (METHOD == SA_METHOD_GA)
							sc[h][e] = raw - A.q + (m + nh[h]) * A.gap_e;
						else
							sc[h][e] = raw;
					}
				}
#pragma unroll
				for (int h = 0; h < 2; h++) {
					if (h == 1 && dup)
						continue;
					const int64_t at = tri[h] + i0 - A.start;
					if (i0 >= ia[h] && i0 + E <= ib[h]) {
						typedef int32_t i32x4 __attribute__((ext_vector_type(4), aligned(4)));
						typedef int16_t i16x4 __attribute__((ext_vector_type(4), aligned(2)));
						if (p16) {
							i16x4 v = { (int16_t)sc[h][0], (int16_t)sc[h][1], (int16_t)sc[h][2], (int16_t)sc[h][3] };
							SA_PK_STORE(pnt, v, reinterpret_cast<i16x4 *>(reinterpret_cast<int16_t *>(pout) + at));
						} else {
							i32x4 v = { sc[h][0], sc[h][1], sc[h][2], sc[h][3] };
							SA_PK_STORE(pnt, v, reinterpret_cast<i32x4 *>(pout + at));
						}
						continue;
					}
#pragma unroll
					for (int e = 0; e < E; e++) {
						const int32_t i = i0 + e;
						if (i < ia[h] || i >= ib[h])
							continue;
						if (p16)
							SA_PK_STORE(pnt, (int16_t)sc[h][e], &reinterpret_cast<int16_t *>(pout)[at + e]);
						else
							SA_PK_STORE(pnt, sc[h][e], &pout[at + e]);
					}
				}
			}
		}
		return;
	}
#pragma unroll
	for (int g = 0; g < NG; g++) {
		int32_t c = i_count - (gw + g) * ch;
		c = c < 0 ? 0 : c > ch ? ch : c;
		if (lane < c && active) {
			const int32_t is = i_begin + (gw + g) * ch + lane;
			const int32_t i = sorted ? rowmap[is] : is;
			const int32_t m = roff[is + 1] - roff[is] - 1;
#pragma unroll
			for (int h = 0; h < 2; h++) {
				if (i < ia[h] || i >= ib[h] || (h == 1 && dup))
					continue;
				const int32_t raw = s_out[h * NG * CH + g * CH + lane];
				int32_t score;
				if (METHOD == SA_METHOD_NW)
					score = raw + (m + nh[h]) * A.gap_g;
				else if (METHOD == SA_METHOD_GA)
					score = raw - A.q + (m + nh[h]) * A.gap_e;
				else
					score = raw;
				if (p16)
					SA_PK_STORE(pnt, (int16_t)score, &reinterpret_cast<int16_t *>(pout)[tri[h] + i - A.start]);
				else
					SA_PK_STORE(pnt, score, &pout[tri[h] + i - A.start]);
			}
		}
	}
}

template <int METHOD, int G, int KLO, bool F16>
__global__ __launch_bounds__(64 * sa_pk_wpb(METHOD, G, KLO)) void sa_k_systolic_pk_bundle(SaSysArgs A0)
{
	__shared__ int32_t s_next;
	constexpr int KMAX = G == 8 ? SA_PK_KMAX : SA_PK16_KMAX;
	if (A0.stagger > 0) {
		if (threadIdx.x == 0)
			s_next = (int32_t)(__builtin_amdgcn_s_getreg((3 << 11) | 4) & 3u);
		__syncthreads();
		const int32_t n = __builtin_amdgcn_readfirstlane(s_next) * A0.stagger;
		for (int32_t k = 0; k < n; k++)
			__builtin_amdgcn_s_sleep(127);
		__syncthreads();
	}
	const uint32_t wave_slot = __builtin_amdgcn_s_getreg((3 << 11) | 4);
	for (;;) {
		if (threadIdx.x == 0)
			s_next = (int32_t)atomicAdd(A0.counter, 1u);
		__syncthreads();
		const int32_t u = __builtin_amdgcn_readfirstlane(s_next);
		__syncthreads();
		if (u >= A0.nlocal)
			break;
		const uint32_t ut = (uint32_t)__builtin_amdgcn_readfirstlane((int32_t)A0.ulist[2 * (size_t)u]);
		const int c = (int)(ut >> SA_PK_UTILE_BITS);
		const int32_t t = (int32_t)(ut & ((1u << SA_PK_UTILE_BITS) - 1u));
		const SaPkClassArgs &P = A0.pkc[c];
		SaSysArgs A = A0;
		A.tile_pair = __builtin_amdgcn_readfirstlane((int32_t)A0.ulist[2 * (size_t)u + 1]);
		A.jlist = uniform_ptr(P.jlist);
		A.tprefix = uniform_ptr(P.tprefix);
		A.dense_off = uniform_ptr(P.dense_off);
		A.ncols = __builtin_amdgcn_readfirstlane(P.ncols);
		A.npart = __builtin_amdgcn_readfirstlane(P.npart);
		A.delta = __builtin_amdgcn_readfirstlane(P.delta);
		A.pk_base = __builtin_amdgcn_readfirstlane(P.pk_base);
		A.rotate_prio = A0.rotate_prio ? (int32_t)(4u + (wave_slot & 3u)) : 0;
		A.chunk = __builtin_amdgcn_readfirstlane(P.chunk);
		A.lvp = P.lv;
		const int32_t ntiles = __builtin_amdgcn_readfirstlane(A.tprefix[(A.ncols + 1) >> 1]) + A.npart;
		const unsigned long long st0 = A0.stamps ? __builtin_amdgcn_s_memrealtime() : 0ull;
		const unsigned long long sc0 = A0.stamps ? __builtin_amdgcn_s_memtime() : 0ull;
		A.stamp_u = u;
		switch (__builtin_amdgcn_readfirstlane(P.k) - KLO) {
#define SA_BCASE(D)                                                  \
	case D:                                                      \
		if constexpr (KLO + D <= KMAX)                       \
			pk_tile<METHOD, G, KLO + D, F16>(A, t, ntiles); \
		break;
			SA_BCASE(0) SA_BCASE(1) SA_BCASE(2) SA_BCASE(3) SA_BCASE(4) SA_BCASE(5) SA_BCASE(6) SA_BCASE(7)
#undef SA_BCASE
		default:
			break;
		}
		if (A0.stamps && threadIdx.x == 0) {
			A0.stamps[3 * (size_t)u + 0] = st0;
			A0.stamps[3 * (size_t)u + 1] = __builtin_amdgcn_s_memrealtime();
			A0.stamps[3 * (size_t)u + 2] = sc0;
			A0.stamps[6 * (size_t)A0.nlocal + (size_t)u] = __builtin_amdgcn_s_memtime();
		}
	}
	if (threadIdx.x == 0) {
		__threadfence();
		if (atomicAdd(A0.counter + 1, 1u) == gridDim.x - 1) {
			atomicExch(A0.counter, 0u);
			atomicExch(A0.counter + 1, 0u);
		}
	}
}

template <int METHOD, int G, int KLO, bool F16>
hipError_t launch_bundle(const SaSysArgs &a, int wgs, unsigned lds_bytes, hipStream_t s)
{
	auto *kern = &sa_k_systolic_pk_bundle<METHOD, G, KLO, F16>;
	if (lds_bytes > 64 * 1024) {
		static std::atomic<unsigned long long> raised{ 0 };
		int dev = 0;
		(void)hipGetDevice(&dev);
		const unsigned long long bit = 1ull << (dev & 63);
		if (!(raised.load() & bit)) {
			(void)hipFuncSetAttribute(reinterpret_cast<const void *>(kern), hipFuncAttributeMaxDynamicSharedMemorySize,
						  sa_pk_lds_bytes(METHOD, G, KLO + SA_PK_BUNDLE - 1 < (G == 8 ? SA_PK_KMAX : SA_PK16_KMAX) ? KLO + SA_PK_BUNDLE - 1
														   : (G == 8 ? SA_PK_KMAX : SA_PK16_KMAX)));
			(void)hipGetLastError();
			raised.fetch_or(bit);
		}
	}
	static_assert(sa_pk_wpb(METHOD, G, KLO) == sa_pk_wpb(METHOD, G, KLO + SA_PK_BUNDLE - 1), "a bundle does not straddle the workgroup sizes");
	hipLaunchKernelGGL(kern, dim3(wgs), dim3(64 * sa_pk_wpb(METHOD, G, KLO)), lds_bytes, s, a);
	return hipGetLastError();
}

template <int METHOD> hipError_t launch_pk(int g, int klo, int f16, const SaSysArgs &a, int wgs, unsigned lds_bytes, hipStream_t s)
{
	if (g != SA_PK_G || !a.pkc || a.npkc < 1 || a.npkc > 2 * SA_PK_BUNDLE)
		return hipErrorInvalidValue;
#if SA_PK_G == 8
	if (!f16)
		return hipErrorInvalidValue;
	switch (klo) {
	case 1:
		return launch_bundle<METHOD, 8, 1, true>(a, wgs, lds_bytes, s);
	case 9:
		return launch_bundle<METHOD, 8, 9, true>(a, wgs, lds_bytes, s);
	case 17:
		return launch_bundle<METHOD, 8, 17, true>(a, wgs, lds_bytes, s);
	default:
		return hipErrorInvalidValue;
	}
#else
#define SA_B16(KLO_)                                                                        \
	case KLO_:                                                                          \
		return f16 ? launch_bundle<METHOD, 16, KLO_, true>(a, wgs, lds_bytes, s)    \
			   : launch_bundle<METHOD, 16, KLO_, false>(a, wgs, lds_bytes, s);
	switch (klo) {
#if SA_PK16_PART == 0
		SA_B16(13) SA_B16(21) SA_B16(29) SA_B16(37)
#else
		SA_B16(45)
	case 53:
		return f16 ? hipErrorInvalidValue : launch_bundle<METHOD, 16, 53, false>(a, wgs, lds_bytes, s);
	case 61:
		return f16 ? hipErrorInvalidValue : launch_bundle<METHOD, 16, 61, false>(a, wgs, lds_bytes, s);
#endif
	default:
		return hipErrorInvalidValue;
	}
#undef SA_B16
#endif
}

}

hipError_t SA_SYS_LAUNCH(int g, int klo, int f16, const SaSysArgs &a, int wgs, unsigned lds_bytes, hipStream_t s)
{
	return launch_pk<SA_SYS_METHOD>(g, klo, f16, a, wgs, lds_bytes, s);
}

hipError_t SA_SYS_WARM(void)
{
	hipFuncAttributes attr;
#if SA_PK_G == 8
	return hipFuncGetAttributes(&attr, reinterpret_cast<const void *>(&sa_k_systolic_pk_bundle<SA_SYS_METHOD, 8, 9, true>));
#else
#if SA_PK16_PART == 0
	return hipFuncGetAttributes(&attr, reinterpret_cast<const void *>(&sa_k_systolic_pk_bundle<SA_SYS_METHOD, 16, SA_PK_K16_MIN, true>));
#else
	return hipFuncGetAttributes(&attr, reinterpret_cast<const void *>(&sa_k_systolic_pk_bundle<SA_SYS_METHOD, 16, 45, false>));
#endif
#endif
}
```

Baseline: 4.013 billion pair-alignments/s.

## Group same-pair tiles into runs that reuse the staged LDS profile

The planner groups consecutive bundle work items that share a class and column pair into runs, bounded by a tail-aware cap. Each persistent workgroup fetches a whole run and skips the substitution and profile staging and build for tiles after the first. This is meant to cut repeated prologue work and block barriers. By default the run cap is one, so runs stay single tiles unless the env variable raises it. The change also adds an extra indirection load per fetch and prologue timing stamps.

```diff
diff --git a/include/seqalign_hip.h b/include/seqalign_hip.h
--- a/include/seqalign_hip.h
+++ b/include/seqalign_hip.h
@@ -65,6 +65,8 @@
 int sa_ctx_align_range(sa_ctx *ctx, int64_t start, int64_t count, int32_t *d_scores, void *stream);
 
 int sa_ctx_token_tiles(const sa_ctx *ctx, int64_t *lean, int64_t *legacy);
+
+int sa_ctx_run_tiles(const sa_ctx *ctx, int64_t *runs, int64_t *multi, int64_t *held);
 
 int sa_ctx_align_host(sa_ctx *ctx, int64_t start, int64_t count, struct sa_output out, double *phase_seconds);
 
diff --git a/sequencealigner_amd/binding.py b/sequencealigner_amd/binding.py
--- a/sequencealigner_amd/binding.py
+++ b/sequencealigner_amd/binding.py
@@ -45,7 +45,7 @@
 
 ABI_SYMBOLS = (
     "sa_hip_memory", "sa_hip_align", "sa_hip_filter", "sa_ctx_create", "sa_ctx_destroy", "sa_ctx_pairs", "sa_pairs_cells",
-    "sa_ctx_align_range", "sa_ctx_align_range16", "sa_ctx_token_tiles", "sa_ctx_scores_fit16", "sa_hip_widen16", "sa_ctx_expand_full", "sa_pairs_partition", "sa_ctx_timing", "sa_ctx_timing_read",
+    "sa_ctx_align_range", "sa_ctx_align_range16", "sa_ctx_token_tiles", "sa_ctx_run_tiles", "sa_ctx_scores_fit16", "sa_hip_widen16", "sa_ctx_expand_full", "sa_pairs_partition", "sa_ctx_timing", "sa_ctx_timing_read",
     "sa_matrix_load", "sa_matrix_count", "sa_matrix_name", "sa_matrix_is_nucleotide", "sa_method_parse",
     "sa_method_name", "sa_method_gap_kind", "sa_hip_device_count", "sa_hip_device_name", "sa_last_error",
     "sa_abi_version",
@@ -122,6 +122,8 @@
     lib.sa_ctx_align_range.restype = C.c_int
     lib.sa_ctx_token_tiles.argtypes = [C.c_void_p, C.POINTER(C.c_int64), C.POINTER(C.c_int64)]
     lib.sa_ctx_token_tiles.restype = C.c_int
+    lib.sa_ctx_run_tiles.argtypes = [C.c_void_p, C.POINTER(C.c_int64), C.POINTER(C.c_int64), C.POINTER(C.c_int64)]
+    lib.sa_ctx_run_tiles.restype = C.c_int
     lib.sa_ctx_align_range16.argtypes = [C.c_void_p, C.c_int64, C.c_int64, C.c_void_p, C.c_void_p]
     lib.sa_ctx_align_range16.restype = C.c_int
     lib.sa_ctx_scores_fit16.argtypes = [C.c_void_p]
@@ -943,6 +945,12 @@
             raise AlignError(_err())
         return int(lean.value), int(legacy.value)
 
+    def run_tiles(self) -> tuple[int, int, int]:
+        runs, multi, held = C.c_int64(0), C.c_int64(0), C.c_int64(0)
+        if self._lib.sa_ctx_run_tiles(self._h, C.byref(runs), C.byref(multi), C.byref(held)):
+            raise AlignError(_err())
+        return int(runs.value), int(multi.value), int(held.value)
+
     @property
     def scores_fit16(self) -> bool:
         return bool(self._lib.sa_ctx_scores_fit16(self._h))
diff --git a/sequencealigner_amd/csrc/sa_context.hip b/sequencealigner_amd/csrc/sa_context.hip
--- a/sequencealigner_amd/csrc/sa_context.hip
+++ b/sequencealigner_amd/csrc/sa_context.hip
@@ -129,6 +129,7 @@
 	in.env_chunk = ctx->env.chunk;
 	in.no_sort = ctx->env.no_sort;
 	in.no_tokens = ctx->env.no_tokens;
+	in.run_tiles = ctx->env.run_tiles;
 	return in;
 }
 
diff --git a/sequencealigner_amd/csrc/sa_ctx.h b/sequencealigner_amd/csrc/sa_ctx.h
--- a/sequencealigner_amd/csrc/sa_ctx.h
+++ b/sequencealigner_amd/csrc/sa_ctx.h
@@ -59,6 +59,7 @@
 	};
 	std::deque<Arranged> arranged;
 	int64_t tok_lean = 0, tok_legacy = 0;
+	int64_t run_count = 0, run_multi = 0, run_held = 0;
 	bool out_is_host = false;
 	struct Plan {
 		SaHostPlan h;
@@ -69,6 +70,7 @@
 		struct DevBundle {
 			SaPkClassArgs *d_args = nullptr;
 			uint32_t *d_ulist = nullptr;
+			int32_t *d_urun = nullptr;
 		};
 		std::vector<DevClass> dc;
 		std::vector<DevBundle> db;
diff --git a/sequencealigner_amd/csrc/sa_env.cpp b/sequencealigner_amd/csrc/sa_env.cpp
--- a/sequencealigner_amd/csrc/sa_env.cpp
+++ b/sequencealigner_amd/csrc/sa_env.cpp
@@ -22,6 +22,7 @@
 	e.no_tokens = flag("SA_HIP_NO_TOKENS");
 	e.chunk = number("SA_HIP_CHUNK", 0, 1, 32);
 	e.stagger = number("SA_HIP_STAGGER", 0, 0, 64);
+	e.run_tiles = number("SA_HIP_RUN_TILES", 0, 1, 64);
 	e.no_pin = flag("SA_HIP_NO_PIN");
 	e.no_direct = flag("SA_HIP_NO_DIRECT");
 	e.no_shells = flag("SA_HIP_NO_SHELLS");
diff --git a/sequencealigner_amd/csrc/sa_env.h b/sequencealigner_amd/csrc/sa_env.h
--- a/sequencealigner_amd/csrc/sa_env.h
+++ b/sequencealigner_amd/csrc/sa_env.h
@@ -9,6 +9,7 @@
 	bool no_tokens = false;
 	int chunk = 0;
 	int stagger = 0;
+	int run_tiles = 0;
 	bool no_pin = false;
 	bool no_direct = false;
 	bool no_shells = false;
diff --git a/sequencealigner_amd/csrc/sa_internal.h b/sequencealigner_amd/csrc/sa_internal.h
--- a/sequencealigner_amd/csrc/sa_internal.h
+++ b/sequencealigner_amd/csrc/sa_internal.h
@@ -64,6 +64,8 @@
 	const SaPkClassArgs *pkc;
 	const uint32_t *ulist;
 	int32_t tile_pair;
+	const int32_t *urun;
+	int32_t nruns;
 	int32_t npkc;
 	unsigned *counter;
 	int32_t rotate_prio;
diff --git a/sequencealigner_amd/csrc/sa_launch.hip b/sequencealigner_amd/csrc/sa_launch.hip
--- a/sequencealigner_amd/csrc/sa_launch.hip
+++ b/sequencealigner_amd/csrc/sa_launch.hip
@@ -17,6 +17,7 @@
 	for (auto &b : pl.db) {
 		(void)hipFree(b.d_args);
 		(void)hipFree(b.d_ulist);
+		(void)hipFree(b.d_urun);
 	}
 	pl.dc.clear();
 	pl.db.clear();
@@ -117,7 +118,7 @@
 			a.pk_base = ha.pk_base;
 			a.chunk = ha.chunk;
 		}
-		if (!upload(pl.db[bi].d_args, args) || !upload(pl.db[bi].d_ulist, b.ulist))
+		if (!upload(pl.db[bi].d_args, args) || !upload(pl.db[bi].d_ulist, b.ulist) || !upload(pl.db[bi].d_urun, b.urun))
 			return false;
 	}
 	return true;
@@ -225,6 +226,22 @@
 	}
 	fprintf(stderr, "[stamps] per tile: prologue %.0f clocks, main loop %.0f (%.0f steps, %.1f clocks per step), epilogue %.0f\n",
 		pro / (double)nstamp, loop / (double)nstamp, steps / (double)nstamp, loop / steps, epi / (double)nstamp);
+	double pb[3] = {}, ph[2] = {}, nb = 0, nh = 0;
+	for (size_t k = 0; k < nstamp; k++) {
+		const unsigned long long c0 = h[3 * k + 2], c1 = h[3 * nstamp + 3 * k], ca = h[7 * nstamp + 3 * k], cb = h[7 * nstamp + 3 * k + 1];
+		if (h[7 * nstamp + 3 * k + 2]) {
+			nh += 1;
+			ph[0] += (double)(cb - c0);
+			ph[1] += (double)(c1 - cb);
+		} else {
+			nb += 1;
+			pb[0] += (double)(ca - c0);
+			pb[1] += (double)(cb - ca);
+			pb[2] += (double)(c1 - cb);
+		}
+	}
+	fprintf(stderr, "[stamps] prologue: %.0f tiles built their profile: staging %.0f clocks, build %.0f, to the first step %.0f; %.0f held it: ring clear %.0f, to the first step %.0f\n",
+		nb, nb ? pb[0] / nb : 0.0, nb ? pb[1] / nb : 0.0, nb ? pb[2] / nb : 0.0, nh, nh ? ph[0] / nh : 0.0, nh ? ph[1] / nh : 0.0);
 	fprintf(stderr, "[stamps] %s: %zu tiles, makespan %.1f us, mean tile %.1f us = %.0f shader clocks (%.0f MHz), mean active workgroups %.0f; active per 5%% of the launch:",
 		name, nstamp, span / 100.0, busy / (double)nstamp / 100.0, clocks / (double)nstamp, clocks / busy * 100.0, busy / span);
 	for (int b = 0; b < BINS; b++)
@@ -254,6 +271,7 @@
 	unsigned lds = 0;
 	int wgs = 0;
 	int32_t ntiles = 0;
+	int32_t nfetch = 0;
 	int64_t pairs = 0, cells = 0;
 	size_t nstamp = 0, stamp_words = 0;
 	char name[96] = "";
@@ -299,12 +317,14 @@
 	a.ulist = pl.db[bi].d_ulist + b.ufirst[(size_t)rk];
 	a.npkc = (int32_t)b.cls.size();
 	a.nlocal = L.ntiles = b.nlocal[(size_t)rk];
+	a.urun = pl.db[bi].d_urun + b.rfirst[(size_t)rk];
+	a.nruns = L.nfetch = b.nruns[(size_t)rk];
 	a.counter = counters + 2 * (SA_PK_CLASS0 + (int)bi);
 	L.pairs = b.pairs[(size_t)rk];
 	L.cells = b.cells[(size_t)rk];
 	L.nstamp = (size_t)L.ntiles;
-	L.stamp_words = 7 * L.nstamp;
-	L.wgs = (int)std::min<int64_t>(ctx->persistent_wgs / 32 * (ctx->leave_room ? 3 : 4), L.ntiles);
+	L.stamp_words = 10 * L.nstamp;
+	L.wgs = (int)std::min<int64_t>(ctx->persistent_wgs / 32 * (ctx->leave_room ? 3 : 4), a.nruns);
 	int klo_seen = b.kmax;
 	for (int ci : b.cls)
 		klo_seen = std::min(klo_seen, sa_pk_decode(pl.h.classes[(size_t)ci].cls).k);
@@ -344,12 +364,12 @@
 	a.delta = (int32_t)(ctx->sys_gain * W + ctx->sys_slack);
 	a.counter = counters + 2 * cls;
 	a.chunk = is_long ? std::min(pl.h.chunk, 16) : pl.h.chunk;
-	L.ntiles = cl.ntiles;
+	L.ntiles = L.nfetch = cl.ntiles;
 	L.pairs = cl.pairs;
 	L.cells = cl.cells;
 	if (share) {
 		a.tlist = dc.d_tlist + cl.rank_first[(size_t)rank];
-		a.nlocal = L.ntiles = cl.rank_first[(size_t)rank + 1] - cl.rank_first[(size_t)rank];
+		a.nlocal = L.ntiles = L.nfetch = cl.rank_first[(size_t)rank + 1] - cl.rank_first[(size_t)rank];
 		a.dense_off = dc.d_doff;
 		L.pairs = cl.rank_pairs[(size_t)rank];
 		L.cells = cl.rank_cells[(size_t)rank];
@@ -378,7 +398,7 @@
 		SA_HIP_CHECK(hipMemset(d_stamps, 0, sizeof(unsigned long long) * std::max<size_t>(L.stamp_words, 1)), return false);
 		L.a.stamps = d_stamps;
 	}
-	ctx->prog_items.push_back({ L.a.counter, L.ntiles });
+	ctx->prog_items.push_back({ L.a.counter, L.nfetch });
 	hipEvent_t e0 = nullptr, e1 = nullptr;
 	if (!timed_begin(ctx, s, e0, e1))
 		return false;
@@ -466,11 +486,15 @@
 
 	ctx->prog_items.clear();
 	ctx->tok_lean = ctx->tok_legacy = 0;
+	ctx->run_count = ctx->run_multi = ctx->run_held = 0;
 	for (size_t bi = 0; bi < pl.h.bundles.size(); bi++) {
 		if (pl.h.bundles[bi].nlocal[(size_t)rk] <= 0)
 			continue;
 		ctx->tok_lean += pl.h.bundles[bi].tok_lean[(size_t)rk];
 		ctx->tok_legacy += pl.h.bundles[bi].tok_legacy[(size_t)rk];
+		ctx->run_count += pl.h.bundles[bi].nruns[(size_t)rk];
+		ctx->run_multi += pl.h.bundles[bi].run_multi[(size_t)rk];
+		ctx->run_held += pl.h.bundles[bi].held[(size_t)rk];
 		Launch L = pk_launch(ctx, pl, bi, rk, share, counters, common);
 		if (!run_launch(ctx, L, s))
 			return 1;
@@ -544,6 +568,20 @@
 	});
 }
 
+extern "C" int sa_ctx_run_tiles(const sa_ctx *ctx, int64_t *runs, int64_t *multi, int64_t *held)
+{
+	return sa_guard("sa_ctx_run_tiles", 1, [&] {
+		if (!ctx || !runs || !multi || !held) {
+			sa_set_error("sa_ctx_run_tiles: null argument");
+			return 1;
+		}
+		*runs = ctx->run_count;
+		*multi = ctx->run_multi;
+		*held = ctx->run_held;
+		return 0;
+	});
+}
+
 extern "C" int sa_ctx_align_range(sa_ctx *ctx, int64_t start, int64_t count, int32_t *d_scores, void *stream)
 {
 	return sa_guard("sa_ctx_align_range", 1, [&] { return sa_align_range_impl(ctx, start, count, d_scores, stream, false); });
diff --git a/sequencealigner_amd/csrc/sa_plan.cpp b/sequencealigner_amd/csrc/sa_plan.cpp
--- a/sequencealigner_amd/csrc/sa_plan.cpp
+++ b/sequencealigner_amd/csrc/sa_plan.cpp
@@ -217,6 +217,7 @@
 		plan.chunk_pk = cpk;
 		constexpr int TWO_SIZES_BELOW = 16, SMALL_TILE_DIV = 4, SMALL_PAIRS_FRAC = 5;
 		const int64_t slots = (int64_t)in.persistent_wgs / 8;
+		plan.run_tiles = in.run_tiles > 0 ? in.run_tiles : SA_RUN_TILES_DEFAULT;
 		if (!in.env_chunk && mine / ((int64_t)2 * SA_PK_WPB * 8 * cpk) < (int64_t)TWO_SIZES_BELOW * slots) {
 			int32_t big = SA_SYS_CHUNK;
 			while (big > 16 && 2 * mine / ((int64_t)2 * SA_PK_WPB * 8 * big) < 5 * slots)
@@ -523,6 +524,11 @@
 		b.cells.assign((size_t)nranks, 0);
 		b.tok_lean.assign((size_t)nranks, 0);
 		b.tok_legacy.assign((size_t)nranks, 0);
+		b.rfirst.assign((size_t)nranks + 1, 0);
+		b.nruns.assign((size_t)nranks, 0);
+		b.nlarge.assign((size_t)nranks, 0);
+		b.run_multi.assign((size_t)nranks, 0);
+		b.held.assign((size_t)nranks, 0);
 		struct Part {
 			int64_t work;
 			uint32_t code, pair;
@@ -570,6 +576,7 @@
 				b.pairs[(size_t)r] += world >= 1 ? cl.rank_pairs[(size_t)r] : cl.pairs;
 				b.cells[(size_t)r] += world >= 1 ? cl.rank_cells[(size_t)r] : cl.cells;
 			}
+			const int64_t nlarge = ((int64_t)ul.size() - b.ufirst[(size_t)r]) / 2;
 			std::stable_sort(parts.begin(), parts.end(), [](const Part &p, const Part &q) { return p.work > q.work; });
 			for (const Part &pt : parts) {
 				ul.push_back(pt.code);
@@ -582,6 +589,26 @@
 				return false;
 			}
 			b.nlocal[(size_t)r] = (int32_t)n;
+			const uint32_t *const mine_ul = ul.data() + b.ufirst[(size_t)r];
+			b.nlarge[(size_t)r] = (int32_t)nlarge;
+			int64_t grouped = nlarge;
+			while (grouped > 0 && sa_run_cap_at(grouped - 1, nlarge, in.persistent_wgs / 8, plan.run_tiles) == 1)
+				grouped--;
+			for (int64_t u = 0; u < n;) {
+				const int64_t most = sa_run_cap_at(u, nlarge, in.persistent_wgs / 8, plan.run_tiles);
+				int64_t v = u + 1;
+				while (v < grouped && v - u < most && (mine_ul[2 * v] >> SA_PK_UTILE_BITS) == (mine_ul[2 * u] >> SA_PK_UTILE_BITS) &&
+				       mine_ul[2 * v + 1] == mine_ul[2 * u + 1])
+					v++;
+				b.urun.push_back((int32_t)u);
+				b.nruns[(size_t)r]++;
+				if (v - u > 1)
+					b.run_multi[(size_t)r] += v - u;
+				b.held[(size_t)r] += v - u - 1;
+				u = v;
+			}
+			b.urun.push_back((int32_t)n);
+			b.rfirst[(size_t)r + 1] = (int64_t)b.urun.size();
 		}
 	}
 	return true;
diff --git a/sequencealigner_amd/csrc/sa_plan.h b/sequencealigner_amd/csrc/sa_plan.h
--- a/sequencealigner_amd/csrc/sa_plan.h
+++ b/sequencealigner_amd/csrc/sa_plan.h
@@ -43,7 +43,21 @@
 	int env_chunk = 0;
 	bool no_sort = false;
 	bool no_tokens = false;
+	int run_tiles = 0;
 };
+
+constexpr int SA_RUN_TILES_DEFAULT = 1;
+constexpr int SA_RUN_TAIL_WGS = 2, SA_RUN_TAIL_DIV = 8;
+inline int64_t sa_run_unit(int64_t large_full, int64_t resident_wgs)
+{
+	const int64_t a = SA_RUN_TAIL_WGS * resident_wgs, b = large_full / SA_RUN_TAIL_DIV;
+	return a < b ? a : b > 1 ? b : 1;
+}
+inline int64_t sa_run_cap_at(int64_t u, int64_t large_full, int64_t resident_wgs, int cap)
+{
+	const int64_t c = u < large_full ? (large_full - u) / sa_run_unit(large_full, resident_wgs) : 1;
+	return c < 1 ? 1 : c > cap ? cap : c;
+}
 
 struct SaKernelLimits {
 	bool sys_ok = false;
@@ -114,6 +128,10 @@
 	std::vector<int32_t> nlocal;
 	std::vector<int64_t> pairs, cells;
 	std::vector<int64_t> tok_lean, tok_legacy;
+	std::vector<int32_t> urun;
+	std::vector<int64_t> rfirst;
+	std::vector<int32_t> nruns, nlarge;
+	std::vector<int64_t> run_multi, held;
 };
 
 struct SaGenericShare {
@@ -126,6 +144,7 @@
 	int32_t chunk_pk = SA_SYS_CHUNK;
 	int32_t chunk_pk_small = 0;
 	int32_t j_small = 0;
+	int run_tiles = 1;
 	std::vector<SaHostClass> classes;
 	std::vector<std::pair<int64_t, int64_t>> generic;
 	int world = 0;
diff --git a/sequencealigner_amd/csrc/sa_systolic_pk.inc b/sequencealigner_amd/csrc/sa_systolic_pk.inc
--- a/sequencealigner_amd/csrc/sa_systolic_pk.inc
+++ b/sequencealigner_amd/csrc/sa_systolic_pk.inc
@@ -132,7 +132,7 @@
 __device__ __forceinline__ int32_t uload(const int32_t *p) { return __builtin_amdgcn_readfirstlane(*p); }
 
 template <int METHOD, int G, int K, bool F16>
-__device__ __forceinline__ void pk_tile(const SaSysArgs &A, const int32_t t_raw, const int32_t ntiles)
+__device__ __forceinline__ void pk_tile(const SaSysArgs &A, const int32_t t_raw, const int32_t ntiles, const int32_t held)
 {
 	static_assert(G == 8 || G == 16, "packed kernels: 8- or 16-lane groups");
 	constexpr int NG = 64 / G, WPB = sa_pk_wpb(METHOD, G, K), NGW = NG * WPB;
@@ -227,46 +227,50 @@
 	const bool sorted = sort_rows > 0;
 
 	int8_t *const sub = reinterpret_cast<int8_t *>(s_out_all);
-	for (int k = lane_id; k < SA_SUB_DIM * SA_SUB_DIM; k += 64 * WPB)
-		sub[k] = A.sub8[k];
-	uint8_t *const s_cols = reinterpret_cast<uint8_t *>(s_ring_all);
-	static_assert(2 * W <= WPB * NG * GSTRIDE * 2, "the staged columns fit the ring storage");
-	for (int k = lane_id; k < 2 * W; k += 64 * WPB) {
-		const int h = k >= W, c0 = k - h * W - pad[h];
-		s_cols[k] = c0 >= 0 ? A.codes[offj[h] + c0] : (uint8_t)0xff;
-	}
-	__syncthreads();
-
-	{
-		constexpr int BUILDERS = NGW / COPIES;
-		constexpr int ROWS_EACH = (SA_CODE_ROWS + BUILDERS - 1) / BUILDERS;
-		const int a_lo = ((gw + grp) / COPIES) * ROWS_EACH;
-		uint8_t *const slot = s_prof + copy * (NSLOT * 16) + lig * 16;
+	if (!held) {
+		for (int k = lane_id; k < SA_SUB_DIM * SA_SUB_DIM; k += 64 * WPB)
+			sub[k] = A.sub8[k];
+		uint8_t *const s_cols = reinterpret_cast<uint8_t *>(s_ring_all);
+		static_assert(2 * W <= WPB * NG * GSTRIDE * 2, "the staged columns fit the ring storage");
+		for (int k = lane_id; k < 2 * W; k += 64 * WPB) {
+			const int h = k >= W, c0 = k - h * W - pad[h];
+			s_cols[k] = c0 >= 0 ? A.codes[offj[h] + c0] : (uint8_t)0xff;
+		}
+		__syncthreads();
+		if (A.stamps && threadIdx.x == 0)
+			A.stamps[7 * (size_t)A.nlocal + 3 * (size_t)A.stamp_u + 0] = __builtin_amdgcn_s_memtime();
+
+		{
+			constexpr int BUILDERS = NGW / COPIES;
+			constexpr int ROWS_EACH = (SA_CODE_ROWS + BUILDERS - 1) / BUILDERS;
+			const int a_lo = ((gw + grp) / COPIES) * ROWS_EACH;
+			uint8_t *const slot = s_prof + copy * (NSLOT * 16) + lig * 16;
 #pragma unroll 4
-		for (int q = 0; q < K; q++) {
-			int bq[2];
-#pragma unroll
-			for (int h = 0; h < 2; h++) {
-				const int c = (int)s_cols[h * W + lig * K + q];
-				bq[h] = c == 0xff ? -1 : c;
-			}
-#pragma unroll
-			for (int r = 0; r < ROWS_EACH; r++) {
-				const int a = a_lo + r;
-				if (a >= SA_CODE_ROWS)
-					break;
-				uint32_t v = 0;
+			for (int q = 0; q < K; q++) {
+				int bq[2];
 #pragma unroll
 				for (int h = 0; h < 2; h++) {
-					int e = 0;
-					if (a < SA_SUB_DIM && bq[h] >= 0) {
-						e = (int)sub[a * SA_SUB_DIM + bq[h]] + A.pconst;
-						if (METHOD == SA_METHOD_GA && pad[h] != 0 && lig * K + q == pad[h])
-							e -= A.q;
-					}
-					v |= (uint32_t)(e & 0xffff) << (16 * h);
-				}
-				*reinterpret_cast<uint32_t *>(slot + a * ROWSTRIDE + (q >> 2) * PARTSTRIDE + (q & 3) * 4) = v;
+					const int c = (int)s_cols[h * W + lig * K + q];
+					bq[h] = c == 0xff ? -1 : c;
+				}
+#pragma unroll
+				for (int r = 0; r < ROWS_EACH; r++) {
+					const int a = a_lo + r;
+					if (a >= SA_CODE_ROWS)
+						break;
+					uint32_t v = 0;
+#pragma unroll
+					for (int h = 0; h < 2; h++) {
+						int e = 0;
+						if (a < SA_SUB_DIM && bq[h] >= 0) {
+							e = (int)sub[a * SA_SUB_DIM + bq[h]] + A.pconst;
+							if (METHOD == SA_METHOD_GA && pad[h] != 0 && lig * K + q == pad[h])
+								e -= A.q;
+						}
+						v |= (uint32_t)(e & 0xffff) << (16 * h);
+					}
+					*reinterpret_cast<uint32_t *>(slot + a * ROWSTRIDE + (q >> 2) * PARTSTRIDE + (q & 3) * 4) = v;
+				}
 			}
 		}
 	}
@@ -403,10 +407,18 @@
 			V[q] = inj0, Y[q] = inj0;
 	}
 
-	__syncthreads();
+	if (!held)
+		__syncthreads();
 	for (int k = lane; k < NG * GSTRIDE; k += 64)
 		s_ring[k] = (uint16_t)NOPWORD;
-	__syncthreads();
+	if (!held)
+		__syncthreads();
+	else
+		__builtin_amdgcn_wave_barrier();
+	if (A.stamps && threadIdx.x == 0) {
+		A.stamps[7 * (size_t)A.nlocal + 3 * (size_t)A.stamp_u + 1] = __builtin_amdgcn_s_memtime();
+		A.stamps[7 * (size_t)A.nlocal + 3 * (size_t)A.stamp_u + 2] = (unsigned long long)(held ? 1 : 0);
+	}
 	uint32_t ev_lo = METHOD == SA_METHOD_GA ? 0x8000u : 0u, ev_hi;
 	uint32_t gm, gmask;
 	if (lean) {
@@ -867,50 +879,59 @@
 		__syncthreads();
 	}
 	const uint32_t wave_slot = __builtin_amdgcn_s_getreg((3 << 11) | 4);
+	int32_t held_c = -1, held_pair = -1;
 	for (;;) {
 		if (threadIdx.x == 0)
 			s_next = (int32_t)atomicAdd(A0.counter, 1u);
 		__syncthreads();
-		const int32_t u = __builtin_amdgcn_readfirstlane(s_next);
+		const int32_t r = __builtin_amdgcn_readfirstlane(s_next);
 		__syncthreads();
-		if (u >= A0.nlocal)
+		if (r >= A0.nruns)
 			break;
-		const uint32_t ut = (uint32_t)__builtin_amdgcn_readfirstlane((int32_t)A0.ulist[2 * (size_t)u]);
-		const int c = (int)(ut >> SA_PK_UTILE_BITS);
-		const int32_t t = (int32_t)(ut & ((1u << SA_PK_UTILE_BITS) - 1u));
-		const SaPkClassArgs &P = A0.pkc[c];
-		SaSysArgs A = A0;
-		A.tile_pair = __builtin_amdgcn_readfirstlane((int32_t)A0.ulist[2 * (size_t)u + 1]);
-		A.jlist = uniform_ptr(P.jlist);
-		A.tprefix = uniform_ptr(P.tprefix);
-		A.dense_off = uniform_ptr(P.dense_off);
-		A.ncols = __builtin_amdgcn_readfirstlane(P.ncols);
-		A.npart = __builtin_amdgcn_readfirstlane(P.npart);
-		A.delta = __builtin_amdgcn_readfirstlane(P.delta);
-		A.pk_base = __builtin_amdgcn_readfirstlane(P.pk_base);
-		A.rotate_prio = A0.rotate_prio ? (int32_t)(4u + (wave_slot & 3u)) : 0;
-		A.chunk = __builtin_amdgcn_readfirstlane(P.chunk);
-		A.lvp = P.lv;
-		const int32_t ntiles = __builtin_amdgcn_readfirstlane(A.tprefix[(A.ncols + 1) >> 1]) + A.npart;
-		const unsigned long long st0 = A0.stamps ? __builtin_amdgcn_s_memrealtime() : 0ull;
-		const unsigned long long sc0 = A0.stamps ? __builtin_amdgcn_s_memtime() : 0ull;
-		A.stamp_u = u;
-		switch (__builtin_amdgcn_readfirstlane(P.k) - KLO) {
-#define SA_BCASE(D)                                                  \
-	case D:                                                      \
-		if constexpr (KLO + D <= KMAX)                       \
-			pk_tile<METHOD, G, KLO + D, F16>(A, t, ntiles); \
+		const int32_t u0 = uload(A0.urun + r), u1 = uload(A0.urun + r + 1);
+		for (int32_t u = u0; u < u1; u++) {
+			if (u > u0)
+				__syncthreads();
+			const uint32_t ut = (uint32_t)__builtin_amdgcn_readfirstlane((int32_t)A0.ulist[2 * (size_t)u]);
+			const int c = (int)(ut >> SA_PK_UTILE_BITS);
+			const int32_t t = (int32_t)(ut & ((1u << SA_PK_UTILE_BITS) - 1u));
+			const SaPkClassArgs &P = A0.pkc[c];
+			SaSysArgs A = A0;
+			A.tile_pair = __builtin_amdgcn_readfirstlane((int32_t)A0.ulist[2 * (size_t)u + 1]);
+			const int32_t held = c == held_c && A.tile_pair == held_pair ? 1 : 0;
+			held_c = c;
+			held_pair = A.tile_pair;
+			A.jlist = uniform_ptr(P.jlist);
+			A.tprefix = uniform_ptr(P.tprefix);
+			A.dense_off = uniform_ptr(P.dense_off);
+			A.ncols = __builtin_amdgcn_readfirstlane(P.ncols);
+			A.npart = __builtin_amdgcn_readfirstlane(P.npart);
+			A.delta = __builtin_amdgcn_readfirstlane(P.delta);
+			A.pk_base = __builtin_amdgcn_readfirstlane(P.pk_base);
+			A.rotate_prio = A0.rotate_prio ? (int32_t)(4u + (wave_slot & 3u)) : 0;
+			A.chunk = __builtin_amdgcn_readfirstlane(P.chunk);
+			A.lvp = P.lv;
+			const int32_t ntiles = __builtin_amdgcn_readfirstlane(A.tprefix[(A.ncols + 1) >> 1]) + A.npart;
+			const unsigned long long st0 = A0.stamps ? __builtin_amdgcn_s_memrealtime() : 0ull;
+			const unsigned long long sc0 = A0.stamps ? __builtin_amdgcn_s_memtime() : 0ull;
+			A.stamp_u = u;
+			switch (__builtin_amdgcn_readfirstlane(P.k) - KLO) {
+#define SA_BCASE(D)                                                        \
+	case D:                                                            \
+		if constexpr (KLO + D <= KMAX)                             \
+			pk_tile<METHOD, G, KLO + D, F16>(A, t, ntiles, held); \
 		break;
-			SA_BCASE(0) SA_BCASE(1) SA_BCASE(2) SA_BCASE(3) SA_BCASE(4) SA_BCASE(5) SA_BCASE(6) SA_BCASE(7)
+				SA_BCASE(0) SA_BCASE(1) SA_BCASE(2) SA_BCASE(3) SA_BCASE(4) SA_BCASE(5) SA_BCASE(6) SA_BCASE(7)
 #undef SA_BCASE
-		default:
-			break;
-		}
-		if (A0.stamps && threadIdx.x == 0) {
-			A0.stamps[3 * (size_t)u + 0] = st0;
-			A0.stamps[3 * (size_t)u + 1] = __builtin_amdgcn_s_memrealtime();
-			A0.stamps[3 * (size_t)u + 2] = sc0;
-			A0.stamps[6 * (size_t)A0.nlocal + (size_t)u] = __builtin_amdgcn_s_memtime();
+			default:
+				break;
+			}
+			if (A0.stamps && threadIdx.x == 0) {
+				A0.stamps[3 * (size_t)u + 0] = st0;
+				A0.stamps[3 * (size_t)u + 1] = __builtin_amdgcn_s_memrealtime();
+				A0.stamps[3 * (size_t)u + 2] = sc0;
+				A0.stamps[6 * (size_t)A0.nlocal + (size_t)u] = __builtin_amdgcn_s_memtime();
+			}
 		}
 	}
 	if (threadIdx.x == 0) {
```

Result: no change. 4.013 billion pair-alignments/s (-0.0%).
